# yozoyugen/HAKAI-fem

Hardware: AMD Instinct MI355X
Metric: M element-updates/sec (hex8, 8 Gauss pts) at 1/2/4/8 MI355X; % HBM roofline (higher is better)
Workload: dtype f64

## Files before the change

hakai-fem_amd/csrc/hakai_capi.cpp:

```cpp
#include <hip/hip_runtime.h>

#include <algorithm>
#include <cmath>
#include <cstdarg>
#include <cstdio>
#include <cstdlib>
#include <cstring>
#include <map>
#include <string>
#include <vector>

#include "../../include/hakai_hip.h"
#include "hakai_history.hpp"
#include "hakai_internal.hpp"
#include "hakai_kernels.hpp"
#include "hakai_own_plan.hpp"

using hk::DevMat;

namespace {
thread_local std::string g_err;
}

namespace hkc {

int fail(int code, const char* fmt, ...) {
    char buf[1024];
    va_list ap;
    va_start(ap, fmt);
    vsnprintf(buf, sizeof buf, fmt, ap);
    va_end(ap);
    g_err = buf;
    return code;
}

int hip_fail(hipError_t e, const char* what) {
    return fail(HAKAI_ERR_DEVICE, "%s: %s", what, hipGetErrorString(e));
}

}

using hkc::fail;
using hkc::hip_fail;

#define HIPCHK(x)                                           \
    do {                                                    \
        hipError_t _e = (x);                                \
        if (_e != hipSuccess) return hip_fail(_e, #x);      \
    } while (0)

template <class T>
static hipError_t dalloc(T** p, size_t n) {
    *p = nullptr;
    if (n == 0) n = 1;
    return hipMalloc((void**)p, n * sizeof(T));
}

template <class T>
static void dfree(T*& p) {
    if (p) (void)hipFree((void*)p);
    p = nullptr;
}

namespace hkc {

static void own_free(hakai_ctx* c) {
    dfree(c->d_own_off);
    dfree(c->d_own_seq);
    dfree(c->d_own_bstart);
    dfree(c->d_own_list);
    dfree(c->d_own_q);
    dfree(c->d_own_rp);
    dfree(c->d_own_rows);
    dfree(c->d_own_ridx);
    dfree(c->d_own_dump);
    c->own_built_g = -1;
    c->own_for_g0 = -1;
    c->own_valid = false;
}

static void free_model(hakai_ctx* c) {
    contact_destroy(c);
    dfree(c->d_coord);
    dfree(c->d_u[0]);
    dfree(c->d_u[1]);
    dfree(c->d_mass);
    dfree(c->d_conn);
    dfree(c->d_flag);
    dfree(c->d_mat);
    dfree(c->d_mats);
    dfree(c->d_stress);
    dfree(c->d_strain);
    dfree(c->d_eqps);
    dfree(c->d_yield);
    dfree(c->d_triax);
    dfree(c->d_fe);
    dfree(c->d_inc_ptr);
    dfree(c->d_inc);
    dfree(c->d_inc_row);
    dfree(c->d_inc8);
    dfree(c->d_del_step);
    dfree(c->d_qbuf);
    dfree(c->d_fext);
    own_free(c);
    c->model_ok = false;
    c->state_ok = false;
}

static void free_bc(hakai_ctx* c) {
    dfree(c->d_bc_of_node);
    dfree(c->d_bc_dof);
    dfree(c->d_bc_grp);
    dfree(c->d_bc_val);
    dfree(c->d_amp_n);
    dfree(c->d_amp_off);
    dfree(c->d_amp_t);
    dfree(c->d_amp_v);
    c->nbc = 0;
}

int build_devmat(const hakai_material_t& in, DevMat& o) {
    std::memset(&o, 0, sizeof o);
    const double young = in.young, poisson = in.poisson;
    const double d1 = (1.0 - poisson), d2 = poisson, d3 = (1.0 - 2.0 * poisson) / 2.0;
    const double cc = young / (1.0 + poisson) / (1.0 - 2.0 * poisson);
    o.Dn = cc * d1;
    o.Do = cc * d2;
    o.Ds = cc * d3;
    o.G = young / 2. / (1.0 + poisson);
    o.density = in.density;
    if (in.n_plastic < 0 || in.n_plastic > hk::kMaxPlastic)
        return fail(HAKAI_ERR_ARG, "material: %d plastic rows (max %d)", in.n_plastic, hk::kMaxPlastic);
    if (in.n_ductile < 0 || in.n_ductile > hk::kMaxDuctile)
        return fail(HAKAI_ERR_ARG, "material: %d ductile rows (max %d)", in.n_ductile, hk::kMaxDuctile);
    if (in.n_plastic == 1)
        return fail(HAKAI_ERR_MODEL,
                    "material: a single *Plastic row gives an empty Hd; the reference raises BoundsError "
                    "(v2/HAKAI_j.jl:1267)");
    o.npp = in.n_plastic;
    o.nd = in.n_ductile;
    o.yield0 = in.n_plastic > 0 ? in.plastic[0] : 0.0;
    for (int r = 0; r < in.n_plastic; ++r) o.pl_eps[r] = in.plastic[2 * r + 1];
    for (int r = 0; r + 1 < in.n_plastic; ++r)
        o.Hd[r] = (in.plastic[2 * (r + 1)] - in.plastic[2 * r]) / (in.plastic[2 * (r + 1) + 1] - in.plastic[2 * r + 1]);
    for (int r = 0; r < in.n_ductile; ++r) {
        o.du_eps[r] = in.ductile[3 * r + 0];
        o.du_tri[r] = in.ductile[3 * r + 1];
    }
    double lo = 0.0, hi = 0.0;
    for (int r = 0; r < in.n_ductile; ++r) {
        lo = r == 0 ? o.du_eps[r] : std::min(lo, o.du_eps[r]);
        hi = r == 0 ? o.du_eps[r] : std::max(hi, o.du_eps[r]);
    }
    o.du_floor = in.n_ductile > 0 ? lo - (std::fabs(hi) + std::fabs(lo)) * 0x1p-40 : 0.0;
    if (!(o.du_floor == o.du_floor)) o.du_floor = -HUGE_VAL;
    o.du_skip = o.du_floor > 0.0 ? o.du_floor - o.du_floor * 0x1p-40 : -HUGE_VAL;
    return 0;
}

void pusai_table(double out[192]) {
    static const double delta[8][3] = {{-1.0, -1.0, -1.0}, {1.0, -1.0, -1.0}, {1.0, 1.0, -1.0}, {-1.0, 1.0, -1.0},
                                       {-1.0, -1.0, 1.0},  {1.0, -1.0, 1.0},  {1.0, 1.0, 1.0},  {-1.0, 1.0, 1.0}};
    const double g = 1.0 / std::sqrt(3.0);
    for (int k = 0; k < 8; ++k) {
        const double gzai = (k & 4) ? g : -g, eta = (k & 2) ? g : -g, tueta = (k & 1) ? g : -g;
        for (int i = 0; i < 8; ++i) {
            out[24 * k + i] = 1.0 / 8.0 * delta[i][0] * (1.0 + eta * delta[i][1]) * (1.0 + tueta * delta[i][2]);
            out[24 * k + 8 + i] = 1.0 / 8.0 * delta[i][1] * (1.0 + gzai * delta[i][0]) * (1.0 + tueta * delta[i][2]);
            out[24 * k + 16 + i] = 1.0 / 8.0 * delta[i][2] * (1.0 + gzai * delta[i][0]) * (1.0 + eta * delta[i][1]);
        }
    }
}

hipStream_t ctx_stream(hakai_ctx* c) { return c->stream; }
int ctx_device(hakai_ctx* c) { return c->device; }

}

static void prof_harvest(hakai_ctx* c) {
    if (c->ev_pending.empty()) return;
    (void)hipEventSynchronize(c->ev_pending.back().b);
    for (auto& p : c->ev_pending) {
        float ms = 0.f;
        if (hipEventElapsedTime(&ms, p.a, p.b) == hipSuccess) {
            c->k_ms[p.kernel] += ms;
            c->k_n[p.kernel] += 1;
        }
        c->ev_pool.push_back(p.a);
        c->ev_pool.push_back(p.b);
    }
    c->ev_pending.clear();
}

static hipEvent_t prof_event(hakai_ctx* c) {
    if (c->ev_pool.empty()) {
        if (c->ev_pending.size() >= 2048) prof_harvest(c);
        if (c->ev_pool.empty()) {
            hipEvent_t e;
            (void)hipEventCreate(&e);
            return e;
        }
    }
    hipEvent_t e = c->ev_pool.back();
    c->ev_pool.pop_back();
    return e;
}

namespace hkc {
void prof_begin(hakai_ctx* c, int kernel, EventPair* p) {
    p->kernel = -1;
    if (!c->prof || !((c->prof_mask >> kernel) & 1u)) return;
    p->kernel = kernel;
    p->a = prof_event(c);
    p->b = prof_event(c);
    (void)hipEventRecord(p->a, c->stream);
}
void prof_end(hakai_ctx* c, EventPair* p) {
    if (!c->prof || p->kernel < 0) return;
    (void)hipEventRecord(p->b, c->stream);
    c->ev_pending.push_back(*p);
}
void graph_invalidate(hakai_ctx* c) {
    c->epoch++;
    c->tdev_next = -1;
}
static void graph_free(hakai_ctx* c) {
    for (int g = 0; g < 2; ++g)
        for (int p = 0; p < 2; ++p)
            if (c->g_exec[g][p]) {
                (void)hipGraphExecDestroy(c->g_exec[g][p]);
                c->g_exec[g][p] = nullptr;
                c->g_epoch[g][p] = -1;
            }
}
}


static hk::ElemArgs elem_args(hakai_ctx* c) {
    hk::ElemArgs ea;
    std::memset(&ea, 0, sizeof ea);
    ea.coord = c->d_coord;
    ea.u = c->d_u[c->cur];
    ea.u_pre = c->d_u[1 - c->cur];
    ea.conn = c->d_conn;
    ea.flag = c->d_flag;
    ea.mat = c->d_mat;
    ea.mats = c->d_mats;
    ea.stress = c->d_stress;
    ea.strain = c->d_strain;
    for (int q = 0; q < 6; ++q) {
        ea.sc[q] = c->d_stress + q * c->ld;
        ea.ec[q] = c->d_strain + q * c->ld;
    }
    ea.eqps = c->d_eqps;
    ea.yield = c->d_yield;
    ea.triax = c->d_triax;
    ea.fe = c->d_fe;
    ea.vol = nullptr;
    ea.nE = c->nE;
    ea.nEp = c->nEp;
    ea.ld = c->ld;
    ea.del_step = c->d_del_step;
    ea.step_i = 0;
    ea.any_plastic = c->any_plastic ? 1 : 0;
    ea.pipe_blocks = (c->nEp / 32 >= (long long)c->pipe_min * c->pipe_blocks) ? c->pipe_blocks : 0;
    ea.gp_nt = c->gp_nt;
    ea.nmat = c->nmat;
    ea.exact = c->elem_exact;
    ea.pusai = c->d_pusai;
    ea.poison = c->d_poison;
    return ea;
}

static int fe_download_qe(hakai_ctx* c, double* Qe) {
    HIPCHK(hipMemcpyAsync(Qe, c->d_fe, 24 * (size_t)c->nE * sizeof(double), hipMemcpyDeviceToHost, c->stream));
    HIPCHK(hipStreamSynchronize(c->stream));
    return 0;
}

static int fe_upload_qe(hakai_ctx* c, const double* Qe) {
    HIPCHK(hipMemcpyAsync(c->d_fe, Qe, 24 * (size_t)c->nE * sizeof(double), hipMemcpyHostToDevice, c->stream));
    HIPCHK(hipStreamSynchronize(c->stream));
    return 0;
}

static int fe_upload_incidence(hakai_ctx* c) {
    std::vector<int> inc(c->h_inc0.size());
    for (size_t j = 0; j < inc.size(); ++j) inc[j] = 24 * (c->h_inc0[j] >> 3) + 3 * (c->h_inc0[j] & 7);
    if (!inc.empty())
        HIPCHK(hipMemcpyAsync(c->d_inc, inc.data(), inc.size() * sizeof(int), hipMemcpyHostToDevice, c->stream));
    if (c->d_inc8) {
        std::vector<int> inc8(8 * (size_t)c->nN, (int)(24 * c->nEp));
        for (long long n = 0; n < c->nN; ++n)
            for (int j = c->h_ptr[n]; j < c->h_ptr[n + 1]; ++j) inc8[8 * n + (j - c->h_ptr[n])] = inc[j];
        HIPCHK(hipMemcpyAsync(c->d_inc8, inc8.data(), inc8.size() * sizeof(int), hipMemcpyHostToDevice, c->stream));
    }
    HIPCHK(hipStreamSynchronize(c->stream));
    return 0;
}

extern "C" {

int hakai_abi_version(void) { return HAKAI_ABI_VERSION; }
const char* hakai_last_error(void) { return g_err.c_str(); }

int hakai_device_count(int* n) {
    if (!n) return fail(HAKAI_ERR_ARG, "null");
    int cnt = 0;
    if (hipGetDeviceCount(&cnt) != hipSuccess) cnt = 0;
    *n = cnt;
    return 0;
}

int hakai_create(hakai_ctx** out, int device) {
    if (!out) return fail(HAKAI_ERR_ARG, "null ctx pointer");
    *out = nullptr;
    int cnt = 0;
    if (hipGetDeviceCount(&cnt) != hipSuccess || cnt <= 0)
        return fail(HAKAI_ERR_DEVICE, "no HIP device visible: the HAKAI MI355X path has no CPU fallback");
    if (device < 0 || device >= cnt) return fail(HAKAI_ERR_ARG, "device %d out of range (%d visible)", device, cnt);
    HIPCHK(hipSetDevice(device));
    hipDeviceProp_t prop;
    HIPCHK(hipGetDeviceProperties(&prop, device));
    if (std::strncmp(prop.gcnArchName, "gfx950", 6) != 0)
        return fail(HAKAI_ERR_DEVICE, "device %d is %s; libhakai_hip is built for gfx950 only", device,
                    prop.gcnArchName);
    hakai_ctx* c = new hakai_ctx();
    c->device = device;
    if (const char* v = std::getenv("HAKAI_PIPE_BLOCKS")) c->pipe_blocks = std::atoi(v);
    if (const char* v = std::getenv("HAKAI_GRAPH")) {
        const int g = std::atoi(v);
        c->graph = (g >= 0 && g <= 1024 && !(g & 1)) ? g : 0;
    }
    hipError_t e = hipStreamCreateWithFlags(&c->stream, hipStreamNonBlocking);
    if (e != hipSuccess) {
        delete c;
        return hip_fail(e, "hipStreamCreate");
    }
    if (dalloc(&c->d_negjac, 1) != hipSuccess || dalloc(&c->d_pusai, 192) != hipSuccess ||
        dalloc(&c->d_poison, 2) != hipSuccess || hipMemset(c->d_poison, 0, 2 * sizeof(int)) != hipSuccess) {
        dfree(c->d_negjac);
        dfree(c->d_pusai);
        dfree(c->d_poison);
        delete c;
        return fail(HAKAI_ERR_DEVICE, "hipMalloc for context bookkeeping failed");
    }
    {
        double pus[192];
        hkc::pusai_table(pus);
        bool odd = true;
        for (int k = 0; k < 8; ++k)
            for (int i = 0; i < 8; ++i) {
                const double* p = pus + 24 * k;
                odd = odd && p[i] == -p[i ^ 1] && p[8 + i] == -p[8 + (i ^ 3)] && p[16 + i] == -p[16 + (i ^ 4)];
            }
        e = odd ? hipMemcpy(c->d_pusai, pus, sizeof pus, hipMemcpyHostToDevice) : hipErrorInvalidValue;
        if (e != hipSuccess) {
            dfree(c->d_negjac);
            dfree(c->d_pusai);
            dfree(c->d_poison);
            delete c;
            return hip_fail(e, "hipMemcpy (Pusai table)");
        }
    }
    if (const char* v = std::getenv("HAKAI_ELEM_EXACT")) c->elem_exact = std::atoi(v) ? 1 : 0;
    if (const char* v = std::getenv("HAKAI_OWN_ASSEMBLY")) c->own_assembly = std::atoi(v) ? 1 : 0;
    *out = c;
    return 0;
}

int hakai_destroy(hakai_ctx* c) {
    if (!c) return 0;
    (void)hipSetDevice(c->device);
    (void)hipStreamSynchronize(c->stream);
    prof_harvest(c);
    hkc::graph_free(c);
    dfree(c->d_tstep);
    hkc::history_destroy(c);
    hkc::comm_destroy(c);
    hkc::free_model(c);
    hkc::free_bc(c);
    dfree(c->d_negjac);
    dfree(c->d_pusai);
    dfree(c->d_poison);
    for (auto e : c->ev_pool) (void)hipEventDestroy(e);
    (void)hipStreamDestroy(c->stream);
    delete c;
    return 0;
}

int hakai_upload_model(hakai_ctx* c, int64_t nNode, const double* coordmat, int64_t nElement,
                       const int64_t* elementmat, const int64_t* element_material, int32_t nMat,
                       const hakai_material_t* mats, const double* diag_M) {
    if (c) hkc::graph_invalidate(c);
    if (!c) return fail(HAKAI_ERR_ARG, "null ctx");
    if (nNode <= 0 || nElement < 0 || !coordmat || (nElement > 0 && (!elementmat || !element_material)) || nMat <= 0 ||
        !mats || !diag_M)
        return fail(HAKAI_ERR_ARG, "upload_model: bad arguments");
    if (26 * (nElement + 32) + 8 >= (int64_t)INT32_MAX || nNode >= (int64_t)INT32_MAX)
        return fail(HAKAI_ERR_ARG, "upload_model: mesh too large for int32 indexing on one rank");
    if (192 * (nElement + 32) >= (int64_t)1 << 32)
        return fail(HAKAI_ERR_ARG, "upload_model: %lld elements exceed one context's 32-bit element-kernel offsets "
                    "(max %lld); split the mesh over ranks", (long long)nElement, (long long)(((int64_t)1 << 32) / 192 - 32));
    if (24 * (nNode + 1) >= (int64_t)1 << 32)
        return fail(HAKAI_ERR_ARG, "upload_model: %lld nodes exceed one context's 32-bit element-kernel offsets "
                    "(max %lld); split the mesh over ranks", (long long)nNode, (long long)(((int64_t)1 << 32) / 24 - 1));
    HIPCHK(hipSetDevice(c->device));
    (void)hipStreamSynchronize(c->stream);
    hkc::history_destroy(c);
    hkc::free_model(c);
    hkc::free_bc(c);
    const long long nN = nNode, nE = nElement;
    const long long nEp = ((nE + 31) / 32) * 32;
    std::vector<int> conn((size_t)(8 * nEp), 0), mat((size_t)nEp, 0);
    for (long long e = 0; e < nE; ++e) {
        for (int i = 0; i < 8; ++i) {
            const int64_t n = elementmat[8 * e + i];
            if (n < 1 || n > nN) return fail(HAKAI_ERR_ARG, "elementmat[%d,%lld] = %lld out of 1..%lld", i + 1, e + 1, (long long)n, nN);
            conn[8 * e + i] = (int)(n - 1);
        }
        const int64_t m = element_material[e];
        if (m < 1 || m > nMat) return fail(HAKAI_ERR_ARG, "element_material[%lld] = %lld out of 1..%d", e + 1, (long long)m, nMat);
        mat[e] = (int)(m - 1);
    }
    std::vector<double> mass((size_t)nN);
    for (long long n = 0; n < nN; ++n) {
        const double m0 = diag_M[3 * n], m1 = diag_M[3 * n + 1], m2 = diag_M[3 * n + 2];
        if (!(m0 == m1 && m1 == m2))
            return fail(HAKAI_ERR_ARG, "diag_M: node %lld has different masses per dof", n + 1);
        mass[n] = m0;
    }
    c->h_mats.assign((size_t)nMat, DevMat());
    c->nmat = nMat;
    c->has_ductile = false;
    for (int i = 0; i < nMat; ++i) {
        int r = hkc::build_devmat(mats[i], c->h_mats[i]);
        if (r) return r;
    }
    c->any_plastic = false;
    for (long long e = 0; e < nE; ++e) {
        if (c->h_mats[mat[e]].nd > 0) c->has_ductile = true;
        if (c->h_mats[mat[e]].npp > 0) c->any_plastic = true;
    }
    std::vector<int> ptr((size_t)nN + 1, 0), inc((size_t)(8 * nE));
    for (long long j = 0; j < 8 * nE; ++j) ptr[conn[j] + 1]++;
    for (long long n = 0; n < nN; ++n) ptr[n + 1] += ptr[n];
    {
        std::vector<int> fill(ptr.begin(), ptr.end() - 1);
        for (long long j = 0; j < 8 * nE; ++j) inc[fill[conn[j]]++] = (int)j;
    }
    int maxinc = 0;
    for (long long n = 0; n < nN; ++n) maxinc = std::max(maxinc, ptr[n + 1] - ptr[n]);
    c->nN = nN;
    c->nE = nE;
    c->nEp = nEp;
    c->ld = 8 * nEp;
    const size_t ld = (size_t)c->ld;
    HIPCHK(dalloc(&c->d_coord, 3 * (size_t)nN));
    HIPCHK(dalloc(&c->d_u[0], 3 * (size_t)nN));
    HIPCHK(dalloc(&c->d_u[1], 3 * (size_t)nN));
    HIPCHK(dalloc(&c->d_mass, (size_t)nN));
    HIPCHK(dalloc(&c->d_conn, 8 * (size_t)nEp));
    HIPCHK(dalloc(&c->d_flag, (size_t)nEp));
    HIPCHK(dalloc(&c->d_mat, (size_t)nEp));
    HIPCHK(dalloc(&c->d_del_step, (size_t)nEp + 2));
    HIPCHK(dalloc(&c->d_mats, (size_t)nMat));
    HIPCHK(dalloc(&c->d_stress, 6 * ld));
    HIPCHK(dalloc(&c->d_strain, 6 * ld));
    HIPCHK(dalloc(&c->d_eqps, ld));
    HIPCHK(dalloc(&c->d_yield, ld));
    HIPCHK(dalloc(&c->d_triax, ld));
    c->fe_len = 26 * nEp + 8;
    HIPCHK(dalloc(&c->d_fe, (size_t)c->fe_len));
    HIPCHK(dalloc(&c->d_inc_ptr, (size_t)nN + 1));
    HIPCHK(dalloc(&c->d_inc, 8 * (size_t)nE));
    HIPCHK(dalloc(&c->d_inc_row, 8 * (size_t)nE));
    HIPCHK(dalloc(&c->d_qbuf, 3 * (size_t)nN));
    hipStream_t s = c->stream;
    HIPCHK(hipMemcpyAsync(c->d_coord, coordmat, 3 * nN * sizeof(double), hipMemcpyHostToDevice, s));
    HIPCHK(hipMemcpyAsync(c->d_mass, mass.data(), nN * sizeof(double), hipMemcpyHostToDevice, s));
    if (nE) {
        HIPCHK(hipMemcpyAsync(c->d_conn, conn.data(), 8 * nEp * sizeof(int), hipMemcpyHostToDevice, s));
        HIPCHK(hipMemcpyAsync(c->d_mat, mat.data(), nEp * sizeof(int), hipMemcpyHostToDevice, s));
        HIPCHK(hipMemcpyAsync(c->d_inc_row, inc.data(), 8 * nE * sizeof(int), hipMemcpyHostToDevice, s));
    }
    HIPCHK(hipMemcpyAsync(c->d_mats, c->h_mats.data(), nMat * sizeof(DevMat), hipMemcpyHostToDevice, s));
    HIPCHK(hipMemcpyAsync(c->d_inc_ptr, ptr.data(), (nN + 1) * sizeof(int), hipMemcpyHostToDevice, s));
    if (maxinc <= 8) HIPCHK(dalloc(&c->d_inc8, 8 * (size_t)nN));
    HIPCHK(hipStreamSynchronize(s));
    c->max_inc = maxinc;
    c->h_ptr = ptr;
    c->h_inc0 = inc;
    {
        int r = fe_upload_incidence(c);
        if (r) return r;
    }
    c->h_coord.assign(coordmat, coordmat + 3 * nN);
    c->h_conn.assign(conn.begin(), conn.begin() + 8 * nE);
    c->h_mat.assign(mat.begin(), mat.begin() + nE);
    c->h_young.resize((size_t)nMat);
    for (int i = 0; i < nMat; ++i) c->h_young[i] = mats[i].young;
    c->model_ok = true;
    c->state_ok = false;
    return hakai_reset_state(c, 0, nullptr, nullptr, 1.0);
}

int hakai_set_bc(hakai_ctx* c, const hakai_bc_t* bc) {
    if (c) hkc::graph_invalidate(c);
    if (!c || !bc) return fail(HAKAI_ERR_ARG, "null");
    if (!c->model_ok) return fail(HAKAI_ERR_STATE, "set_bc before upload_model");
    HIPCHK(hipSetDevice(c->device));
    (void)hipStreamSynchronize(c->stream);
    hkc::free_bc(c);
    const int G = bc->n_groups;
    if (G <= 0) return hkc::history_bc_changed(c);
    std::map<long long, std::pair<int, double>> last;
    for (int g = 0; g < G; ++g) {
        if (bc->amp_n[g] == 1)
            return fail(HAKAI_ERR_MODEL, "BC group %d: one-point amplitude, the reference raises BoundsError (:598)", g + 1);
        for (int64_t en = bc->entry_off[g]; en < bc->entry_off[g + 1]; ++en)
            for (int64_t d = bc->dof_off[en]; d < bc->dof_off[en + 1]; ++d) {
                const int64_t dof = bc->dofs[d];
                if (dof < 1 || dof > 3 * c->nN) return fail(HAKAI_ERR_ARG, "BC dof %lld out of range", (long long)dof);
                last[dof - 1] = std::make_pair(g, bc->entry_value[en]);
            }
    }
    std::vector<int> dof, grp;
    std::vector<double> val;
    for (auto& kv : last) {
        dof.push_back((int)kv.first);
        grp.push_back(kv.second.first);
        val.push_back(kv.second.second);
    }
    std::vector<int> amp_n(G), amp_off(G);
    long long n_amp = 0;
    for (int g = 0; g < G; ++g) {
        amp_n[g] = bc->amp_n[g];
        amp_off[g] = (int)bc->amp_off[g];
        n_amp = std::max<long long>(n_amp, bc->amp_off[g] + bc->amp_n[g]);
    }
    c->nbc = (int)dof.size();
    HIPCHK(dalloc(&c->d_bc_dof, dof.size()));
    HIPCHK(dalloc(&c->d_bc_grp, grp.size()));
    HIPCHK(dalloc(&c->d_bc_val, val.size()));
    HIPCHK(dalloc(&c->d_amp_n, (size_t)G));
    HIPCHK(dalloc(&c->d_amp_off, (size_t)G));
    HIPCHK(dalloc(&c->d_amp_t, (size_t)n_amp));
    HIPCHK(dalloc(&c->d_amp_v, (size_t)n_amp));
    hipStream_t s = c->stream;
    if (!dof.empty()) {
        HIPCHK(hipMemcpyAsync(c->d_bc_dof, dof.data(), dof.size() * sizeof(int), hipMemcpyHostToDevice, s));
        HIPCHK(hipMemcpyAsync(c->d_bc_grp, grp.data(), grp.size() * sizeof(int), hipMemcpyHostToDevice, s));
        HIPCHK(hipMemcpyAsync(c->d_bc_val, val.data(), val.size() * sizeof(double), hipMemcpyHostToDevice, s));
    }
    HIPCHK(hipMemcpyAsync(c->d_amp_n, amp_n.data(), G * sizeof(int), hipMemcpyHostToDevice, s));
    HIPCHK(hipMemcpyAsync(c->d_amp_off, amp_off.data(), G * sizeof(int), hipMemcpyHostToDevice, s));
    if (n_amp) {
        HIPCHK(hipMemcpyAsync(c->d_amp_t, bc->amp_time, n_amp * sizeof(double), hipMemcpyHostToDevice, s));
        HIPCHK(hipMemcpyAsync(c->d_amp_v, bc->amp_value, n_amp * sizeof(double), hipMemcpyHostToDevice, s));
    }
    if (!dof.empty()) {
        std::vector<int> of((size_t)c->nN, -1);
        for (size_t i = dof.size(); i-- > 0;) of[(size_t)dof[i] / 3] = (int)i;
        HIPCHK(dalloc(&c->d_bc_of_node, of.size()));
        HIPCHK(hipMemcpyAsync(c->d_bc_of_node, of.data(), of.size() * sizeof(int), hipMemcpyHostToDevice, s));
    }
    HIPCHK(hipStreamSynchronize(s));
    return hkc::history_bc_changed(c);
}

int hakai_reset_state(hakai_ctx* c, int64_t n_ic, const int64_t* ic_dofs, const double* ic_values, double d_time) {
    if (c) hkc::graph_invalidate(c);
    if (c) c->own_valid = false;
    if (!c) return fail(HAKAI_ERR_ARG, "null");
    if (!c->model_ok) return fail(HAKAI_ERR_STATE, "reset_state before upload_model");
    HIPCHK(hipSetDevice(c->device));
    hipStream_t s = c->stream;
    const size_t fn = 3 * (size_t)c->nN;
    c->cur = 0;
    HIPCHK(hipMemsetAsync(c->d_u[0], 0, fn * sizeof(double), s));
    HIPCHK(hipMemsetAsync(c->d_u[1], 0, fn * sizeof(double), s));
    HIPCHK(hipMemsetAsync(c->d_fe, 0, (size_t)c->fe_len * sizeof(double), s));
    HIPCHK(hipMemsetAsync(c->d_del_step, 0, ((size_t)c->nEp + 2) * sizeof(int), s));
    HIPCHK(hk::launch_reset_gp(c->d_stress, c->d_strain, c->d_eqps, c->d_yield, c->d_triax, c->d_flag, c->d_mat,
                               c->d_mats, c->nE, c->nEp, c->ld, s));
    c->h_velo0.assign(fn, 0.0);
    c->q_from_buf = false;
    c->fe_ok = c->triax_ok = true;
    c->steps_done = 0;
    HIPCHK(hipMemsetAsync(c->d_poison, 0, 2 * sizeof(int), s));
    hkc::comm_reset(c);
    if (n_ic > 0) {
        if (!ic_dofs || !ic_values) return fail(HAKAI_ERR_ARG, "reset_state: null IC arrays");
        std::vector<double> dpre(fn, 0.0);
        for (int64_t j = 0; j < n_ic; ++j) {
            const int64_t d = ic_dofs[j];
            if (d < 1 || d > (int64_t)fn) return fail(HAKAI_ERR_ARG, "IC dof %lld out of range", (long long)d);
            dpre[d - 1] = -ic_values[j] * d_time;
            c->h_velo0[d - 1] = ic_values[j];
        }
        HIPCHK(hipMemcpyAsync(c->d_u[1 - c->cur], dpre.data(), fn * sizeof(double), hipMemcpyHostToDevice, s));
        HIPCHK(hipStreamSynchronize(s));
    }
    c->state_ok = true;
    if (int r = hkc::contact_state_reset(c, c->h_velo0.data())) return r;
    if (int r = hkc::history_restart(c)) return r;
    HIPCHK(hipStreamSynchronize(s));
    return 0;
}

static int own_materialize(hakai_ctx* c);

int hakai_upload_state(hakai_ctx* c, const hakai_state_t* st) {
    if (c) hkc::graph_invalidate(c);
    if (!c || !st) return fail(HAKAI_ERR_ARG, "null");
    if (!c->model_ok) return fail(HAKAI_ERR_STATE, "upload_state before upload_model");
    HIPCHK(hipSetDevice(c->device));
    if (c->own_valid && !c->fe_ok && !st->Q && !st->Qe) {
        bool dels = false;
        for (long long e = 0; st->element_flag && e < c->nE && !dels; ++e) dels = st->element_flag[e] == 0;
        if (dels || c->comm)
            return fail(HAKAI_ERR_STATE, "upload_state: the last element step's forces exist only as owner-computed "
                        "node sums (a contact overflow skipped the call's last step); upload Q (from "
                        "hakai_download_state) or Qe with this state");
        if (int r = own_materialize(c)) return r;
    }
    c->own_valid = false;
    hipStream_t s = c->stream;
    const size_t fn = 3 * (size_t)c->nN, nGP = 8 * (size_t)c->nE;
    if (st->disp) HIPCHK(hipMemcpyAsync(c->d_u[c->cur], st->disp, fn * sizeof(double), hipMemcpyHostToDevice, s));
    if (st->disp_pre)
        HIPCHK(hipMemcpyAsync(c->d_u[1 - c->cur], st->disp_pre, fn * sizeof(double), hipMemcpyHostToDevice, s));
    if (st->velo) c->h_velo0.assign(st->velo, st->velo + fn);
    if (st->Q) {
        HIPCHK(hipMemcpyAsync(c->d_qbuf, st->Q, fn * sizeof(double), hipMemcpyHostToDevice, s));
        c->q_from_buf = true;
    }
    if (st->integ_stress || st->integ_strain) {
        double* tmp = nullptr;
        HIPCHK(dalloc(&tmp, 6 * nGP));
        if (st->integ_stress) {
            HIPCHK(hipMemcpyAsync(tmp, st->integ_stress, 6 * nGP * sizeof(double), hipMemcpyHostToDevice, s));
            HIPCHK(hk::launch_aos_to_soa6(tmp, c->d_stress, (long long)nGP, c->ld, s));
        }
        if (st->integ_strain) {
            HIPCHK(hipMemcpyAsync(tmp, st->integ_strain, 6 * nGP * sizeof(double), hipMemcpyHostToDevice, s));
            HIPCHK(hk::launch_aos_to_soa6(tmp, c->d_strain, (long long)nGP, c->ld, s));
        }
        HIPCHK(hipStreamSynchronize(s));
        dfree(tmp);
    }
    if (st->integ_yield_stress)
        HIPCHK(hipMemcpyAsync(c->d_yield, st->integ_yield_stress, nGP * sizeof(double), hipMemcpyHostToDevice, s));
    if (st->integ_eq_plastic_strain)
        HIPCHK(hipMemcpyAsync(c->d_eqps, st->integ_eq_plastic_strain, nGP * sizeof(double), hipMemcpyHostToDevice, s));
    if (st->integ_triax_stress)
        HIPCHK(hipMemcpyAsync(c->d_triax, st->integ_triax_stress, nGP * sizeof(double), hipMemcpyHostToDevice, s));
    if (st->element_flag) {
        std::vector<int> f((size_t)c->nE);
        for (long long e = 0; e < c->nE; ++e) f[e] = st->element_flag[e] != 0 ? 1 : 0;
        HIPCHK(hipMemcpyAsync(c->d_flag, f.data(), c->nE * sizeof(int), hipMemcpyHostToDevice, s));
        std::vector<int> ds((size_t)c->nE);
        for (long long e = 0; e < c->nE; ++e) ds[e] = f[e] ? 0 : -1;
        HIPCHK(hipMemcpyAsync(c->d_del_step, ds.data(), c->nE * sizeof(int), hipMemcpyHostToDevice, s));
        HIPCHK(hipMemsetAsync(c->d_del_step + c->nEp, 0, 2 * sizeof(int), s));
        HIPCHK(hipStreamSynchronize(s));
        bool any = false;
        for (long long e = 0; e < c->nE; ++e) any |= !f[e];
        if (any && !st->Qe) {
            std::vector<double> qe(24 * (size_t)c->nE);
            int r = fe_download_qe(c, qe.data());
            if (r) return r;
            for (long long e = 0; e < c->nE; ++e)
                if (!f[e]) std::fill(qe.begin() + 24 * e, qe.begin() + 24 * (e + 1), 0.0);
            if ((r = fe_upload_qe(c, qe.data()))) return r;
        }
    }
    if (st->Qe) {
        int r = fe_upload_qe(c, st->Qe);
        if (r) return r;
    }
    HIPCHK(hipMemsetAsync(c->d_poison, 0, 2 * sizeof(int), s));
    HIPCHK(hipStreamSynchronize(s));
    c->steps_done = 0;
    c->fe_ok = c->triax_ok = true;
    hkc::comm_reset(c);
    c->state_ok = true;
    if (int r = hkc::history_restart(c)) return r;
    if (c->contact) {
        if (int r = hkc::contact_state_reset(c, c->h_velo0.empty() ? nullptr : c->h_velo0.data())) return r;
        HIPCHK(hipStreamSynchronize(s));
    }
    return 0;
}

int hakai_download_state(hakai_ctx* c, hakai_state_t* st) {
    if (!c || !st) return fail(HAKAI_ERR_ARG, "null");
    if (!c->state_ok) return fail(HAKAI_ERR_STATE, "download_state without state");
    if (st->Qe && !c->fe_ok)
        return fail(HAKAI_ERR_STATE, "download_state: Qe is not available after a call whose last steps a contact "
                    "overflow skipped (owner-computed assembly keeps node sums only); Q is -- or step once more");
    if (st->integ_triax_stress && !c->triax_ok)
        return fail(HAKAI_ERR_STATE, "download_state: integ_triax_stress is not available after a call whose last "
                    "steps a contact overflow skipped (it is stored on a call's last step); step once more");
    HIPCHK(hipSetDevice(c->device));
    hipStream_t s = c->stream;
    const size_t fn = 3 * (size_t)c->nN, nGP = 8 * (size_t)c->nE;
    HIPCHK(hipStreamSynchronize(s));
    if (st->disp) HIPCHK(hipMemcpyAsync(st->disp, c->d_u[c->cur], fn * sizeof(double), hipMemcpyDeviceToHost, s));
    if (st->disp_pre)
        HIPCHK(hipMemcpyAsync(st->disp_pre, c->d_u[1 - c->cur], fn * sizeof(double), hipMemcpyDeviceToHost, s));
    if (st->velo) {
        if (c->steps_done == 0) {
            std::memcpy(st->velo, c->h_velo0.data(), fn * sizeof(double));
        } else {
            std::vector<double> a(fn), b(fn);
            HIPCHK(hipMemcpyAsync(a.data(), c->d_u[c->cur], fn * sizeof(double), hipMemcpyDeviceToHost, s));
            HIPCHK(hipMemcpyAsync(b.data(), c->d_u[1 - c->cur], fn * sizeof(double), hipMemcpyDeviceToHost, s));
            HIPCHK(hipStreamSynchronize(s));
            for (size_t i = 0; i < fn; ++i) {
                const double dd = a[i] - b[i];
                st->velo[i] = dd / c->last_dt;
            }
        }
    }
    if (st->Q) {
        if (c->q_from_buf) {
            HIPCHK(hipMemcpyAsync(st->Q, c->d_qbuf, fn * sizeof(double), hipMemcpyDeviceToHost, s));
        } else {
            double* tmp = nullptr;
            HIPCHK(dalloc(&tmp, fn));
            if (c->own_valid)
                HIPCHK(hk::launch_own_q(c->d_own_q, c->d_own_rp, c->d_own_ridx, c->d_own_rows, tmp, c->nN, s));
            else
                HIPCHK(hk::launch_gather_q(c->d_inc_ptr, c->d_inc, c->d_fe, tmp, c->nN, s));
            HIPCHK(hipMemcpyAsync(st->Q, tmp, fn * sizeof(double), hipMemcpyDeviceToHost, s));
            HIPCHK(hipStreamSynchronize(s));
            dfree(tmp);
        }
    }
    if (st->integ_stress || st->integ_strain) {
        double* tmp = nullptr;
        HIPCHK(dalloc(&tmp, 6 * nGP));
        if (st->integ_stress) {
            HIPCHK(hk::launch_soa_to_aos6(c->d_stress, tmp, (long long)nGP, c->ld, s));
            HIPCHK(hipMemcpyAsync(st->integ_stress, tmp, 6 * nGP * sizeof(double), hipMemcpyDeviceToHost, s));
            HIPCHK(hipStreamSynchronize(s));
        }
        if (st->integ_strain) {
            HIPCHK(hk::launch_soa_to_aos6(c->d_strain, tmp, (long long)nGP, c->ld, s));
            HIPCHK(hipMemcpyAsync(st->integ_strain, tmp, 6 * nGP * sizeof(double), hipMemcpyDeviceToHost, s));
            HIPCHK(hipStreamSynchronize(s));
        }
        dfree(tmp);
    }
    if (st->integ_yield_stress)
        HIPCHK(hipMemcpyAsync(st->integ_yield_stress, c->d_yield, nGP * sizeof(double), hipMemcpyDeviceToHost, s));
    if (st->integ_eq_plastic_strain)
        HIPCHK(hipMemcpyAsync(st->integ_eq_plastic_strain, c->d_eqps, nGP * sizeof(double), hipMemcpyDeviceToHost, s));
    if (st->integ_triax_stress)
        HIPCHK(hipMemcpyAsync(st->integ_triax_stress, c->d_triax, nGP * sizeof(double), hipMemcpyDeviceToHost, s));
    if (st->element_flag) {
        std::vector<int> f((size_t)c->nE);
        HIPCHK(hipMemcpyAsync(f.data(), c->d_flag, c->nE * sizeof(int), hipMemcpyDeviceToHost, s));
        HIPCHK(hipStreamSynchronize(s));
        for (long long e = 0; e < c->nE; ++e) st->element_flag[e] = (f[e] == 1) ? 1 : 0;
    }
    if (st->Qe) {
        int r = fe_download_qe(c, st->Qe);
        if (r) return r;
    }
    HIPCHK(hipStreamSynchronize(s));
    return 0;
}

static bool own_upload(hakai_ctx* c, const hk::OwnSched& sc, const hk::OwnPlan& pl) {
    hkc::own_free(c);
    const long long nN = c->nN, G = (long long)sc.bstart.size() - 1;
    std::vector<int> bst(sc.bstart.begin(), sc.bstart.end());
    hipStream_t s = c->stream;
    auto up = [&](int** d, const std::vector<int>& h) -> hipError_t {
        hipError_t e = dalloc(d, std::max<size_t>(h.size(), 1));
        if (e == hipSuccess && !h.empty()) e = hipMemcpyAsync(*d, h.data(), h.size() * sizeof(int), hipMemcpyHostToDevice, s);
        return e;
    };
    if (up(&c->d_own_off, pl.off) || up(&c->d_own_seq, sc.seq) || up(&c->d_own_bstart, bst) ||
        up(&c->d_own_list, pl.list) || up(&c->d_own_rp, pl.rp) || up(&c->d_own_ridx, pl.ridx) ||
        dalloc(&c->d_own_q, 3 * (size_t)nN) || dalloc(&c->d_own_rows, 3 * (size_t)std::max(pl.rows, 1LL)) ||
        dalloc(&c->d_own_dump, 8 * (size_t)G) ||
        hipMemsetAsync(c->d_own_q, 0, 3 * (size_t)nN * sizeof(double), s) ||
        hipStreamSynchronize(s)) {
        hkc::own_free(c);
        return false;
    }
    c->own_nop = (int)pl.ne;
    c->own_slots = pl.max_slots;
    c->own_rows = pl.rows;
    c->own_entries = pl.ne;
    c->own_built_g = G;
    c->own_s = pl.S;
    c->own_round2 = pl.round2;
    c->own_banded = sc.banded ? 1 : 0;
    return true;
}

static long long own_grid(const hakai_ctx* c) {
    const long long nb = c->nEp / 32;
    const bool pipe = nb >= (long long)c->pipe_min * c->pipe_blocks && c->pipe_blocks > 0;
    return pipe ? std::min<long long>(nb, c->pipe_blocks) : 0;
}

static int own_materialize(hakai_ctx* c) {
    if (!c->own_valid) return 0;
    if (c->comm)
        return fail(HAKAI_ERR_STATE, "owner-computed assembly cannot be switched off or rebuilt on a multi-GPU rank "
                    "mid-run: upload or reset the state first");
    HIPCHK(hk::launch_own_q(c->d_own_q, c->d_own_rp, c->d_own_ridx, c->d_own_rows, c->d_qbuf, c->nN, c->stream));
    c->q_from_buf = true;
    c->own_valid = false;
    return 0;
}

static bool own_use(hakai_ctx* c) {
    if (!c->own_assembly || c->nmat > hk::kMaxLdsMats || c->nE <= 0)
        return false;
    const long long G0 = own_grid(c);
    if (G0 <= 0) return false;
    bool ok = c->own_built_g > 0;
    if (c->own_for_g0 != G0) {
        if (c->own_valid && own_materialize(c)) return false;
        const hk::OwnInput in{c->nE, c->nN, c->nEp, c->h_conn, c->h_ptr, c->h_inc0, c->max_inc,
                              c->own_band_rows, c->own_pass_batches, hkc::comm_dn_nodes(c),
                              {hk::own_slot_cap(c->elem_exact != 0, 1, c->nmat),
                               hk::own_slot_cap(c->elem_exact != 0, 2, c->nmat)}};
        hk::OwnSched sc;
        hk::OwnPlan pl;
        ok = hk::own_choose(in, G0, sc, pl) && own_upload(c, sc, pl);
        if (!ok) {
            hkc::own_free(c);
            c->own_built_g = -2;
        }
        c->own_for_g0 = G0;
    }
    if (ok && c->elem_exact && c->own_round2 > 0 && c->own_assembly == 1 && !(c->comm && c->own_valid))
        return false;
    return ok;
}

enum { kPhaseA1 = 1, kPhaseRest = 2, kPhaseA2 = 4, kPhaseA3 = 8, kPhaseAll = 15 };
static int step_once(hakai_ctx* c, double t, double d_time, bool last, int phase = kPhaseAll) {
    hipStream_t s = c->stream;
    EventPair ep;
    if (c->contact) {
        const int part_bit[3] = {kPhaseA1, kPhaseA2, kPhaseA3};
        for (int part = 1; part <= 3; ++part) {
            if (!(phase & part_bit[part - 1]) || (part > 1 && !hkc::contact_multi(c))) continue;
            hkc::prof_begin(c, HAKAI_K_CONTACT, &ep);
            const int rc = hkc::contact_phase(c, part, t, d_time);
            hkc::prof_end(c, &ep);
            if (rc) return rc;
        }
    }
    if (!(phase & kPhaseRest)) return 0;
    const int par = c->cur;
    hk::NodalArgs na;
    na.u = c->d_u[c->cur];
    na.u_pre_out = c->d_u[1 - c->cur];
    na.mass = c->d_mass;
    na.inc_ptr = c->d_inc_ptr;
    na.inc = c->d_inc;
    na.inc8 = c->d_inc8;
    na.fe = c->d_fe;
    const bool own = own_use(c);
    if (c->own_valid && !own) {
        if (int r = own_materialize(c)) return r;
    }
    na.qbuf = c->q_from_buf ? c->d_qbuf : nullptr;
    na.fext = nullptr;
    na.nN = c->nN;
    na.dt = d_time;
    na.bc_of_node = nullptr;
    const bool own_q = c->own_valid && !na.qbuf;
    na.own_q = own_q ? c->d_own_q : nullptr;
    na.own_rp = own_q ? c->d_own_rp : nullptr;
    na.own_rows = own_q ? c->d_own_rows : nullptr;
    na.own_ridx = own_q ? c->d_own_ridx : nullptr;
    hk::BCArgs ba;
    ba.dof = c->d_bc_dof;
    ba.grp = c->d_bc_grp;
    ba.val = c->d_bc_val;
    ba.n = c->nbc;
    ba.amp_n = c->d_amp_n;
    ba.amp_off = c->d_amp_off;
    ba.amp_t = c->d_amp_t;
    ba.amp_v = c->d_amp_v;
    ba.out = c->d_u[1 - c->cur];
    ba.ct = t * d_time;
    ba.t_rd = c->g_trd;
    ba.dt = d_time;
    ba.poison = c->d_poison;
    na.poison = c->d_poison;
    const bool fuse_bc = c->nbc > 0 && c->d_bc_of_node && c->fuse_bc && !c->comm &&
                         (c->nN <= kFuseBcMaxNodes || c->fuse_bc == 2);
    if (fuse_bc) {
        na.bc_of_node = c->d_bc_of_node;
        na.bc = ba;
    }
    int rc = 0;
    if (c->contact) {
        if (hkc::contact_multi(c)) {
            hkc::prof_begin(c, HAKAI_K_CONTACT_SUM, &ep);
            rc = hkc::contact_step_b(c);
            hkc::prof_end(c, &ep);
            if (rc) return rc;
        }
        na.fext = c->d_fext;
    }
    rc = hkc::comm_pre_nodal(c);
    if (rc) return rc;
    if (c->hist && (rc = hkc::history_seed(c, na, s))) return rc;
    hkc::prof_begin(c, HAKAI_K_NODAL, &ep);
    HIPCHK(hk::launch_nodal(na, s));
    hkc::prof_end(c, &ep);
    hkc::CommFix fix;
    rc = hkc::comm_post_nodal(c, d_time, &fix);
    if (rc) return rc;
    if (c->nbc > 0 && !fuse_bc) {
        hkc::prof_begin(c, HAKAI_K_BC, &ep);
        HIPCHK(hk::launch_bc(ba, s));
        hkc::prof_end(c, &ep);
    }
    if (c->hist && (rc = hkc::history_step(c, na, fix, t, c->g_trd, s))) return rc;
    c->cur = 1 - c->cur;
    c->q_from_buf = false;
    hk::ElemArgs ea = elem_args(c);
    ea.step_i = (int)t;
    if (own) {
        ea.own = c->own_s;
        ea.own_grid = (int)c->own_built_g;
        ea.own_seq = c->d_own_seq;
        ea.own_bstart = c->d_own_bstart;
        ea.own_off = c->d_own_off;
        ea.own_list = reinterpret_cast<const int4*>(c->d_own_list);
        ea.own_nop = c->own_nop;
        ea.own_slots = c->own_slots;
        ea.own_q = c->d_own_q;
        ea.own_rows = c->d_own_rows;
        ea.own_dump = c->d_own_dump;
    }
    if (c->g_trd) {
        ea.t_rd = c->g_trd;
        ea.t_wr = c->d_tstep + par;
    }
    hkc::prof_begin(c, HAKAI_K_ELEMENT, &ep);
    HIPCHK(hk::launch_element(ea, c->has_ductile, last, s));
    hkc::prof_end(c, &ep);
    c->own_valid = own;
    c->own_steps += own ? 1 : 0;
    c->fe_ok = !own || last;
    c->triax_ok = last;
    rc = hkc::comm_post_element(c, (long long)t);
    if (rc) return rc;
    rc = hkc::contact_post_step(c);
    if (rc) return rc;
    c->steps_done++;
    c->last_dt = d_time;
    return 0;
}

static bool graph_eligible(const hakai_ctx* c, double t) {
    return c->graph && !c->comm && !c->prof && !c->q_from_buf && c->nE > 0 && hkc::contact_graph_ok(c, t) &&
           !hkc::history_needs_seed(c) &&
           c->own_valid == own_use(const_cast<hakai_ctx*>(c));
}

static int step_graph(hakai_ctx* c, double t, double d_time, int len) {
    hipStream_t s = c->stream;
    const int p0 = c->cur;
    const int gi = len == 2 ? 1 : 0;
    hipGraphExec_t& ge = c->g_exec[gi][p0];
    if (!c->d_tstep) HIPCHK(dalloc(&c->d_tstep, 2));
    if (c->tdev_next != (long long)t) HIPCHK(hk::launch_set_step(c->d_tstep + (1 - p0), t - 1.0, s));
    if (ge && (c->g_epoch[gi][p0] != c->epoch || c->g_dt[gi][p0] != d_time || c->g_len[gi][p0] != len)) {
        HIPCHK(hipStreamSynchronize(s));
        (void)hipGraphExecDestroy(ge);
        ge = nullptr;
    }
    if (!ge) {
        hipGraph_t g = nullptr;
        HIPCHK(hipStreamBeginCapture(s, hipStreamCaptureModeThreadLocal));
        int rc = 0;
        for (int k = 0; k < len && !rc; ++k) {
            c->g_trd = c->d_tstep + (1 - c->cur);
            rc = step_once(c, t + k, d_time, false);
        }
        c->g_trd = nullptr;
        hipError_t e = hipStreamEndCapture(s, &g);
        if (rc) {
            if (g) (void)hipGraphDestroy(g);
            return rc;
        }
        if (e != hipSuccess) return hip_fail(e, "hipStreamEndCapture (step graph)");
        e = hipGraphInstantiate(&ge, g, nullptr, nullptr, 0);
        (void)hipGraphDestroy(g);
        if (e != hipSuccess) {
            ge = nullptr;
            return hip_fail(e, "hipGraphInstantiate (step graph)");
        }
        c->g_epoch[gi][p0] = c->epoch;
        c->g_dt[gi][p0] = d_time;
        c->g_len[gi][p0] = len;
    } else {
        hkc::contact_graph_advance(c, t + len - 1);
        c->q_from_buf = false;
        c->own_steps += c->own_valid ? len : 0;
        c->fe_ok = !c->own_valid;
        c->triax_ok = false;
        c->steps_done += len;
        c->last_dt = d_time;
    }
    HIPCHK(hipGraphLaunch(ge, s));
    c->tdev_next = (long long)t + len;
    c->graph_steps += len;
    return 0;
}

struct CallSnap {
    int cur = 0;
    long long done = 0;
    bool fe_ok = true, triax_ok = true, own_valid = false, q_from_buf = false;
    bool comm_pending = false;
    int comm_par = 0;
};
static CallSnap call_snap(const hakai_ctx* c) {
    CallSnap s;
    hkc::comm_pending_get(c, &s.comm_pending, &s.comm_par);
    s.cur = c->cur;
    s.done = c->steps_done;
    s.fe_ok = c->fe_ok;
    s.triax_ok = c->triax_ok;
    s.own_valid = c->own_valid;
    s.q_from_buf = c->q_from_buf;
    return s;
}

static int finish_call(hakai_ctx* c, double t_first, int64_t n_steps, const CallSnap& s0) {
    const int rc = hkc::contact_check(c);
    if (rc && c->contact) {
        int pz[2] = {0, 0};
        HIPCHK(hipMemcpy(pz, c->d_poison, sizeof pz, hipMemcpyDeviceToHost));
        if (pz[0]) {
            c->poison_step = pz[1];
            const long long good = (long long)pz[1] - (long long)t_first;
            const bool rolled = good >= 0 && good <= n_steps;
            if (rolled) {
                c->cur = (good & 1) ? 1 - s0.cur : s0.cur;
                c->steps_done = s0.done + good;
                if (good == 0) {
                    c->fe_ok = s0.fe_ok;
                    c->triax_ok = s0.triax_ok;
                    c->own_valid = s0.own_valid;
                    c->q_from_buf = s0.q_from_buf;
                } else {
                    c->fe_ok = !c->own_valid;
                    c->triax_ok = false;
                }
                hkc::comm_rollback(c, good > 0, (long long)pz[1] - 1, s0.comm_pending, s0.comm_par);
            }
            hkc::graph_invalidate(c);
            hkc::contact_after_overflow(c, c->steps_done);
            if (!rolled) (void)hkc::contact_exchange_retry(c);
            HIPCHK(hipMemset(c->d_poison, 0, 2 * sizeof(int)));
            const std::string msg = hakai_last_error();
            return fail(rc, "%s; step %d was not applied: the state is that after step %d", msg.c_str(), pz[1],
                        pz[1] - 1);
        }
    }
    return rc;
}

static int step_call(hakai_ctx* c, double t_first, int64_t n_steps, double d_time);
static constexpr int kExchangeRetries = 8;

int hakai_step(hakai_ctx* c, double t_first, int64_t n_steps, double d_time) {
    if (!c) return fail(HAKAI_ERR_ARG, "null");
    if (!c->model_ok || !c->state_ok) return fail(HAKAI_ERR_STATE, "step before upload_model/reset_state");
    if (n_steps < 0 || !(d_time > 0)) return fail(HAKAI_ERR_ARG, "step: n_steps=%lld d_time=%g", (long long)n_steps, d_time);
    if (n_steps > 1 && hkc::comm_is_local(c))
        return fail(HAKAI_ERR_ARG, "step: an in-process group is stepped one step per call, rank by rank");
    if (hkc::comm_is_local(c) && hkc::contact_multi(c) && hkc::comm_size(c) > 1)
        return fail(HAKAI_ERR_STATE, "step: rank %d of an in-process group with multi-GPU contact is stepped by "
                    "hakai_step_group only", hkc::comm_rank(c));
    HIPCHK(hipSetDevice(c->device));
    for (int attempt = 0;; ++attempt) {
        const int rc = step_call(c, t_first, n_steps, d_time);
        if (!rc || attempt >= kExchangeRetries || !hkc::contact_exchange_retry(c)) return rc;
        ++c->exchange_retries;
        n_steps -= (int64_t)(c->poison_step - (long long)t_first);
        t_first = (double)c->poison_step;
    }
}

static int step_call(hakai_ctx* c, double t_first, int64_t n_steps, double d_time) {
    (void)own_use(c);
    const CallSnap s0 = call_snap(c);
    int64_t it = 0;
    while (it < n_steps) {
        const double t = t_first + (double)it;
        int rc;
        const int len = (c->graph > 2 && it + c->graph < n_steps) ? c->graph : 2;
        if (c->graph && it + len < n_steps && graph_eligible(c, t)) {
            rc = step_graph(c, t, d_time, len);
            it += len;
        } else {
            rc = step_once(c, t, d_time, it == n_steps - 1);
            c->tdev_next = -1;
            ++it;
        }
        if (rc) return rc;
    }
    return finish_call(c, t_first, n_steps, s0);
}

static int step_group_call(hakai_ctx** ctxs, int32_t n, double t_first, int64_t n_steps, double d_time) {
    std::vector<CallSnap> s0(n);
    for (int r = 0; r < n; ++r) {
        (void)own_use(ctxs[r]);
        s0[r] = call_snap(ctxs[r]);
    }
    const int phases[4] = {kPhaseA1, kPhaseA2, kPhaseA3, kPhaseRest};
    for (int64_t it = 0; it < n_steps; ++it) {
        const double t = t_first + (double)it;
        const bool last = it == n_steps - 1;
        for (int ph : phases)
            for (int r = 0; r < n; ++r) {
                if (ctxs[0]->group_serial == 2) HIPCHK(hk::launch_hold(96, ctxs[r]->stream));
                if (int rc = step_once(ctxs[r], t, d_time, last, ph)) return rc;
                if (ph == kPhaseRest) ctxs[r]->tdev_next = -1;
                if (ctxs[0]->group_serial) HIPCHK(hipStreamSynchronize(ctxs[r]->stream));
            }
    }
    int first = 0;
    for (int r = 0; r < n; ++r) {
        const int rc = finish_call(ctxs[r], t_first, n_steps, s0[r]);
        if (rc && !first) first = rc;
    }
    return first;
}

int hakai_step_group(hakai_ctx** ctxs, int32_t n, double t_first, int64_t n_steps, double d_time) {
    if (!ctxs || n <= 0) return fail(HAKAI_ERR_ARG, "step_group: no contexts");
    if (n_steps < 0 || !(d_time > 0)) return fail(HAKAI_ERR_ARG, "step_group: n_steps=%lld d_time=%g",
                                                  (long long)n_steps, d_time);
    for (int r = 0; r < n; ++r) {
        hakai_ctx* c = ctxs[r];
        if (!c) return fail(HAKAI_ERR_ARG, "step_group: null context %d", r);
        if (!c->model_ok || !c->state_ok) return fail(HAKAI_ERR_STATE, "step_group: rank %d has no model/state", r);
        if (n > 1 && (!c->comm || hkc::comm_rank(c) != r || hkc::comm_size(c) != n ||
                      hkc::comm_peer_ctx(c, r) != c))
            return fail(HAKAI_ERR_ARG, "step_group: context %d is not rank %d of an in-process group of %d", r, r, n);
        hkc::graph_invalidate(c);
    }
    HIPCHK(hipSetDevice(ctxs[0]->device));
    for (int attempt = 0;; ++attempt) {
        const int rc = step_group_call(ctxs, n, t_first, n_steps, d_time);
        if (!rc || attempt >= kExchangeRetries) return rc;
        bool retry = true;
        for (int r = 0; r < n; ++r) retry = hkc::contact_exchange_retry(ctxs[r]) && retry;
        if (!retry) return rc;
        const long long p = ctxs[0]->poison_step;
        for (int r = 1; r < n; ++r)
            if (ctxs[r]->poison_step != p)
                return fail(rc, "step_group: ranks disagree on the poisoned step (rank 0: %lld, rank %d: %lld)", p, r,
                            ctxs[r]->poison_step);
        for (int r = 0; r < n; ++r) ++ctxs[r]->exchange_retries;
        n_steps -= (int64_t)(p - (long long)t_first);
        t_first = (double)p;
    }
}

int hakai_graph_steps(hakai_ctx* c, int64_t* n) {
    if (!c || !n) return fail(HAKAI_ERR_ARG, "null");
    *n = c->graph_steps;
    return 0;
}

int hakai_stat(hakai_ctx* c, const char* key, int64_t* value) {
    if (!c || !key || !value) return fail(HAKAI_ERR_ARG, "null");
    if (!std::strcmp(key, "graph_steps")) *value = c->graph_steps;
    else if (!std::strcmp(key, "own_steps")) *value = c->own_steps;
    else if (!std::strcmp(key, "exchange_retries")) *value = c->exchange_retries;
    else if (!std::strcmp(key, "own_rows")) *value = c->own_built_g > 0 ? c->own_rows : -1;
    else if (!std::strcmp(key, "own_entries")) *value = c->own_built_g > 0 ? c->own_entries : -1;
    else if (!std::strcmp(key, "own_superbatch")) *value = c->own_built_g > 0 ? c->own_s : 0;
    else if (!std::strcmp(key, "own_round2")) *value = c->own_built_g > 0 ? c->own_round2 : 0;
    else if (!std::strcmp(key, "own_slots")) *value = c->own_built_g > 0 ? c->own_slots : 0;
    else if (!std::strcmp(key, "own_banded")) *value = c->own_built_g > 0 ? c->own_banded : 0;
    else if (!std::strcmp(key, "own_grid")) *value = c->own_built_g > 0 ? c->own_built_g : 0;
    else return fail(HAKAI_ERR_ARG, "unknown stat '%s'", key);
    return 0;
}

int hakai_sync(hakai_ctx* c) {
    if (!c) return fail(HAKAI_ERR_ARG, "null");
    HIPCHK(hipSetDevice(c->device));
    HIPCHK(hipStreamSynchronize(c->stream));
    return 0;
}

int hakai_deleted(hakai_ctx* c, int64_t* n_deleted, int64_t* log, int64_t cap) {
    if (!c) return fail(HAKAI_ERR_ARG, "null");
    if (!c->model_ok) return fail(HAKAI_ERR_STATE, "deleted before upload_model");
    HIPCHK(hipSetDevice(c->device));
    std::vector<int> ds((size_t)c->nE);
    if (c->nE) HIPCHK(hipMemcpyAsync(ds.data(), c->d_del_step, c->nE * sizeof(int), hipMemcpyDeviceToHost, c->stream));
    HIPCHK(hipStreamSynchronize(c->stream));
    std::vector<std::pair<long long, long long>> v;
    for (long long e = 0; e < c->nE; ++e)
        if (ds[e] > 0) v.push_back(std::make_pair((long long)ds[e], e + 1 + c->elem_offset));
    std::sort(v.begin(), v.end());
    if (n_deleted) *n_deleted = (int64_t)v.size();
    if (log)
        for (long long i = 0; i < (long long)v.size() && i < cap; ++i) {
            log[2 * i] = v[i].first;
            log[2 * i + 1] = v[i].second;
        }
    return 0;
}

int hakai_set_tuning(hakai_ctx* c, const char* key, int64_t value) {
    if (c) hkc::graph_invalidate(c);
    if (!c || !key) return fail(HAKAI_ERR_ARG, "set_tuning: null");
    if (!std::strcmp(key, "elem_pipe_blocks")) {
        if (value < 0 || value > 65536) return fail(HAKAI_ERR_ARG, "elem_pipe_blocks out of range");
        c->pipe_blocks = (int)value;
        return 0;
    }
    if (!std::strcmp(key, "elem_gp_nt")) {
        if (value != 0 && value != 1) return fail(HAKAI_ERR_ARG, "elem_gp_nt must be 0 or 1");
        c->gp_nt = (int)value;
        return 0;
    }
    if (!std::strcmp(key, "fuse_bc")) {
        if (value < 0 || value > 2) return fail(HAKAI_ERR_ARG, "fuse_bc must be 0, 1 or 2 (any mesh size)");
        c->fuse_bc = (int)value;
        return 0;
    }
    if (!std::strcmp(key, "elem_pipe_min")) {
        if (value < 0 || value > 1024) return fail(HAKAI_ERR_ARG, "elem_pipe_min out of range");
        c->pipe_min = (int)value;
        return 0;
    }
    if (!std::strcmp(key, "elem_exact")) {
        if (value != 0 && value != 1) return fail(HAKAI_ERR_ARG, "elem_exact must be 0 or 1");
        if (c->elem_exact != (int)value && c->own_for_g0 != -1) {
            if (!(c->comm && c->own_valid)) {
                c->own_for_g0 = -1;
            } else if (c->own_built_g > 0 && c->own_slots > hk::own_slot_cap(value != 0, c->own_s, c->nmat)) {
                return fail(HAKAI_ERR_STATE, "elem_exact: the owner-assembly lists of this multi-GPU rank need %d LDS "
                            "slots, more than the %s kernel has; switch between calls after hakai_upload_state / "
                            "hakai_reset_state", c->own_slots, value ? "reference-order" : "fused");
            }
        }
        c->elem_exact = (int)value;
        return 0;
    }
    if (!std::strcmp(key, "group_serial")) {
        if (value < 0 || value > 2) return fail(HAKAI_ERR_ARG, "group_serial must be 0, 1 or 2");
        c->group_serial = (int)value;
        return 0;
    }
    if (!std::strcmp(key, "nodal_padded")) {
        if (!value) {
            dfree(c->d_inc8);
            return 0;
        }
        return c->d_inc8 ? 0 : fail(HAKAI_ERR_STATE, "padded incidence table unavailable (>8 incidences)");
    }
    if (!std::strcmp(key, "own_assembly")) {
        if (value < 0 || value > 2) return fail(HAKAI_ERR_ARG, "own_assembly must be 0, 1 or 2");
        c->own_assembly = (int)value;
        return 0;
    }
    if (!std::strcmp(key, "own_pass_batches")) {
        if (value < 0 || value > 2) return fail(HAKAI_ERR_ARG, "own_pass_batches must be 0, 1 or 2");
        if (c->own_pass_batches != (int)value) c->own_for_g0 = -1;
        c->own_pass_batches = (int)value;
        return 0;
    }
    if (!std::strcmp(key, "own_band_rows")) {
        if (value < 0 || value > 4096) return fail(HAKAI_ERR_ARG, "own_band_rows must be in [0, 4096]");
        if (c->own_band_rows != (int)value) c->own_for_g0 = -1;
        c->own_band_rows = (int)value;
        return 0;
    }
    if (!std::strcmp(key, "graph")) {
        if (value < 0 || value > 1024 || (value & 1)) return fail(HAKAI_ERR_ARG, "graph must be 0 or an even step count <= 1024");
        c->graph = (int)value;
        return 0;
    }
    if (!std::strcmp(key, "history_one_block")) {
        if (value < -1 || value > 1) return fail(HAKAI_ERR_ARG, "history_one_block must be -1 (by size), 0 or 1");
        c->hist_one_block = (int)value;
        return 0;
    }
    if (!std::strncmp(key, "contact_", 8)) {
        HIPCHK(hipSetDevice(c->device));
        return hkc::contact_tuning(c, key, value);
    }
    return fail(HAKAI_ERR_ARG, "unknown tuning key '%s'", key);
}

int hakai_set_element_offset(hakai_ctx* c, int64_t element_offset) {
    if (c) hkc::graph_invalidate(c);
    if (!c || element_offset < 0) return fail(HAKAI_ERR_ARG, "set_element_offset: bad args");
    c->elem_offset = element_offset;
    return 0;
}

int hakai_negative_jacobians(hakai_ctx* c, int64_t* n) {
    if (!c || !n) return fail(HAKAI_ERR_ARG, "null");
    if (!c->state_ok) return fail(HAKAI_ERR_STATE, "negative_jacobians without state");
    HIPCHK(hipSetDevice(c->device));
    HIPCHK(hipMemsetAsync(c->d_negjac, 0, sizeof(unsigned long long), c->stream));
    HIPCHK(hk::launch_negjac(elem_args(c), c->d_negjac, c->stream));
    unsigned long long v = 0;
    HIPCHK(hipMemcpyAsync(&v, c->d_negjac, sizeof v, hipMemcpyDeviceToHost, c->stream));
    HIPCHK(hipStreamSynchronize(c->stream));
    *n = (int64_t)v;
    return 0;
}

int hakai_node_stress_strain(hakai_ctx* c, double* node_stress, double* node_strain, double* node_eqps,
                             double* node_mises, double* node_triax) {
    if (!c) return fail(HAKAI_ERR_ARG, "null");
    if (!c->state_ok) return fail(HAKAI_ERR_STATE, "node_stress_strain without state");
    HIPCHK(hipSetDevice(c->device));
    hipStream_t s = c->stream;
    const size_t nN = (size_t)c->nN;
    double *ns = nullptr, *nn = nullptr, *ne = nullptr, *nm = nullptr, *nt = nullptr;
    HIPCHK(dalloc(&ns, 6 * nN));
    HIPCHK(dalloc(&nn, 6 * nN));
    HIPCHK(dalloc(&ne, nN));
    HIPCHK(dalloc(&nm, nN));
    HIPCHK(dalloc(&nt, nN));
    HIPCHK(hk::launch_node_average(c->d_inc_ptr, c->d_inc_row, c->d_stress, c->d_strain, c->d_eqps, c->d_triax, c->ld,
                                   c->nN, ns, nn, ne, nm, nt, s));
    if (node_stress) HIPCHK(hipMemcpyAsync(node_stress, ns, 6 * nN * sizeof(double), hipMemcpyDeviceToHost, s));
    if (node_strain) HIPCHK(hipMemcpyAsync(node_strain, nn, 6 * nN * sizeof(double), hipMemcpyDeviceToHost, s));
    if (node_eqps) HIPCHK(hipMemcpyAsync(node_eqps, ne, nN * sizeof(double), hipMemcpyDeviceToHost, s));
    if (node_mises) HIPCHK(hipMemcpyAsync(node_mises, nm, nN * sizeof(double), hipMemcpyDeviceToHost, s));
    if (node_triax) HIPCHK(hipMemcpyAsync(node_triax, nt, nN * sizeof(double), hipMemcpyDeviceToHost, s));
    HIPCHK(hipStreamSynchronize(s));
    dfree(ns);
    dfree(nn);
    dfree(ne);
    dfree(nm);
    dfree(nt);
    return 0;
}

int hakai_profile_enable(hakai_ctx* c, int on) { return hakai_profile_mask(c, on ? (1u << HAKAI_K_COUNT) - 1 : 0u); }

int hakai_profile_mask(hakai_ctx* c, uint32_t mask) {
    if (c) hkc::graph_invalidate(c);
    if (!c) return fail(HAKAI_ERR_ARG, "null");
    if (!mask) prof_harvest(c);
    c->prof = mask != 0;
    c->prof_mask = mask;
    for (int k = 0; k < HAKAI_K_COUNT; ++k) {
        c->k_ms[k] = 0;
        c->k_n[k] = 0;
    }
    return 0;
}

int hakai_profile_read(hakai_ctx* c, int kernel, double* total_ms, int64_t* launches) {
    if (!c || kernel < 0 || kernel >= HAKAI_K_COUNT) return fail(HAKAI_ERR_ARG, "bad profile query");
    (void)hipSetDevice(c->device);
    prof_harvest(c);
    if (total_ms) *total_ms = c->k_ms[kernel];
    if (launches) *launches = c->k_n[kernel];
    return 0;
}

int hakai_stress_hexa(int device, int64_t nNode, int64_t nElement, double* Qe, double* integ_stress,
                      double* integ_strain, double* integ_yield_stress, double* integ_eq_plastic_strain,
                      const double* position, const double* d_disp, const int64_t* elementmat,
                      const int64_t* element_flag, int32_t integ_num, int32_t nMat, const hakai_material_t* mats,
                      const int64_t* element_material, double* elementVolume) {
    if (integ_num != 8) return fail(HAKAI_ERR_ARG, "integ_num must be 8 (v2/HAKAI_j.jl:177)");
    if (!Qe || !integ_stress || !integ_strain || !integ_yield_stress || !integ_eq_plastic_strain || !position ||
        !d_disp || !element_flag)
        return fail(HAKAI_ERR_ARG, "stress_hexa: null array");
    hakai_ctx* c = nullptr;
    int r = hakai_create(&c, device);
    if (r) return r;
    struct Guard {
        hakai_ctx* c;
        ~Guard() { hakai_destroy(c); }
    } guard{c};
    std::vector<double> ones(3 * (size_t)nNode, 1.0);
    r = hakai_upload_model(c, nNode, position, nElement, elementmat, element_material, nMat, mats, ones.data());
    if (r) return r;
    std::vector<double> zero(3 * (size_t)nNode, 0.0), mdu(3 * (size_t)nNode);
    for (size_t i = 0; i < mdu.size(); ++i) mdu[i] = -d_disp[i];
    hakai_state_t st;
    std::memset(&st, 0, sizeof st);
    st.disp = zero.data();
    st.disp_pre = mdu.data();
    st.integ_stress = integ_stress;
    st.integ_strain = integ_strain;
    st.integ_yield_stress = integ_yield_stress;
    st.integ_eq_plastic_strain = integ_eq_plastic_strain;
    st.element_flag = const_cast<int64_t*>(element_flag);
    r = hakai_upload_state(c, &st);
    if (r) return r;
    hipStream_t s = c->stream;
    double* d_vol = nullptr;
    HIPCHK(dalloc(&d_vol, (size_t)c->nEp));
    HIPCHK(hipMemsetAsync(c->d_fe, 0, 24 * (size_t)nElement * sizeof(double), s));
    hk::ElemArgs ea = elem_args(c);
    ea.vol = d_vol;
    ea.pipe_blocks = 0;
    HIPCHK(hk::launch_element(ea, false, false, s));
    std::vector<double> fe(24 * (size_t)nElement), vol((size_t)nElement);
    HIPCHK(hipMemcpyAsync(fe.data(), c->d_fe, fe.size() * sizeof(double), hipMemcpyDeviceToHost, s));
    HIPCHK(hipMemcpyAsync(vol.data(), d_vol, vol.size() * sizeof(double), hipMemcpyDeviceToHost, s));
    HIPCHK(hipStreamSynchronize(s));
    dfree(d_vol);
    c->steps_done = 1;
    c->last_dt = 1.0;
    hakai_state_t out;
    std::memset(&out, 0, sizeof out);
// ... 38 lines not shown
```

hakai-fem_amd/csrc/hakai_comm.cpp:

```cpp
#include <hip/hip_runtime.h>
#include <rccl/rccl.h>

#include <algorithm>
#include <cstdint>
#include <cstring>
#include <map>
#include <mutex>
#include <vector>

#include "hakai_internal.hpp"

namespace hkc {

struct LocalGroup;

struct Comm {
    int mode = 0;
    ncclComm_t nc = nullptr;
    LocalGroup* group = nullptr;
    long long group_key = 0;
    int rank = 0, nranks = 1;
    hipStream_t cs = nullptr;
    hipEvent_t ev_packed[2] = {nullptr, nullptr}, ev_done = nullptr;
    int nslot = 0;
// ... 224 lines not shown
        hipEventCreateWithFlags(&m->ev_done, hipEventDisableTiming) != hipSuccess) {
        c->comm = m;
        hkc::comm_destroy(c);
        return fail(HAKAI_ERR_DEVICE, "comm_init: stream/event creation failed");
    }
    c->comm = m;
    return 0;
}

__global__ void k_gather_local(hkc::LocalGather g, char* dst) {
    const int q = (int)blockIdx.y;
    const char* src = g.src[q];
    char* out = dst + g.off[q];
    const long long nb = g.bytes[q];
    if (!src || nb <= 0) return;
    const long long nw = nb >> 3;
    const long long stride = (long long)gridDim.x * blockDim.x;
    const long long i0 = blockIdx.x * (long long)blockDim.x + threadIdx.x;
    for (long long i = i0; i < nw; i += stride)
        reinterpret_cast<unsigned long long*>(out)[i] = reinterpret_cast<const unsigned long long*>(src)[i];
    for (long long i = (nw << 3) + i0; i < nb; i += stride) out[i] = src[i];
}

}

namespace hkc {

int gather_local(hakai_ctx* c, const LocalGather& g, int n, void* dst) {
    long long mx = 0;
    for (int q = 0; q < n; ++q) {
        if (((uintptr_t)g.src[q] | (uintptr_t)g.off[q]) & 7)
            return fail(HAKAI_ERR_ARG, "gather_local: rank %d block not 8-byte aligned", q);
        mx = std::max(mx, g.bytes[q]);
    }
    if (mx <= 0) return 0;
    const unsigned gx = (unsigned)std::min<long long>(std::max<long long>(((mx >> 3) + 255) / 256, 1), 512);
    hipLaunchKernelGGL(k_gather_local, dim3(gx, (unsigned)n), dim3(256), 0, c->stream, g, (char*)dst);
    HIPCHK(hipGetLastError());
    return 0;
}

void comm_destroy(hakai_ctx* c) {
    Comm* m = c->comm;
    if (!m) return;
    if (m->cs) (void)hipStreamSynchronize(m->cs);
    (void)hipStreamSynchronize(c->stream);
    free_iface(m);
    if (m->nc) (void)ncclCommDestroy(m->nc);
    if (m->group) {
        std::lock_guard<std::mutex> lk(g_groups_mu);
        m->group->ctx[m->rank] = nullptr;
        if (--m->group->refs == 0) {
            g_groups.erase(m->group_key);
            delete m->group;
        }
    }
    for (int p = 0; p < 2; ++p)
        if (m->ev_packed[p]) (void)hipEventDestroy(m->ev_packed[p]);
    if (m->ev_ag_ready) (void)hipEventDestroy(m->ev_ag_ready);
    if (m->ev_ag_done) (void)hipEventDestroy(m->ev_ag_done);
    if (m->ev_done) (void)hipEventDestroy(m->ev_done);
    if (m->cs) (void)hipStreamDestroy(m->cs);
    delete m;
    c->comm = nullptr;
}

bool comm_is_local(const hakai_ctx* c) {
    return c->comm && c->comm->mode == 1 && (c->comm->n_up + c->comm->n_dn > 0 || c->contact);
}

int comm_rank(const hakai_ctx* c) { return c->comm ? c->comm->rank : 0; }
int comm_size(const hakai_ctx* c) { return c->comm ? c->comm->nranks : 1; }

int comm_allgather_raw(hakai_ctx* c, const void* send, void* recv, size_t bytes) {
    Comm* m = c->comm;
    if (!m || m->mode != 0) return fail(HAKAI_ERR_STATE, "all-gather: not an RCCL communicator");
    if (bytes == 0) return 0;
    HIPCHK(hipEventRecord(m->ev_ag_ready, c->stream));
    HIPCHK(hipStreamWaitEvent(m->cs, m->ev_ag_ready, 0));
    NCCLCHK(ncclAllGather(send, recv, bytes, ncclUint8, m->nc, m->cs));
    HIPCHK(hipEventRecord(m->ev_ag_done, m->cs));
    HIPCHK(hipStreamWaitEvent(c->stream, m->ev_ag_done, 0));
    return 0;
}

int comm_allgatherv_raw(hakai_ctx* c, const void* send, void* recv, const size_t* bytes, const size_t* off) {
    Comm* m = c->comm;
    if (!m || m->mode != 0) return fail(HAKAI_ERR_STATE, "all-gather: not an RCCL communicator");
    HIPCHK(hipEventRecord(m->ev_ag_ready, c->stream));
    HIPCHK(hipStreamWaitEvent(m->cs, m->ev_ag_ready, 0));
    NCCLCHK(ncclGroupStart());
    for (int q = 0; q < m->nranks; ++q) {
        if (q == m->rank) continue;
        if (bytes[m->rank]) NCCLCHK(ncclSend(send, bytes[m->rank], ncclUint8, q, m->nc, m->cs));
        if (bytes[q]) NCCLCHK(ncclRecv(static_cast<char*>(recv) + off[q], bytes[q], ncclUint8, q, m->nc, m->cs));
    }
    NCCLCHK(ncclGroupEnd());
    HIPCHK(hipEventRecord(m->ev_ag_done, m->cs));
    HIPCHK(hipStreamWaitEvent(c->stream, m->ev_ag_done, 0));
    return 0;
}

int comm_allreduce_min_u64(hakai_ctx* c, const void* send, void* recv, size_t count) {
    Comm* m = c->comm;
    if (!m || m->mode != 0) return fail(HAKAI_ERR_STATE, "all-reduce: not an RCCL communicator");
    if (count == 0) return 0;
    HIPCHK(hipEventRecord(m->ev_ag_ready, c->stream));
    HIPCHK(hipStreamWaitEvent(m->cs, m->ev_ag_ready, 0));
    NCCLCHK(ncclAllReduce(send, recv, count, ncclUint64, ncclMin, m->nc, m->cs));
    HIPCHK(hipEventRecord(m->ev_ag_done, m->cs));
    HIPCHK(hipStreamWaitEvent(c->stream, m->ev_ag_done, 0));
    return 0;
}

bool comm_is_rccl(const hakai_ctx* c) { return c->comm && c->comm->mode == 0; }

hakai_ctx* comm_peer_ctx(hakai_ctx* c, int q) {
    Comm* m = c->comm;
    if (!m || m->mode != 1 || !m->group || q < 0 || q >= m->nranks) return nullptr;
    return m->group->ctx[q];
}

int comm_reset(hakai_ctx* c) {
    if (c->comm) c->comm->pending = false;
    return 0;
}

void comm_pending_get(const hakai_ctx* c, bool* pending, int* par) {
    *pending = c->comm && c->comm->pending;
    *par = c->comm ? c->comm->pending_par : 0;
}

void comm_rollback(hakai_ctx* c, bool had_good, long long last_good, bool pending, int par) {
    Comm* m = c->comm;
    if (!m) return;
    if (had_good) {
        m->pending = m->n_up + m->n_dn > 0;
        m->pending_par = (int)(last_good & 1);
    } else {
        m->pending = pending;
        m->pending_par = par;
    }
}

const std::vector<int>* comm_dn_nodes(const hakai_ctx* c) { return c->comm ? &c->comm->h_dn : nullptr; }
const std::vector<int>* comm_up_nodes(const hakai_ctx* c) { return c->comm ? &c->comm->h_up : nullptr; }
bool comm_iface_set(const hakai_ctx* c) { return c->comm && c->comm->iface_set; }

int comm_pre_nodal(hakai_ctx* c) {
    Comm* m = c->comm;
    if (!m || m->n_up + m->n_dn == 0 || !m->pending) return 0;
    const int n = m->n_up + m->n_dn;
    hipLaunchKernelGGL(k_save_upre, dim3((n + 255) / 256), dim3(256), 0, c->stream, m->d_up, m->n_up, m->d_dn, m->n_dn,
                       c->d_u[1 - c->cur], m->d_saved);
    HIPCHK(hipGetLastError());
    return 0;
}

int comm_post_nodal(hakai_ctx* c, double d_time, CommFix* fix) {
    Comm* m = c->comm;
    if (!m || m->n_up + m->n_dn == 0 || !m->pending) return 0;
    m->pending = false;
    const int par = m->pending_par;
    if (fix && !c->q_from_buf) {
        fix->ran = true;
        fix->n_up = m->n_up;
        fix->nslot = m->nslot;
        fix->up_sendP = m->d_up_sendP[par];
        fix->up_recvC = m->d_up_recvC;
    }
    EventPair ep;
    prof_begin(c, HAKAI_K_EXCHANGE, &ep);
    if (m->mode == 0) {
        HIPCHK(hipStreamWaitEvent(c->stream, m->ev_done, 0));
    } else {
        if (m->n_up) {
            Comm* p = peer(m, m->rank + 1);
            if (!p) return fail(HAKAI_ERR_COMM, "local group: rank %d missing", m->rank + 1);
            HIPCHK(hipStreamWaitEvent(c->stream, p->ev_packed[par], 0));
            HIPCHK(hipMemcpyAsync(m->d_up_recvC, p->d_dn_sendC[par], sizeof(double) * 3 * m->nslot * m->n_up,
                                  hipMemcpyDeviceToDevice, c->stream));
        }
        if (m->n_dn) {
            Comm* p = peer(m, m->rank - 1);
            if (!p) return fail(HAKAI_ERR_COMM, "local group: rank %d missing", m->rank - 1);
            HIPCHK(hipStreamWaitEvent(c->stream, p->ev_packed[par], 0));
            HIPCHK(hipMemcpyAsync(m->d_dn_recvP, p->d_up_sendP[par], sizeof(double) * 3 * m->n_dn,
                                  hipMemcpyDeviceToDevice, c->stream));
        }
    }
    if (!c->q_from_buf && c->own_valid) {
        const int n = m->n_up + m->n_dn;
        hipLaunchKernelGGL(k_fix_own, dim3((n + 255) / 256), dim3(256), 0, c->stream, m->d_up, m->n_up, m->d_dn,
                           m->n_dn, c->d_own_rp, c->d_own_ridx, c->d_own_rows, m->nslot, m->d_up_sendP[par],
                           m->d_up_recvC, m->d_dn_recvP, m->d_saved, c->d_u[c->cur], c->d_u[1 - c->cur], c->d_mass,
                           c->contact ? c->d_fext : nullptr, d_time, c->d_poison);
        HIPCHK(hipGetLastError());
    } else if (!c->q_from_buf) {
        const int n = m->n_up + m->n_dn;
        hipLaunchKernelGGL(k_fix, dim3((n + 255) / 256), dim3(256), 0, c->stream, m->d_up, m->n_up, m->d_dn, m->n_dn,
                           c->d_inc_ptr, c->d_inc, c->d_fe, m->nslot, m->d_up_sendP[par], m->d_up_recvC, m->d_dn_recvP,
                           m->d_saved, c->d_u[c->cur], c->d_u[1 - c->cur], c->d_mass, c->contact ? c->d_fext : nullptr,
                           d_time, c->d_poison);
        HIPCHK(hipGetLastError());
    }
    prof_end(c, &ep);
    return 0;
}

int comm_post_element(hakai_ctx* c, long long step) {
    Comm* m = c->comm;
    if (!m || m->n_up + m->n_dn == 0) return 0;
    const int par = (int)(step & 1);
    const int n = m->n_up + m->n_dn;
    if (c->own_valid)
        hipLaunchKernelGGL(k_pack_own, dim3((n + 255) / 256), dim3(256), 0, c->stream, m->d_up, m->n_up, m->d_dn,
                           m->n_dn, c->d_own_rp, c->d_own_ridx, c->d_own_rows, c->d_own_q, m->nslot,
                           m->d_up_sendP[par], m->d_dn_sendC[par]);
    else
        hipLaunchKernelGGL(k_pack, dim3((n + 255) / 256), dim3(256), 0, c->stream, m->d_up, m->n_up, m->d_dn, m->n_dn,
                           c->d_inc_ptr, c->d_inc, c->d_fe, m->nslot, m->d_up_sendP[par], m->d_dn_sendC[par]);
    HIPCHK(hipGetLastError());
    HIPCHK(hipEventRecord(m->ev_packed[par], c->stream));
    if (m->mode == 0) {
        HIPCHK(hipStreamWaitEvent(m->cs, m->ev_packed[par], 0));
        NCCLCHK(ncclGroupStart());
        if (m->n_up) {
            NCCLCHK(ncclSend(m->d_up_sendP[par], (size_t)3 * m->n_up, ncclDouble, m->rank + 1, m->nc, m->cs));
            NCCLCHK(ncclRecv(m->d_up_recvC, (size_t)3 * m->nslot * m->n_up, ncclDouble, m->rank + 1, m->nc, m->cs));
        }
        if (m->n_dn) {
            NCCLCHK(ncclSend(m->d_dn_sendC[par], (size_t)3 * m->nslot * m->n_dn, ncclDouble, m->rank - 1, m->nc, m->cs));
            NCCLCHK(ncclRecv(m->d_dn_recvP, (size_t)3 * m->n_dn, ncclDouble, m->rank - 1, m->nc, m->cs));
        }
        NCCLCHK(ncclGroupEnd());
        HIPCHK(hipEventRecord(m->ev_done, m->cs));
    }
    m->pending = true;
    m->pending_par = par;
    return 0;
}

}

extern "C" {

int hakai_comm_unique_id(uint8_t id[128]) {
    if (!id) return fail(HAKAI_ERR_ARG, "null id");
    static_assert(sizeof(ncclUniqueId) == 128, "ncclUniqueId size");
    ncclUniqueId u;
    NCCLCHK(ncclGetUniqueId(&u));
    std::memcpy(id, &u, 128);
    return 0;
}

int hakai_comm_init(hakai_ctx* c, int rank, int nranks, const uint8_t id[128]) {
    if (c) hkc::graph_invalidate(c);
    if (!c || !id || nranks < 1 || rank < 0 || rank >= nranks) return fail(HAKAI_ERR_ARG, "comm_init: bad args");
    if (c->hist)
        return fail(HAKAI_ERR_STATE, "comm_init: history output is enabled (its node ownership comes from the "
                    "interface); disable it first");
    HIPCHK(hipSetDevice(c->device));
    hkc::comm_destroy(c);
    hkc::Comm* m = new hkc::Comm();
    m->rank = rank;
    m->nranks = nranks;
    ncclUniqueId u;
    std::memcpy(&u, id, 128);
    ncclResult_t r = ncclCommInitRank(&m->nc, nranks, u, rank);
    if (r != ncclSuccess) {
        delete m;
        return fail(HAKAI_ERR_COMM, "ncclCommInitRank: %s", ncclGetErrorString(r));
    }
    return comm_common_init(c, m);
}

int hakai_comm_init_local(hakai_ctx* c, int rank, int nranks, int64_t group_key) {
    if (c) hkc::graph_invalidate(c);
    if (!c || nranks < 1 || rank < 0 || rank >= nranks) return fail(HAKAI_ERR_ARG, "comm_init_local: bad args");
    if (c->hist)
        return fail(HAKAI_ERR_STATE, "comm_init_local: history output is enabled (its node ownership comes from "
                    "the interface); disable it first");
    HIPCHK(hipSetDevice(c->device));
    hkc::comm_destroy(c);
    hkc::Comm* m = new hkc::Comm();
    m->mode = 1;
    m->rank = rank;
    m->nranks = nranks;
    m->group_key = group_key;
    {
        std::lock_guard<std::mutex> lk(hkc::g_groups_mu);
        hkc::LocalGroup*& g = hkc::g_groups[group_key];
        if (!g) {
            g = new hkc::LocalGroup();
            g->nranks = nranks;
            g->ctx.assign(nranks, nullptr);
        }
        if (g->nranks != nranks || g->ctx[rank]) {
            delete m;
            return fail(HAKAI_ERR_ARG, "comm_init_local: group %lld size/rank clash", (long long)group_key);
        }
        for (int q = 0; q < nranks; ++q)
            if (g->ctx[q] && g->ctx[q]->device != c->device) {
                delete m;
                return fail(HAKAI_ERR_ARG, "comm_init_local: rank %d is on device %d but rank %d of group %lld is on "
                            "device %d; an in-process group shares one device (use hakai_comm_init, RCCL, across "
                            "devices)", rank, c->device, q, (long long)group_key, g->ctx[q]->device);
            }
        g->ctx[rank] = c;
        g->refs++;
        m->group = g;
    }
    return comm_common_init(c, m);
}

int hakai_set_interface(hakai_ctx* c, int64_t n_shared, const int64_t* local_node, const int32_t* rank_lo,
                        const int32_t* rank_hi) {
    if (c) hkc::graph_invalidate(c);
    if (!c) return fail(HAKAI_ERR_ARG, "null");
    hkc::Comm* m = c->comm;
    if (!m) return fail(HAKAI_ERR_STATE, "set_interface before comm_init");
    if (!c->model_ok) return fail(HAKAI_ERR_STATE, "set_interface before upload_model");
    if (c->hist)
        return fail(HAKAI_ERR_STATE, "set_interface: history output is enabled (its node ownership comes from the "
                    "interface); disable it first");
    if (n_shared < 0 || (n_shared > 0 && (!local_node || !rank_lo || !rank_hi)))
        return fail(HAKAI_ERR_ARG, "set_interface: bad arrays");
    HIPCHK(hipSetDevice(c->device));
    HIPCHK(hipStreamSynchronize(c->stream));
    HIPCHK(hipStreamSynchronize(m->cs));
    free_iface(m);
    std::vector<int> up, dn;
    for (int64_t j = 0; j < n_shared; ++j) {
        if (rank_hi[j] != rank_lo[j] + 1)
            return fail(HAKAI_ERR_ARG, "set_interface: node shared by ranks %d..%d; only adjacent-rank sharing is supported",
                        rank_lo[j], rank_hi[j]);
        if (local_node[j] < 0 || local_node[j] >= c->nN) return fail(HAKAI_ERR_ARG, "set_interface: node out of range");
        if (rank_lo[j] == m->rank) up.push_back((int)local_node[j]);
        else if (rank_hi[j] == m->rank) dn.push_back((int)local_node[j]);
        else return fail(HAKAI_ERR_ARG, "set_interface: node %lld not shared with this rank", (long long)local_node[j]);
    }
    if ((!up.empty() && m->rank + 1 >= m->nranks) || (!dn.empty() && m->rank == 0))
        return fail(HAKAI_ERR_ARG, "set_interface: neighbour rank does not exist");
    std::vector<int> ptr((size_t)c->nN + 1);
    HIPCHK(hipMemcpy(ptr.data(), c->d_inc_ptr, ptr.size() * sizeof(int), hipMemcpyDeviceToHost));
    int nslot = 0;
    for (int n : dn) nslot = std::max(nslot, ptr[n + 1] - ptr[n]);
    if (m->mode == 0) {
        int* d_ns = nullptr;
        HIPCHK(dalloc(&d_ns, 1));
        HIPCHK(hipMemcpy(d_ns, &nslot, sizeof(int), hipMemcpyHostToDevice));
        NCCLCHK(ncclAllReduce(d_ns, d_ns, 1, ncclInt32, ncclMax, m->nc, m->cs));
        HIPCHK(hipStreamSynchronize(m->cs));
        HIPCHK(hipMemcpy(&nslot, d_ns, sizeof(int), hipMemcpyDeviceToHost));
        dfree(d_ns);
// ... 30 lines not shown
```

hakai-fem_amd/csrc/hakai_contact.hip:

```cpp
#include <hip/hip_runtime.h>

#include <algorithm>
#include <climits>
#include <cmath>
#include <cstring>
#include <vector>

#include "hakai_contact_dev.hpp"

using hkc::fail;
using hkc::hip_fail;

#define HIPCHK(x)                                      \
    do {                                               \
        hipError_t _e = (x);                           \
        if (_e != hipSuccess) return hip_fail(_e, #x); \
    } while (0)

namespace {

using namespace hkc::ck;
using hkc::Contact;
using hkc::PairParam;
using hkc::Seg;
// ... 628 lines not shown
        }
        unsigned base = 0;
        if (lane == 63) base = atomicAdd(&ctl[kTerms], (unsigned)x);
        base = __shfl(base, 63);
        if (q < nt) {
            toff[q] = (int)base + x - c;
            tcnt[q] = c;
        }
    }
}

__global__ void k_ct_alloc(unsigned int* ctl, int tsel, const int* touched, const int* cnt, int* toff, int* tcnt) {
    alloc_body(blockIdx.x, gridDim.x, ctl, tsel, touched, cnt, toff, tcnt);
}

__device__ __forceinline__ void scatter_body(int bid, int nb, unsigned int* ctl, const unsigned int* evs,
                                             long long shard_cap, const int* ev_nodes, const double* ev_f,
                                             const int* toff, const int* tpos, int* cnt, double* terms) {
#pragma clang fp contract(off)
    __shared__ unsigned s_pre[kEvShards + 4];
    const long long n = 4 * shard_prefix(bid, ctl, evs, shard_cap, s_pre);
    for (long long e = bid * (long long)blockDim.x + threadIdx.x; e < n; e += (long long)nb * blockDim.x) {
        const long long ev = shard_slot(s_pre, shard_cap, e >> 2);
        const int role = (int)(e & 3);
        const int node = ev_nodes[4 * ev + role];
        const int slot = toff[tpos[node]] + atomicSub(&cnt[node], 1) - 1;
        const double* f = ev_f + 3 * ev;
        double* o = terms + 3 * (long long)slot;
        term_write(o, role, f);
    }
}

__global__ void k_ct_scatter(unsigned int* ctl, const unsigned int* evs, long long shard_cap, const int* ev_nodes,
                             const double* ev_f, const int* toff, const int* tpos, int* cnt, double* terms) {
    scatter_body(blockIdx.x, gridDim.x, ctl, evs, shard_cap, ev_nodes, ev_f, toff, tpos, cnt, terms);
}

__device__ __forceinline__ void sum_body(int bid, int nb, const unsigned int* ctl, int tsel, const int* touched,
                                         const int* toff, const int* tcnt, const double* terms, double* fext,
                                         const int* g2l = nullptr) {
#pragma clang fp contract(off)
    const int nt = (int)ld_ctl(&ctl[kTouched + tsel]);
    for (int q = bid * blockDim.x + threadIdx.x; q < nt; q += nb * blockDim.x) {
        const long long n = g2l ? g2l[touched[q]] : touched[q];
        const int a = toff[q], b = a + tcnt[q];
        for (int c = 0; c < 3; ++c) {
            double s = 0.0, e = 0.0;
            for (int i = a; i < b; ++i) {
                const double x = terms[3 * (long long)i + c];
                const double t = s + x;
                const double bp = t - s;
                const double err = (s - (t - bp)) + (x - bp);
                s = t;
                e += err;
            }
            fext[3 * n + c] = s + e;
        }
    }
}

__global__ void k_ct_sum(unsigned int* ctl, int tsel, const int* touched, const int* toff, const int* tcnt,
                         const double* terms, double* fext, const int* g2l) {
    sum_body(blockIdx.x, gridDim.x, ctl, tsel, touched, toff, tcnt, terms, fext, g2l);
    if (g2l && blockIdx.x == 0 && threadIdx.x == 0) ctl[kTouched + 1 - tsel] = 0;
}

constexpr int kSmallThreads = 1024;

__global__ __launch_bounds__(kSmallThreads) void k_ct_prologue1(
    unsigned long long* bbox, int npairs, unsigned int* ctl, unsigned int* evs, unsigned int* ccnt, const int* del_any,
    int t, const double* t_rd, const int* touched_prev, int tsel, double* fext, const int* del_step, int nE,
    int* dlist, AppendIn A, int* reg, int* ni_live, int* nj_live, int* tri_live, int with_lists) {
    reset_body(0, 1, bbox, npairs, ctl, evs, ccnt, 0, del_any, t, t_rd, touched_prev, tsel, fext);
    if (!with_lists) return;
    __syncthreads();
    find_del_body(0, 1, ctl, del_step, nE, t, t_rd, dlist);
    __syncthreads();
    append_body(0, 1, ctl, dlist, A, del_step, t, t_rd, reg, ni_live, nj_live, tri_live, (int)threadIdx.x,
                (int)blockDim.x);
}

__global__ __launch_bounds__(kSmallThreads) void k_ct_gather1(unsigned int* ctl, const unsigned int* evs,
                                                              long long shard_cap, const int* ev_nodes,
                                                              const double* ev_f, int* cnt, int* touched, int* tpos,
                                                              int tsel, int* poison, int t,
                                                              const double* t_rd, int* toff, int* tcnt,
                                                              double* terms, double* fext) {
    count_body(0, 1, ctl, evs, shard_cap, ev_nodes, cnt, touched, tpos, tsel, poison, t, t_rd);
    __syncthreads();
    alloc_body(0, 1, ctl, tsel, touched, cnt, toff, tcnt);
    __syncthreads();
    scatter_body(0, 1, ctl, evs, shard_cap, ev_nodes, ev_f, toff, tpos, cnt, terms);
    __syncthreads();
    sum_body(0, 1, ctl, tsel, touched, toff, tcnt, terms, fext);
}

__global__ __launch_bounds__(kB) void k_ct_binfilter(StepIn s, const Seg* segs, const int* reg, const int* ni_live,
                                                     const int* ni_pair, const int* ni_node, const PairParam* par,
                                                     const unsigned long long* bbox, const unsigned int* ctl,
                                                     unsigned long long* head, BEnt* blist, BVel* bvel,
                                                     int sb, int nbin, const int* tri_cnt,
                                                     const int* tri_live, const int* tri_pair, const int* tri_nodes,
                                                     const int* tri_ele, unsigned int* ccnt, TriRec* cand,
                                                     long long cshard_cap, uint2* item) {
    if ((int)blockIdx.x < nbin)
        bin_body(blockIdx.x, s, segs, reg, ni_live, ni_pair, ni_node, par, bbox, ctl, head, blist, bvel, sb);
    else
        tri_filter_body(blockIdx.x - nbin, gridDim.x - nbin, s, tri_cnt, tri_live, tri_pair, tri_nodes, tri_ele, par,
                        bbox, ccnt, cand, cshard_cap, item);
}

}

namespace hkc {

void contact_destroy(hakai_ctx* c) {
    Contact* C = c->contact;
    if (!C) return;
    (void)hipStreamSynchronize(c->stream);
    if (C->xr) xr_destroy(C);
    delete C;
    c->contact = nullptr;
    c->d_fext = nullptr;
}

int contact_state_reset(hakai_ctx* c, const double* velo0_host) {
    Contact* C = c->contact;
    if (!C) return 0;
    C->use_velo0 = true;
    C->force_rebuild = true;
    if (velo0_host)
        HIPCHK(hipMemcpyAsync(C->d_velo0, velo0_host, 3 * (size_t)c->nN * sizeof(double), hipMemcpyHostToDevice,
                              c->stream));
    return C->xr ? xr_state_reset(c) : 0;
}

static int search(hakai_ctx* c, const StepIn& in, bool fused);

unsigned filter_grid(const Contact* C) {
    return (unsigned)std::max(1, std::min((C->n_tri + kB - 1) / kB, kFilterBlocks));
}

void tri_prefilter(hakai_ctx* c, const StepIn& in, const unsigned long long* bbox) {
    Contact* C = c->contact;
    hipLaunchKernelGGL(k_ct_tri_filter, dim3(filter_grid(C)), dim3(kB), 0, c->stream, in, C->d_reg + 2 * C->tri_reg + 1,
                       C->d_tri_live, C->d_tri_pair, C->d_tri_nodes, C->d_tri_ele, C->d_par, bbox, C->d_ccnt,
                       C->d_cand, C->cshard_cap, C->small ? nullptr : C->d_item);
}

StepIn step_in(hakai_ctx* c, double t, double d_time) {
    Contact* C = c->contact;
    StepIn in;
    in.coord = c->d_coord;
    in.u = c->d_u[c->cur];
    in.u_pre = c->d_u[1 - c->cur];
    in.flag = c->d_flag;
    in.conn = c->d_conn;
    in.mass = c->d_mass;
    in.l2g = nullptr;
    in.del_step = c->d_del_step;
    in.velo0 = C->use_velo0 ? C->d_velo0 : nullptr;
    in.d_time = d_time;
    in.t = (int)t;
    return in;
}

static AppendIn append_in(const Contact* C) {
    AppendIn A;
    A.el_tri_ptr = C->d_el_tri_ptr; A.el_tri = C->d_el_tri;
    A.el_ni_ptr = C->d_el_ni_ptr; A.el_ni = C->d_el_ni; A.el_nj_ptr = C->d_el_nj_ptr; A.el_nj = C->d_el_nj;
    A.ni_orig = C->d_ni_orig; A.ni_aptr = C->d_ni_aptr; A.ni_add = C->d_ni_add; A.ni_pair = C->d_ni_pair;
    A.nj_orig = C->d_nj_orig; A.nj_aptr = C->d_nj_aptr; A.nj_add = C->d_nj_add; A.nj_pair = C->d_nj_pair;
    A.pair_reg = C->d_pair_reg;
    A.tri_reg = C->tri_reg;
    return A;
}

static LiveIn live_in(const hakai_ctx* c, const int* del_step, int t) {
    const Contact* C = c->contact;
    LiveIn L;
    L.ni_orig = C->d_ni_orig; L.ni_aptr = C->d_ni_aptr; L.ni_add = C->d_ni_add;
    L.nj_orig = C->d_nj_orig; L.nj_aptr = C->d_nj_aptr; L.nj_add = C->d_nj_add;
    L.tri_ele = C->d_tri_ele; L.tri_adder = C->d_tri_adder;
    L.flag = c->d_flag; L.del_step = del_step; L.t = t;
    return L;
}

bool step_begin(Contact* C, int t) {
    if ((long long)t != C->last_t + 1 || C->always_rebuild) C->force_rebuild = true;
    const bool rebuild = C->force_rebuild;
    C->tsel = 1 - C->tsel;
    C->force_rebuild = false;
    C->last_t = t;
    return rebuild;
}

void launch_reset(hakai_ctx* c, unsigned long long* bbox, bool rebuild, const int* del_any, int t, const int* g2l,
                  int* zero_hdr) {
    Contact* C = c->contact;
    hipLaunchKernelGGL(k_ct_reset, dim3(C->g_reset), dim3(kB), 0, c->stream, bbox, C->npairs, C->d_ctl, C->d_evs,
                       C->d_ccnt, rebuild ? 1 : 0, del_any, t, c->g_trd, C->d_touched[1 - C->tsel], C->tsel, c->d_fext,
                       g2l, zero_hdr);
}

void live_rebuild(hakai_ctx* c, const int* del_step, int t) {
    Contact* C = c->contact;
    if (C->ntile == 0) return;
    hipStream_t s = c->stream;
    const LiveIn L = live_in(c, del_step, t);
    const Tile* tl = C->d_tiles;
    const unsigned gt = (unsigned)std::min(C->ntile, 2048);
    hipLaunchKernelGGL(k_ct_live_count, dim3(gt), dim3(kB), 0, s, C->d_ctl, L, tl, C->ntile, C->d_tile_cnt);
    hipLaunchKernelGGL(k_ct_live_scan, dim3(1), dim3(kB), 0, s, C->d_ctl, C->ntile, C->d_tile_cnt, C->d_tile_off,
                       C->nreg, C->d_reg_first, C->d_reg);
    hipLaunchKernelGGL(k_ct_live_write, dim3(gt), dim3(kB), 0, s, C->d_ctl, L, tl, C->ntile, C->d_tile_off,
                       C->d_reg_first, C->d_reg, C->d_ni_live, C->d_nj_live, C->d_tri_live);
}

void live_append(hakai_ctx* c, const int* del_step, int t) {
    Contact* C = c->contact;
    if (C->ntile == 0) return;
    hipLaunchKernelGGL(k_ct_append, dim3(256), dim3(64), 0, c->stream, C->d_ctl, C->d_dlist, append_in(C), del_step, t,
                       c->g_trd, C->d_reg, C->d_ni_live, C->d_nj_live, C->d_tri_live);
}

void launch_boxes(hakai_ctx* c, const StepIn& in, unsigned long long* bbox) {
    Contact* C = c->contact;
    if (C->nseg > 0)
        hipLaunchKernelGGL(k_ct_bbox, dim3(C->nseg * C->g_box), dim3(kB), 0, c->stream, in, C->d_seg, C->d_reg,
                           C->d_ni_live, C->d_nj_live, C->d_ni_node, C->d_nj_node, bbox, C->g_box);
}

void launch_alloc(hakai_ctx* c) {
    Contact* C = c->contact;
    hipLaunchKernelGGL(k_ct_alloc, dim3(C->g_node), dim3(kB), 0, c->stream, C->d_ctl, C->tsel, C->d_touched[C->tsel],
                       C->d_cnt, C->d_toff, C->d_tcnt);
}

void launch_sum(hakai_ctx* c, const int* g2l) {
    Contact* C = c->contact;
    hipLaunchKernelGGL(k_ct_sum, dim3(C->g_node), dim3(kB), 0, c->stream, C->d_ctl, C->tsel, C->d_touched[C->tsel],
                       C->d_toff, C->d_tcnt, C->d_terms, c->d_fext, g2l);
}

static int step_start(hakai_ctx* c, double t, double d_time) {
    Contact* C = c->contact;
    hipStream_t s = c->stream;
    const StepIn in = step_in(c, t, d_time);
    const int* del_step = c->d_del_step;
    const int* del_any = c->d_del_step + c->nEp + 1;
    const bool rebuild = step_begin(C, in.t);
    const bool fused = C->small && C->fuse_small;
    if (fused && !rebuild) {
        hipLaunchKernelGGL(k_ct_prologue1, dim3(1), dim3(kSmallThreads), 0, s, C->d_bbox, C->npairs, C->d_ctl, C->d_evs,
                           C->d_ccnt, del_any, in.t, c->g_trd, C->d_touched[1 - C->tsel], C->tsel, c->d_fext, del_step,
                           (int)C->nE, C->d_dlist, append_in(C), C->d_reg, C->d_ni_live, C->d_nj_live, C->d_tri_live,
                           C->ntile > 0 ? 1 : 0);
    } else {
        launch_reset(c, C->d_bbox, rebuild, del_any, in.t, nullptr, nullptr);
        if (rebuild) live_rebuild(c, del_step, in.t);
        if (C->ntile > 0)
            hipLaunchKernelGGL(k_ct_find_del, dim3(C->g_del), dim3(kB), 0, s, C->d_ctl, del_step, (int)C->nE, in.t,
                               c->g_trd, C->d_dlist);
        live_append(c, del_step, in.t);
    }
    launch_boxes(c, in, C->d_bbox);
    HIPCHK(hipGetLastError());
    return search(c, in, fused);
}

static int search(hakai_ctx* c, const StepIn& in, bool fused) {
    Contact* C = c->contact;
    hipStream_t s = c->stream;
    const int tsel = C->tsel;
    const unsigned gfilt = filter_grid(C);
    const bool fused_mid = (fused || C->fuse_binfilter) && C->nseg > 0 && C->n_tri > 0;
    const Seg* sg = C->d_seg;
    if (C->nseg > 0) {
        if (fused_mid) {
            const int nbin = C->nseg * C->g_seg;
            hipLaunchKernelGGL(k_ct_binfilter, dim3((unsigned)nbin + gfilt), dim3(kB), 0, s, in, sg, C->d_reg,
                               C->d_ni_live, C->d_ni_pair, C->d_ni_node, C->d_par, C->d_bbox, C->d_ctl, C->d_head,
                               C->d_blist, C->d_bvel, C->g_seg, nbin, C->d_reg + 2 * C->tri_reg + 1, C->d_tri_live,
                               C->d_tri_pair, C->d_tri_nodes, C->d_tri_ele, C->d_ccnt, C->d_cand,
                               C->cshard_cap, C->small ? nullptr : C->d_item);
        } else {
            hipLaunchKernelGGL(k_ct_bin, dim3(C->nseg * C->g_seg), dim3(kB), 0, s, in, sg, C->d_reg, C->d_ni_live,
                               C->d_ni_pair, C->d_ni_node, C->d_par, C->d_bbox, C->d_ctl, C->d_head, C->d_blist,
                               C->d_bvel, C->g_seg);
        }
    }
    if (C->n_tri > 0) {
        if (!fused_mid) tri_prefilter(c, in, C->d_bbox);
        tri_search(c, in);
    }
    const unsigned ge = (unsigned)C->g_ev;
    if (fused) {
        hipLaunchKernelGGL(k_ct_gather1, dim3(1), dim3(kSmallThreads), 0, s, C->d_ctl, C->d_evs, C->cap / kEvShards,
                           C->d_ev_nodes, C->d_ev_f, C->d_cnt, C->d_touched[tsel], C->d_tpos, tsel, c->d_poison,
                           in.t, c->g_trd, C->d_toff, C->d_tcnt, C->d_terms, c->d_fext);
        HIPCHK(hipGetLastError());
        C->use_velo0 = false;
        return 0;
    }
    hipLaunchKernelGGL(k_ct_count, dim3(ge), dim3(kB), 0, s, C->d_ctl, C->d_evs, C->cap / kEvShards, C->d_ev_nodes,
                       C->d_cnt, C->d_touched[tsel], C->d_tpos, tsel, c->d_poison, in.t, c->g_trd);
    launch_alloc(c);
    hipLaunchKernelGGL(k_ct_scatter, dim3(ge), dim3(kB), 0, s, C->d_ctl, C->d_evs, C->cap / kEvShards, C->d_ev_nodes,
// ... 389 lines not shown
```

hakai-fem_amd/csrc/hakai_internal.hpp:

```cpp
#pragma once
#include <hip/hip_runtime.h>

#include <string>
#include <vector>

#include "../../include/hakai_hip.h"
#include "hakai_device.hpp"

namespace hkc {
struct Comm;
struct Contact;
struct History;
int fail(int code, const char* fmt, ...);
int hip_fail(hipError_t e, const char* what);
}

struct EventPair {
    hipEvent_t a, b;
    int kernel;
};


constexpr long long kFuseBcMaxNodes = 1 << 18;

struct hakai_ctx {
    int device = 0;
    hipStream_t stream = nullptr;
    long long nN = 0, nE = 0, nEp = 0, ld = 0;
    double* d_coord = nullptr;
    double* d_u[2] = {nullptr, nullptr};
    int cur = 0;
    double* d_mass = nullptr;
    int* d_conn = nullptr;
    int* d_flag = nullptr;
    int* d_mat = nullptr;
    hk::DevMat* d_mats = nullptr;
    std::vector<hk::DevMat> h_mats;
    bool has_ductile = false;
    double* d_stress = nullptr;
    double* d_strain = nullptr;
    double* d_eqps = nullptr;
    double* d_yield = nullptr;
    double* d_triax = nullptr;
    double* d_fe = nullptr;
    int* d_inc_ptr = nullptr;
    int* d_inc = nullptr;
    int* d_inc_row = nullptr;
    int* d_inc8 = nullptr;
    long long fe_len = 0;
    int max_inc = 0;
    std::vector<int> h_ptr, h_inc0;
    int pipe_blocks = 512;
    int pipe_min = 2;
    int gp_nt = 1;
    int elem_exact = 0;
    int group_serial = 0;
    double* d_pusai = nullptr;
    int nmat = 0;
    long long elem_offset = 0;
    int nbc = 0;
    int* d_bc_dof = nullptr;
    int* d_bc_grp = nullptr;
    double* d_bc_val = nullptr;
    int* d_amp_n = nullptr;
    int* d_amp_off = nullptr;
    double* d_amp_t = nullptr;
    double* d_amp_v = nullptr;
    int* d_bc_of_node = nullptr;
    int fuse_bc = 1;
    double* d_qbuf = nullptr;
    bool q_from_buf = false;
    bool fe_ok = true, triax_ok = true;
    std::vector<double> h_velo0;
    long long steps_done = 0;
    double last_dt = 0.0;
    int* d_del_step = nullptr;
    unsigned long long* d_negjac = nullptr;
    int* d_poison = nullptr;
    long long poison_step = -1;
    long long exchange_retries = 0;
    bool any_plastic = false;
    bool model_ok = false;
    bool state_ok = false;
    std::vector<double> h_coord;
    std::vector<int> h_conn;
    std::vector<int> h_mat;
    std::vector<double> h_young;
    double* d_fext = nullptr;
    hkc::Contact* contact = nullptr;
    bool prof = false;
    uint32_t prof_mask = 0;
    std::vector<hipEvent_t> ev_pool;
    std::vector<EventPair> ev_pending;
    double k_ms[HAKAI_K_COUNT] = {0, 0, 0, 0};
    long long k_n[HAKAI_K_COUNT] = {0, 0, 0, 0};
    double* d_tstep = nullptr;
    const double* g_trd = nullptr;
    hipGraphExec_t g_exec[2][2] = {{nullptr, nullptr}, {nullptr, nullptr}};
    double g_dt[2][2] = {{0.0, 0.0}, {0.0, 0.0}};
    long long g_epoch[2][2] = {{-1, -1}, {-1, -1}};
    int g_len[2][2] = {{0, 0}, {0, 0}};
    long long epoch = 0;
    long long tdev_next = -1;
    int graph = 16;
    long long graph_steps = 0;
    int own_assembly = 1;
    long long own_built_g = -1;
    long long own_for_g0 = -1;
    int own_band_rows = 0;
    int own_pass_batches = 0;
    bool own_valid = false;
    int* d_own_off = nullptr;
    int* d_own_seq = nullptr;
    int* d_own_bstart = nullptr;
    int own_banded = 0;
    long long own_round2 = 0;
    int* d_own_list = nullptr;
    int own_nop = 0;
    int own_slots = 0;
    double* d_own_q = nullptr;
    int* d_own_rp = nullptr;
    double* d_own_rows = nullptr;
    int* d_own_ridx = nullptr;
    double* d_own_dump = nullptr;
    long long own_rows = 0, own_entries = 0;
    long long own_steps = 0;
    int own_s = 2;
    hkc::Comm* comm = nullptr;
    hkc::History* hist = nullptr;
    int hist_one_block = -1;
};


namespace hkc {
void prof_begin(hakai_ctx* c, int kernel, EventPair* p);
void prof_end(hakai_ctx* c, EventPair* p);
void comm_destroy(hakai_ctx* c);
int comm_reset(hakai_ctx* c);
void comm_pending_get(const hakai_ctx* c, bool* pending, int* par);
void comm_rollback(hakai_ctx* c, bool had_good, long long last_good, bool pending, int par);
int comm_pre_nodal(hakai_ctx* c);
struct CommFix {
    bool ran = false;
    int n_up = 0, nslot = 0;
    const double* up_sendP = nullptr;
    const double* up_recvC = nullptr;
};
int comm_post_nodal(hakai_ctx* c, double d_time, CommFix* fix = nullptr);
int comm_post_element(hakai_ctx* c, long long step);
bool comm_is_local(const hakai_ctx* c);
const std::vector<int>* comm_dn_nodes(const hakai_ctx* c);
const std::vector<int>* comm_up_nodes(const hakai_ctx* c);
bool comm_iface_set(const hakai_ctx* c);
int comm_rank(const hakai_ctx* c);
int comm_size(const hakai_ctx* c);
constexpr int kMaxLocalGather = 64;
struct LocalGather {
    const char* src[kMaxLocalGather];
    long long bytes[kMaxLocalGather];
    long long off[kMaxLocalGather];
};
int gather_local(hakai_ctx* c, const LocalGather& g, int n, void* dst);
int comm_allgather_raw(hakai_ctx* c, const void* send, void* recv, size_t bytes);
int comm_allgatherv_raw(hakai_ctx* c, const void* send, void* recv, const size_t* bytes, const size_t* off);
int comm_allreduce_min_u64(hakai_ctx* c, const void* send, void* recv, size_t count);
bool comm_is_rccl(const hakai_ctx* c);
hakai_ctx* comm_peer_ctx(hakai_ctx* c, int q);
void contact_destroy(hakai_ctx* c);
int contact_state_reset(hakai_ctx* c, const double* velo0_host);
int contact_step(hakai_ctx* c, double t, double d_time);
int contact_phase(hakai_ctx* c, int part, double t, double d_time);
int contact_step_b(hakai_ctx* c);
bool contact_multi(const hakai_ctx* c);
int contact_post_step(hakai_ctx* c);
int contact_check(hakai_ctx* c);
void contact_after_overflow(hakai_ctx* c, long long steps_since_reset);
bool contact_exchange_retry(hakai_ctx* c);
void graph_invalidate(hakai_ctx* c);
bool contact_graph_ok(const hakai_ctx* c, double t);
void contact_graph_advance(hakai_ctx* c, double t_last);
int contact_tuning(hakai_ctx* c, const char* key, long long value);
}
```

hakai-fem_amd/csrc/hakai_kernels.hip:

```cpp
#include <hip/hip_runtime.h>

#include <algorithm>
#include <type_traits>

#include "hakai_exact_math.hpp"
#include "hakai_kernels.hpp"

namespace hk {

constexpr int kBlock = 256;
constexpr int kEPB = kBlock / 8;
constexpr int kLdsStride = 50;
constexpr int kFeStride = 25;
__device__ __forceinline__ int fe_at(int l, int c) { return (l >> 3) * kFeStride + 3 * (l & 7) + c; }
constexpr int kPusStride = 26;

__device__ __forceinline__ int ref_of_sign(int s) {
    constexpr unsigned kTab = 0u | 4u << 3 | 3u << 6 | 7u << 9 | 1u << 12 | 5u << 15 | 2u << 18 | 6u << 21;
    return (int)((kTab >> (3 * s)) & 7u);
}

__device__ constexpr double kSx[8] = {-1., 1., 1., -1., -1., 1., 1., -1.};
__device__ constexpr double kSy[8] = {-1., -1., 1., 1., -1., -1., 1., 1.};
__device__ constexpr double kSz[8] = {-1., -1., -1., -1., 1., 1., 1., 1.};
// ... 537 lines not shown
            const double dep = (q - ys) / (3.0 * M->G + H);
            const double s = ys + H * dep;
            const double rq = 1.0 / q;
#pragma unroll
            for (int r = 0; r < 3; ++r) fin[r] = div_cr(dev[r] * s, q, rq) + mean;
#pragma unroll
            for (int r = 3; r < 6; ++r) fin[r] = div_cr(dev[r] * s, q, rq) + 0.0;
            eqp = eqp + dep;
            ys = ys + H * dep;
        }
    }
    auto triax = [&]() {
        const double mean = div3(fin[0] + fin[1] + fin[2]);
        const double a01 = fin[0] - fin[1], a12 = fin[1] - fin[2], a20 = fin[2] - fin[0];
        const double oeq = sqrt(0.5 * (a01 * a01 + a12 * a12 + a20 * a20) +
                                3.0 * (fin[3] * fin[3] + fin[4] * fin[4] + fin[5] * fin[5]));
        return (oeq < 1e-10) ? 0.0 : mean / oeq;
    };
    double eps[6];
#pragma unroll
    for (int c = 0; c < 6; ++c) eps[c] = active ? in.eps[c] + de[c] : in.eps[c];
#pragma unroll
    for (int c = 0; c < 6; ++c) fin[c] = active ? fin[c] : in.sig[c];
    if (!active) {
        eqp = in.eqp;
        ys = in.ys;
    }

    HK_PH(pc, 5);
    double tri = STORE_TRIAX ? triax() : 0.0;
    bool kill = false;
    if (DO_DELETE && nd > 0 && __builtin_amdgcn_ballot_w64(eqp >= M->du_skip) != 0) {
        const double v_e = gp_all8(xb, k, eqp) * 0.125;
        if (v_e >= M->du_floor) {
            if (!STORE_TRIAX) tri = triax();
            const double t_e = gp_all8(xb, k, tri) * 0.125;
            if (!(t_e < 0.0)) kill = active && v_e >= ductile_fr(M->du_eps, M->du_tri, nd, t_e);
        }
    }

    if (WITH_VOL) a.vol[e] = V;
    {
        const double nofk[3] = {0.0, 0.0, 0.0};
        elem_writeback<DO_DELETE, STORE_TRIAX, ANY_PLASTIC, NT, true, OWN, true, kWbState>(a, e, k, in, active, kill,
                                                                                          nofk, fin, eps, eqp, ys, tri);
    }
    double fk[3];
    {
        double w[8];
#pragma unroll
        for (int i = 0; i < 8; ++i) {
            const double t0 = tq(i, 0);
            double acc = (pd[i][0] + t0) * fin[0];
            acc = __builtin_fma(t0, fin[1], acc);
            acc = __builtin_fma(t0, fin[2], acc);
            acc = __builtin_fma(pd[i][1], fin[3], acc);
            acc = __builtin_fma(pd[i][2], fin[5], acc);
            w[i] = v * acc;
        }
        fk[0] = gp_sum8(xb, k, w);
#pragma unroll
        for (int i = 0; i < 8; ++i) {
            const double t1 = tq(i, 1);
            double acc = t1 * fin[0];
            acc = __builtin_fma(pd[i][1] + t1, fin[1], acc);
            acc = __builtin_fma(t1, fin[2], acc);
            acc = __builtin_fma(pd[i][0], fin[3], acc);
            acc = __builtin_fma(pd[i][2], fin[4], acc);
            w[i] = v * acc;
        }
        fk[1] = gp_sum8(xb, k, w);
#pragma unroll
        for (int i = 0; i < 8; ++i) {
            const double t2 = tq(i, 2);
            double acc = t2 * fin[0];
            acc = __builtin_fma(t2, fin[1], acc);
            acc = __builtin_fma(pd[i][2] + t2, fin[2], acc);
            acc = __builtin_fma(pd[i][1], fin[4], acc);
            acc = __builtin_fma(pd[i][0], fin[5], acc);
            w[i] = v * acc;
        }
        fk[2] = gp_sum8(xb, k, w);
    }
    HK_PH(pc, 6);
    elem_writeback<DO_DELETE, STORE_TRIAX, ANY_PLASTIC, NT, true, OWN, true, kWbForce>(a, e, k, in, active, kill, fk,
                                                                                      fin, eps, eqp, ys, tri, sfe);
    HK_PH(pc, 7);
}

__device__ __forceinline__ void stage_pusai(const ElemArgs& a, double* s_pus) {
    for (int w = threadIdx.x; w < 192; w += blockDim.x) s_pus[w / 24 * kPusStride + w % 24] = a.pusai[w];
}

__device__ __forceinline__ bool poisoned(const int* p) { return p && *p; }

__device__ __forceinline__ void graph_step(ElemArgs& a) {
    if (a.t_rd) {
        const double tp = *a.t_rd;
        a.step_i = (int)tp + 1;
        if (a.t_wr && blockIdx.x == 0 && threadIdx.x == 0) *a.t_wr = tp + 1.0;
    }
}

template <bool DO_DELETE, bool STORE_TRIAX, bool WITH_VOL, bool EXACT>
__global__ __launch_bounds__(kBlock, 2) void k_element(ElemArgs a) {
    __shared__ __attribute__((aligned(16))) double s_nd[kEPB * kLdsStride];
    __shared__ __attribute__((aligned(16))) double s_xb[EXACT ? kEPB * kXbStride : 1];
    __shared__ __attribute__((aligned(16))) double s_pus[EXACT ? 8 * kPusStride : 1];
    const long long vb = xcd_remap(blockIdx.x, gridDim.x);
    if (poisoned(a.poison)) return;
    graph_step(a);
    const int k = threadIdx.x & 7;
    const int grp = threadIdx.x >> 3;
    if (EXACT) {
        stage_pusai(a, s_pus);
        __syncthreads();
    }
    const long long e = vb * kEPB + grp;
    ElemIn in;
    load_stage_a<EXACT>(a, e, k, in);
    if (EXACT) {
        load_node_raw(a, in);
        load_gp<true>(a, e, k, in);
    } else {
        load_stage_b<true>(a, e, k, in);
    }
#ifdef HK_DIAG_PHASE
    PhaseClock pc;
#endif
    if (EXACT)
        elem_step_exact<DO_DELETE, STORE_TRIAX, true, WITH_VOL>(a, a.mats, e, k, s_nd + grp * kLdsStride,
                                                                s_xb + grp * kXbStride, s_pus, in, nullptr HK_PH_PASS);
    else
        elem_step<DO_DELETE, STORE_TRIAX, true, WITH_VOL>(a, a.mats, e, k, s_nd + grp * kLdsStride, in);
}


__device__ __forceinline__ void lds_barrier() {
    __builtin_amdgcn_fence(__ATOMIC_RELEASE, "workgroup", "local");
    __builtin_amdgcn_s_barrier();
    __builtin_amdgcn_fence(__ATOMIC_ACQUIRE, "workgroup", "local");
}

__device__ __forceinline__ int4 own_load(const ElemArgs& a, long long b) {
    const int o0 = a.own_off[b], o1 = a.own_off[b + 1];
    const int idx = o0 + (int)threadIdx.x;
    int4 en = a.own_list[idx < o1 ? idx : a.own_nop];
    en.y |= (o1 - o0 > kBlock) ? kOwnRound2 : 0;
    return en;
}

__device__ __forceinline__ int own_lane(int4 en, int j) { return own_lane(en.y, en.z, en.w, j); }

__device__ __forceinline__ void own_entry(const ElemArgs& a, int4 en, const double* s_fe, double* s_part) {
#pragma clang fp contract(off)
    const int slot = own_slot(en.y), flags = own_flags(en.y), n = own_n(en.y);
    double* dump = a.own_dump + 8 * (long long)blockIdx.x;
    double v[3];
    if (flags & (kOwnExp | kOwnNop)) {
#pragma unroll
        for (int j = 0; j < kOwnExpRows; ++j) {
            const int l = own_lane(en, j);
            double* dst = ((flags & kOwnExp) && j < n) ? a.own_rows + 3 * ((long long)en.x + (long long)j * slot) : dump;
#pragma unroll
            for (int c = 0; c < 3; ++c) dst[c] = s_fe[fe_at(l, c)];
        }
        return;
    }
#pragma unroll
    for (int c = 0; c < 3; ++c) v[c] = (flags & kOwnInit) ? 0.0 : s_part[3 * slot + c];
    for (int j = 0; j < n; ++j) {
        const int l = own_lane(en, j);
#pragma unroll
        for (int c = 0; c < 3; ++c) v[c] += s_fe[fe_at(l, c)];
    }
    if (!(flags & kOwnFin)) {
#pragma unroll
        for (int c = 0; c < 3; ++c) s_part[3 * slot + c] = v[c];
    }
    double* dst = (flags & kOwnFin) ? a.own_q + 3 * (long long)en.x : dump;
#pragma unroll
    for (int c = 0; c < 3; ++c) dst[c] = v[c];
}

#ifdef HK_DIAG_WAVE
constexpr int kDiagWaves = 8192, kDiagWords = 8;
__device__ unsigned long long g_diag[kDiagWaves * kDiagWords];
struct PassClock {
    long long bar = 0, pass = 0, n = 0;
};
#define HK_DIAG_ARG , PassClock& dg
#define HK_DIAG_PASS , dg
#else
#define HK_DIAG_ARG
#define HK_DIAG_PASS
#endif

__device__ __forceinline__ void own_pass(const ElemArgs& a, int4 en, long long sb, const double* s_fe,
                                         double* s_part HK_DIAG_ARG) {
#ifdef HK_DIAG_WAVE
    const long long t0 = clock64();
#endif
    lds_barrier();
#ifdef HK_DIAG_WAVE
    const long long t1 = clock64();
#endif
    const int o0 = a.own_off[sb], o1 = a.own_off[sb + 1];
    if (o0 + (int)(threadIdx.x & ~63u) < o1) own_entry(a, en, s_fe, s_part);
    if (en.y & kOwnRound2) {
        const int idx = o0 + kBlock + (int)threadIdx.x;
        if (o0 + kBlock + (int)(threadIdx.x & ~63u) < o1)
            own_entry(a, a.own_list[idx < o1 ? idx : a.own_nop], s_fe, s_part);
    }
#ifdef HK_DIAG_WAVE
    const long long t2 = clock64();
    dg.bar += t1 - t0;
    dg.pass += t2 - t1;
    dg.n += 1;
#endif
}

template <bool DO_DELETE, bool STORE_TRIAX, bool ANY_PLASTIC, bool LDS_MATS, int NT, bool EXACT, int OS = 0>
__global__ __launch_bounds__(kBlock, 2) void k_element_pipe(ElemArgs a) {
    constexpr bool OWN = OS > 0;
    constexpr int kOwnFe = OS * kEPB * kFeStride;
    __shared__ __attribute__((aligned(16))) double s_nd[kEPB * kLdsStride];
    __shared__ __attribute__((aligned(16))) double s_fe[OWN ? 2 * kOwnFe : 1];
    extern __shared__ __attribute__((aligned(16))) double s_dyn[];
    double* s_part = s_dyn;
    DevMat* s_mats = reinterpret_cast<DevMat*>(s_dyn + (OWN ? 3 * a.own_slots : 0));
    __shared__ __attribute__((aligned(16))) double s_xb[EXACT ? kEPB * kXbStride : 1];
    __shared__ __attribute__((aligned(16))) double s_pus[EXACT ? 8 * kPusStride : 1];
    if (poisoned(a.poison)) return;
    graph_step(a);
    const int k = threadIdx.x & 7;
    const int grp = threadIdx.x >> 3;
    if (LDS_MATS) {
        const int words = a.nmat * (int)(sizeof(DevMat) / sizeof(double));
        const double* src = reinterpret_cast<const double*>(a.mats);
        double* dst = reinterpret_cast<double*>(s_mats);
        for (int w = threadIdx.x; w < words; w += kBlock) dst[w] = src[w];
    }
    if (EXACT) stage_pusai(a, s_pus);
    if (LDS_MATS || EXACT) __syncthreads();
    const DevMat* mats = LDS_MATS ? s_mats : a.mats;
    double* nd8 = s_nd + grp * kLdsStride;
    double* xb = s_xb + (EXACT ? grp * kXbStride : 0);
    const long long nb = a.nEp / kEPB;
    long long first, stride, count;
    if (OWN) {
        first = a.own_bstart[blockIdx.x];
        stride = 1;
        count = a.own_bstart[blockIdx.x + 1] - first;
    } else if (gridDim.x % 8 != 0) {
        first = (long long)blockIdx.x * nb / gridDim.x;
        stride = 1;
        count = ((long long)blockIdx.x + 1) * nb / gridDim.x - first;
    } else {
        const long long x = blockIdx.x & 7, j = blockIdx.x >> 3, per = gridDim.x >> 3;
        const long long r0 = x * nb / 8, r1 = (x + 1) * nb / 8;
        first = r0 + j;
        stride = per;
        count = first < r1 ? (r1 - first + per - 1) / per : 0;
    }
    if (count <= 0) return;
    auto pos_of = [&](long long i) { return first + (i < count ? i : count - 1) * stride; };
    auto vb_of = [&](long long i) { return OWN ? (long long)a.own_seq[pos_of(i)] : pos_of(i); };
    auto elem_of = [&](long long i) { return vb_of(i) * kEPB + grp; };

#ifdef HK_DIAG_WAVE
    PassClock dg;
    const long long dg_t0 = clock64();
#endif
#ifdef HK_DIAG_PHASE
    PhaseClock pc;
#endif
    ElemIn cur, nxt;
    int4 ent_cur = {0, 0, 0, 0}, ent_nxt = {0, 0, 0, 0};
    load_stage_a<EXACT>(a, elem_of(0), k, cur);
    load_stage_a<EXACT>(a, elem_of(1), k, nxt);
    if (!EXACT) load_stage_b<ANY_PLASTIC, NT>(a, elem_of(0), k, cur);
    constexpr int S = OS > 0 ? OS : 1;
    auto sb_of = [&](long long i) { return pos_of((i < count ? i : count - 1) / S * S); };
    if (OWN) ent_cur = own_load(a, sb_of(0));
    for (long long i = 0; i < count; ++i) {
        ElemIn nn;
        load_stage_a<EXACT>(a, elem_of(i + 2), k, nn);
        if (!EXACT) load_stage_b<ANY_PLASTIC, NT>(a, elem_of(i + 1), k, nxt);
        if (OWN) ent_nxt = own_load(a, sb_of(i + 1));
        double* sfe = s_fe + ((i / S) & 1) * kOwnFe + (i % S) * (kEPB * kFeStride);
        if (EXACT) {
#ifdef HK_DIAG_PHASE
            pc.last = clock64();
#endif
            load_node_raw(a, cur);
            load_gp<ANY_PLASTIC, NT>(a, elem_of(i), k, cur);
            HK_PH(pc, 0);
            elem_step_exact<DO_DELETE, STORE_TRIAX, ANY_PLASTIC, false, NT, OWN>(a, mats, elem_of(i), k, nd8, xb, s_pus,
                                                                                 cur, sfe HK_PH_PASS);
        }
        else
            elem_step<DO_DELETE, STORE_TRIAX, ANY_PLASTIC, false, NT, OWN>(a, mats, elem_of(i), k, nd8, cur, sfe);
        if (OWN) {
            if ((i + 1) % S == 0 || i + 1 == count)
                own_pass(a, ent_cur, sb_of(i), s_fe + ((i / S) & 1) * kOwnFe, s_part HK_DIAG_PASS);
            ent_cur = ent_nxt;
        }
        cur = nxt;
        nxt = nn;
    }
#ifdef HK_DIAG_WAVE
    const long long dg_t1 = clock64();
    const unsigned gw = blockIdx.x * (kBlock / 64) + threadIdx.x / 64;
    if ((threadIdx.x & 63) == 0 && gw < (unsigned)kDiagWaves) {
        unsigned long long* d = g_diag + (size_t)kDiagWords * gw;
        atomicAdd(d + 0, (unsigned long long)(dg_t1 - dg_t0));
        atomicAdd(d + 1, (unsigned long long)dg.bar);
        atomicAdd(d + 2, (unsigned long long)dg.pass);
        atomicAdd(d + 3, (unsigned long long)dg.n);
        atomicAdd(d + 4, (unsigned long long)count);
        atomicAdd(d + 5, 1ull);
        atomicExch(d + 6, (unsigned long long)__builtin_amdgcn_s_getreg((31 << 11) | 4));
#ifdef HK_DIAG_PHASE
        unsigned long long* q = g_diag + (size_t)kDiagWords * (kDiagWaves / 2 + gw);
        for (int j = 0; j < 8; ++j) atomicAdd(q + j, (unsigned long long)pc.t[j]);
#endif
    }
#endif
}

#ifdef HK_DIAG_WAVE
extern "C" int hk_diag_reset() {
    void* p = nullptr;
    if (hipGetSymbolAddress(&p, HIP_SYMBOL(g_diag)) != hipSuccess) return -1;
    return hipMemset(p, 0, sizeof(g_diag)) == hipSuccess ? 0 : -1;
}
extern "C" int hk_diag_read(unsigned long long* out, int n) {
    if (hipDeviceSynchronize() != hipSuccess) return -1;
    return hipMemcpyFromSymbol(out, HIP_SYMBOL(g_diag), sizeof(unsigned long long) * (size_t)std::min(n, kDiagWaves * kDiagWords)) == hipSuccess ? 0 : -1;
}
#endif

template <bool EXACT>
static void launch_element_w(const ElemArgs& a, bool do_delete, bool store_triax, bool with_vol, unsigned grid,
                             hipStream_t s) {
    if (with_vol) {
        hipLaunchKernelGGL((k_element<false, false, true, EXACT>), dim3(grid), dim3(kBlock), 0, s, a);
    } else if (do_delete) {
        if (store_triax)
            hipLaunchKernelGGL((k_element<true, true, false, EXACT>), dim3(grid), dim3(kBlock), 0, s, a);
        else
            hipLaunchKernelGGL((k_element<true, false, false, EXACT>), dim3(grid), dim3(kBlock), 0, s, a);
    } else {
        if (store_triax)
            hipLaunchKernelGGL((k_element<false, true, false, EXACT>), dim3(grid), dim3(kBlock), 0, s, a);
        else
            hipLaunchKernelGGL((k_element<false, false, false, EXACT>), dim3(grid), dim3(kBlock), 0, s, a);
    }
}

template <bool ANY_PLASTIC, bool LDS_MATS, int NT, bool EXACT, int OS>
static void launch_pipe(const ElemArgs& a, bool do_delete, bool store_triax, unsigned grid, hipStream_t s) {
    const size_t dyn = (OS > 0 ? 24 * (size_t)a.own_slots : 0) + (LDS_MATS ? sizeof(DevMat) * (size_t)a.nmat : 0);
    if (do_delete) {
        if (store_triax)
            hipLaunchKernelGGL((k_element_pipe<true, true, ANY_PLASTIC, LDS_MATS, NT, EXACT, OS>), dim3(grid),
                               dim3(kBlock), dyn, s, a);
        else
            hipLaunchKernelGGL((k_element_pipe<true, false, ANY_PLASTIC, LDS_MATS, NT, EXACT, OS>), dim3(grid),
                               dim3(kBlock), dyn, s, a);
    } else {
        if (store_triax)
            hipLaunchKernelGGL((k_element_pipe<false, true, ANY_PLASTIC, LDS_MATS, NT, EXACT, OS>), dim3(grid),
                               dim3(kBlock), dyn, s, a);
        else
            hipLaunchKernelGGL((k_element_pipe<false, false, ANY_PLASTIC, LDS_MATS, NT, EXACT, OS>), dim3(grid),
                               dim3(kBlock), dyn, s, a);
    }
}

template <bool ANY_PLASTIC, bool LDS_MATS, bool EXACT, int OS>
static void launch_pipe_nt(const ElemArgs& a, bool do_delete, bool store_triax, unsigned grid, hipStream_t s) {
    if (a.gp_nt)
        launch_pipe<ANY_PLASTIC, LDS_MATS, 3, EXACT, OS>(a, do_delete, store_triax, grid, s);
    else
        launch_pipe<ANY_PLASTIC, LDS_MATS, 0, EXACT, OS>(a, do_delete, store_triax, grid, s);
}

template <bool ANY_PLASTIC, bool LDS_MATS, bool EXACT>
static void launch_pipe_os(const ElemArgs& a, bool do_delete, bool store_triax, unsigned grid, hipStream_t s) {
    if (a.own == 1)
        launch_pipe_nt<ANY_PLASTIC, true, EXACT, 1>(a, do_delete, store_triax, grid, s);
    else if (a.own == 2)
        launch_pipe_nt<ANY_PLASTIC, true, EXACT, 2>(a, do_delete, store_triax, grid, s);
    else
        launch_pipe_nt<ANY_PLASTIC, LDS_MATS, EXACT, 0>(a, do_delete, store_triax, grid, s);
}

template <bool EXACT>
static void launch_pipe_p(const ElemArgs& a, bool do_delete, bool store_triax, unsigned grid, hipStream_t s) {
    const bool lds = a.nmat <= kMaxLdsMats;
    if (a.any_plastic) {
        if (lds) launch_pipe_os<true, true, EXACT>(a, do_delete, store_triax, grid, s);
        else launch_pipe_os<true, false, EXACT>(a, do_delete, store_triax, grid, s);
    } else {
        if (lds) launch_pipe_os<false, true, EXACT>(a, do_delete, store_triax, grid, s);
        else launch_pipe_os<false, false, EXACT>(a, do_delete, store_triax, grid, s);
    }
}

hipError_t launch_element(const ElemArgs& a, bool do_delete, bool store_triax, hipStream_t s) {
    if (a.nE <= 0) return hipSuccess;
    if (a.exact && !a.pusai) return hipErrorInvalidValue;
    const long long nb = a.nEp / kEPB;
    if (nb <= 0) return hipSuccess;
    if (a.own) {
        if (a.own > 2 || a.vol || a.pipe_blocks <= 0 || a.nmat > kMaxLdsMats || !a.own_off || !a.own_list ||
            !a.own_seq || !a.own_bstart || !a.own_q || !a.own_dump || a.own_slots < 1 ||
            a.own_slots > own_slot_cap(a.exact != 0, a.own, a.nmat))
            return hipErrorInvalidValue;
        if (a.own_grid <= 0 || a.own_grid > nb) return hipErrorInvalidValue;
        if (a.exact)
            launch_pipe_p<true>(a, do_delete, store_triax, (unsigned)a.own_grid, s);
        else
            launch_pipe_p<false>(a, do_delete, store_triax, (unsigned)a.own_grid, s);
        return hipGetLastError();
    }
    if (a.pipe_blocks > 0 && !a.vol) {
        const unsigned grid = (unsigned)std::min<long long>(nb, a.pipe_blocks);
        if (a.exact)
            launch_pipe_p<true>(a, do_delete, store_triax, grid, s);
        else
            launch_pipe_p<false>(a, do_delete, store_triax, grid, s);
        return hipGetLastError();
    }
    if (a.exact)
        launch_element_w<true>(a, do_delete, store_triax, a.vol != nullptr, (unsigned)nb, s);
    else
        launch_element_w<false>(a, do_delete, store_triax, a.vol != nullptr, (unsigned)nb, s);
    return hipGetLastError();
}

__global__ void k_negjac(ElemArgs a, unsigned long long* count) {
    const long long t = (long long)blockIdx.x * blockDim.x + threadIdx.x;
    if (t >= 8 * a.nE) return;
    const long long e = t >> 3;
    const int k = t & 7;
    if (a.flag[e] != 1) return;
    const double g = 1.0 / __builtin_sqrt(3.0);
    const double gz = (k & 4) ? g : -g, et = (k & 2) ? g : -g, tu = (k & 1) ? g : -g;
    double J[3][3] = {{0., 0., 0.}, {0., 0., 0.}, {0., 0., 0.}};
    for (int i = 0; i < 8; ++i) {
        const long long n = a.conn[8 * e + i];
        const double p0 = 0.125 * kSx[i] * (1.0 + et * kSy[i]) * (1.0 + tu * kSz[i]);
        const double p1 = 0.125 * kSy[i] * (1.0 + gz * kSx[i]) * (1.0 + tu * kSz[i]);
        const double p2 = 0.125 * kSz[i] * (1.0 + gz * kSx[i]) * (1.0 + et * kSy[i]);
        for (int c = 0; c < 3; ++c) {
            const double X = a.coord[3 * n + c] + a.u[3 * n + c];
            J[0][c] += p0 * X;
            J[1][c] += p1 * X;
            J[2][c] += p2 * X;
        }
    }
    const double det = J[0][0] * (J[1][1] * J[2][2] - J[1][2] * J[2][1]) +
                       J[0][1] * (J[1][2] * J[2][0] - J[1][0] * J[2][2]) +
                       J[0][2] * (J[1][0] * J[2][1] - J[1][1] * J[2][0]);
    if (det < 0.0) atomicAdd(count, 1ull);
}

hipError_t launch_negjac(const ElemArgs& a, unsigned long long* count, hipStream_t s) {
    if (a.nE <= 0) return hipSuccess;
    hipLaunchKernelGGL(k_negjac, dim3((unsigned)((8 * a.nE + 255) / 256)), dim3(256), 0, s, a, count);
    return hipGetLastError();
}

__device__ __forceinline__ double bc_value(const BCArgs& a, int i) {
#pragma clang fp contract(off)
    const int g = a.grp[i];
    const double ct = a.t_rd ? (*a.t_rd + 1.0) * a.dt : a.ct;
    double amp = 1.0;
    const int na = a.amp_n[g];
    if (na > 0) {
        const double* at = a.amp_t + a.amp_off[g];
        const double* av = a.amp_v + a.amp_off[g];
        int ti = 0;
        for (int j = 0; j < na - 1; ++j)
            if (ct >= at[j] && ct <= at[j + 1]) {
                ti = j;
                break;
            }
        amp = av[ti] + (av[ti + 1] - av[ti]) * (ct - at[ti]) / (at[ti + 1] - at[ti]);
    }
    return a.val[i] * amp;
}

struct NodeIn {
    double m, uc[3], up[3], f[3];
};

template <bool FEXT>
__device__ __forceinline__ void nodal_load(const NodalArgs& a, long long n, NodeIn& in) {
    in.m = a.mass[n];
#pragma unroll
    for (int c = 0; c < 3; ++c) {
        in.uc[c] = a.u[3 * n + c];
        in.up[c] = a.u_pre_out[3 * n + c];
        in.f[c] = FEXT ? a.fext[3 * n + c] : 0.0;
    }
}

template <bool BCF>
__device__ __forceinline__ void nodal_update(const NodalArgs& a, long long n, const NodeIn& in, double Q0, double Q1,
                                             double Q2) {
#pragma clang fp contract(off)
    const double m = in.m;
    const double dt = a.dt;
    const double dC = 0.0 * m;
    const double mdt2 = m / (dt * dt);
    const double inv = 1.0 / (mdt2 + dC / 2.0 / dt);
    const double Q[3] = {Q0, Q1, Q2};
    const int b0 = BCF ? a.bc_of_node[n] : -1;
#pragma unroll
    for (int c = 0; c < 3; ++c) {
        const double up = in.up[c];
        double v = inv * (in.f[c] - Q[c] + mdt2 * (2.0 * in.uc[c] - up) + dC / 2.0 / dt * up);
        if (BCF) {
            const long long dc = 3 * n + c;
            for (int j = b0; j >= 0 && j < a.bc.n && a.bc.dof[j] <= dc; ++j)
                if (a.bc.dof[j] == dc) v = bc_value(a.bc, j);
        }
        a.u_pre_out[3 * n + c] = v;
    }
}

template <int MODE, bool FEXT, bool BCF>
__global__ __launch_bounds__(kBlock) void k_nodal(NodalArgs a) {
#pragma clang fp contract(off)
    if (poisoned(a.poison)) return;
    const unsigned lb = xcd_remap_rev(blockIdx.x, gridDim.x);
    const long long n = (long long)lb * kBlock + threadIdx.x;
    if (n >= a.nN) return;
    NodeIn in;
    nodal_load<FEXT>(a, n, in);
    double Q0 = 0.0, Q1 = 0.0, Q2 = 0.0;
    if (MODE == 2) {
        Q0 = a.qbuf[3 * n + 0];
        Q1 = a.qbuf[3 * n + 1];
        Q2 = a.qbuf[3 * n + 2];
    } else if (MODE == 3) {
        Q0 = a.own_q[3 * n + 0];
        Q1 = a.own_q[3 * n + 1];
        Q2 = a.own_q[3 * n + 2];
        const int j0 = a.own_rp[n], j1 = a.own_rp[n + 1];
        for (int j = j0; j < j1; ++j) {
            const long long r = a.own_ridx[j];
            Q0 += a.own_rows[3 * r + 0];
            Q1 += a.own_rows[3 * r + 1];
            Q2 += a.own_rows[3 * r + 2];
        }
    } else if (MODE == 0) {
        const int4 lo = reinterpret_cast<const int4*>(a.inc8)[2 * n];
        const int4 hi = reinterpret_cast<const int4*>(a.inc8)[2 * n + 1];
        const int idx[8] = {lo.x, lo.y, lo.z, lo.w, hi.x, hi.y, hi.z, hi.w};
        double f[8][3];
#pragma unroll
        for (int j = 0; j < 8; ++j) {
            const double* p = a.fe + idx[j];
            f[j][0] = p[0];
            f[j][1] = p[1];
            f[j][2] = p[2];
        }
#pragma unroll
        for (int j = 0; j < 8; ++j) {
            Q0 += f[j][0];
            Q1 += f[j][1];
            Q2 += f[j][2];
        }
    } else {
        const int j0 = a.inc_ptr[n], j1 = a.inc_ptr[n + 1];
        for (int j = j0; j < j1; ++j) {
            const double* f = a.fe + a.inc[j];
            Q0 += f[0];
            Q1 += f[1];
            Q2 += f[2];
        }
    }
    nodal_update<BCF>(a, n, in, Q0, Q1, Q2);
}

template <bool FEXT, bool BCF>
static void launch_nodal_m(const NodalArgs& a, unsigned grid, hipStream_t s) {
    if (a.qbuf)
        hipLaunchKernelGGL((k_nodal<2, FEXT, BCF>), dim3(grid), dim3(kBlock), 0, s, a);
    else if (a.own_q)
        hipLaunchKernelGGL((k_nodal<3, FEXT, BCF>), dim3(grid), dim3(kBlock), 0, s, a);
    else if (a.inc8)
        hipLaunchKernelGGL((k_nodal<0, FEXT, BCF>), dim3(grid), dim3(kBlock), 0, s, a);
    else
        hipLaunchKernelGGL((k_nodal<1, FEXT, BCF>), dim3(grid), dim3(kBlock), 0, s, a);
}

hipError_t launch_nodal(const NodalArgs& a, hipStream_t s) {
    if (a.nN <= 0) return hipSuccess;
    const unsigned grid = (unsigned)((a.nN + kBlock - 1) / kBlock);
    if (a.bc_of_node) {
        if (a.fext)
            launch_nodal_m<true, true>(a, grid, s);
        else
            launch_nodal_m<false, true>(a, grid, s);
    } else {
        if (a.fext)
            launch_nodal_m<true, false>(a, grid, s);
        else
            launch_nodal_m<false, false>(a, grid, s);
    }
    return hipGetLastError();
}

__global__ __launch_bounds__(kBlock) void k_bc(BCArgs a) {
    if (poisoned(a.poison)) return;
    const int i = blockIdx.x * kBlock + threadIdx.x;
    if (i >= a.n) return;
    a.out[a.dof[i]] = bc_value(a, i);
}

hipError_t launch_bc(const BCArgs& a, hipStream_t s) {
    if (a.n <= 0) return hipSuccess;
    hipLaunchKernelGGL(k_bc, dim3((a.n + kBlock - 1) / kBlock), dim3(kBlock), 0, s, a);
    return hipGetLastError();
}

__global__ void k_set_step(double* slot, double t_prev) {
    if (threadIdx.x == 0) *slot = t_prev;
}

__global__ void k_hold(int rounds) {
    for (int i = 0; i < rounds; ++i) __builtin_amdgcn_s_sleep(127);
}

hipError_t launch_hold(int rounds, hipStream_t s) {
    hipLaunchKernelGGL(k_hold, dim3(1), dim3(64), 0, s, rounds);
    return hipGetLastError();
}

hipError_t launch_set_step(double* slot, double t_prev, hipStream_t s) {
    hipLaunchKernelGGL(k_set_step, dim3(1), dim3(64), 0, s, slot, t_prev);
    return hipGetLastError();
}

__global__ void k_gather_q(const int* __restrict__ ptr, const int* __restrict__ inc, const double* __restrict__ fe,
                           double* Q, long long nN) {
#pragma clang fp contract(off)
    const long long n = (long long)blockIdx.x * blockDim.x + threadIdx.x;
    if (n >= nN) return;
    double q0 = 0.0, q1 = 0.0, q2 = 0.0;
    for (int j = ptr[n]; j < ptr[n + 1]; ++j) {
        const double* f = fe + inc[j];
        q0 += f[0];
        q1 += f[1];
        q2 += f[2];
    }
    Q[3 * n + 0] = q0;
    Q[3 * n + 1] = q1;
    Q[3 * n + 2] = q2;
}

hipError_t launch_gather_q(const int* inc_ptr, const int* inc, const double* fe, double* Q, long long nN,
                           hipStream_t s) {
    if (nN <= 0) return hipSuccess;
    hipLaunchKernelGGL(k_gather_q, dim3((unsigned)((nN + 255) / 256)), dim3(256), 0, s, inc_ptr, inc, fe, Q, nN);
    return hipGetLastError();
}

__global__ void k_own_q(const double* __restrict__ own_q, const int* __restrict__ rp, const int* __restrict__ ridx,
                        const double* __restrict__ rows, double* Q, long long nN) {
#pragma clang fp contract(off)
    const long long n = (long long)blockIdx.x * blockDim.x + threadIdx.x;
    if (n >= nN) return;
    double q0 = own_q[3 * n + 0], q1 = own_q[3 * n + 1], q2 = own_q[3 * n + 2];
    for (int j = rp[n]; j < rp[n + 1]; ++j) {
        const long long r = ridx[j];
        q0 += rows[3 * r + 0];
        q1 += rows[3 * r + 1];
        q2 += rows[3 * r + 2];
    }
    Q[3 * n + 0] = q0;
    Q[3 * n + 1] = q1;
    Q[3 * n + 2] = q2;
}

hipError_t launch_own_q(const double* own_q, const int* rp, const int* ridx, const double* rows, double* Q,
                        long long nN, hipStream_t s) {
    if (nN <= 0) return hipSuccess;
    hipLaunchKernelGGL(k_own_q, dim3((unsigned)((nN + 255) / 256)), dim3(256), 0, s, own_q, rp, ridx, rows, Q, nN);
    return hipGetLastError();
}

__global__ void k_aos_to_soa6(const double* __restrict__ aos, double* __restrict__ soa, long long n, long long ld) {
    const long long i = (long long)blockIdx.x * blockDim.x + threadIdx.x;
    if (i >= 6 * n) return;
    const long long g = i / 6, c = i % 6;
    soa[c * ld + g] = aos[i];
}
__global__ void k_soa_to_aos6(const double* __restrict__ soa, double* __restrict__ aos, long long n, long long ld) {
    const long long i = (long long)blockIdx.x * blockDim.x + threadIdx.x;
    if (i >= 6 * n) return;
    const long long g = i / 6, c = i % 6;
    aos[i] = soa[c * ld + g];
}

hipError_t launch_aos_to_soa6(const double* aos, double* soa, long long nGP, long long ld, hipStream_t s) {
    if (nGP <= 0) return hipSuccess;
    hipLaunchKernelGGL(k_aos_to_soa6, dim3((unsigned)((6 * nGP + 255) / 256)), dim3(256), 0, s, aos, soa, nGP, ld);
    return hipGetLastError();
}
hipError_t launch_soa_to_aos6(const double* soa, double* aos, long long nGP, long long ld, hipStream_t s) {
    if (nGP <= 0) return hipSuccess;
    hipLaunchKernelGGL(k_soa_to_aos6, dim3((unsigned)((6 * nGP + 255) / 256)), dim3(256), 0, s, soa, aos, nGP, ld);
    return hipGetLastError();
}

__global__ void k_reset_gp(double* stress, double* strain, double* eqps, double* yield, double* triax, int* flag,
                           const int* mat, const DevMat* mats, long long nE, long long nEp, long long ld) {
    const long long g = (long long)blockIdx.x * blockDim.x + threadIdx.x;
    if (g >= 8 * nEp) return;
    const long long e = g >> 3;
#pragma unroll
    for (int c = 0; c < 6; ++c) {
        stress[c * ld + g] = 0.0;
        strain[c * ld + g] = 0.0;
    }
    eqps[g] = 0.0;
    triax[g] = 0.0;
    const DevMat* M = mats + mat[e];
    yield[g] = (e < nE && M->npp > 0) ? M->yield0 : 0.0;
    if ((g & 7) == 0) flag[e] = e < nE ? 1 : 0;
}

hipError_t launch_reset_gp(double* stress, double* strain, double* eqps, double* yield, double* triax, int* flag,
                           const int* mat, const DevMat* mats, long long nE, long long nEp, long long ld, hipStream_t s) {
    if (nEp <= 0) return hipSuccess;
    hipLaunchKernelGGL(k_reset_gp, dim3((unsigned)((8 * nEp + 255) / 256)), dim3(256), 0, s, stress, strain, eqps,
                       yield, triax, flag, mat, mats, nE, nEp, ld);
    return hipGetLastError();
}

__global__ void k_triax_aos(const double* __restrict__ st, double* __restrict__ tx, long long n) {
    const long long i = (long long)blockIdx.x * blockDim.x + threadIdx.x;
    if (i >= n) return;
    const double* s = st + 6 * i;
    const double mean = (s[0] + s[1] + s[2]) / 3.0;
    const double a01 = s[0] - s[1], a12 = s[1] - s[2], a20 = s[2] - s[0];
    const double oeq = sqrt(0.5 * (a01 * a01 + a12 * a12 + a20 * a20) + 3.0 * (s[3] * s[3] + s[4] * s[4] + s[5] * s[5]));
    tx[i] = (oeq < 1e-10) ? 0.0 : mean / oeq;
}

// ... 66 lines not shown
```

hakai-fem_amd/csrc/hakai_kernels.hpp:

```cpp
#pragma once
#include <hip/hip_runtime.h>
#include <stdint.h>

#include "hakai_device.hpp"
#include "hakai_own_entry.hpp"

namespace hk {

struct ElemArgs {
    const double* coord;
    const double* u;
    const double* u_pre;
    const int* conn;
    int* flag;
    const int* mat;
    const DevMat* mats;
    double* stress;
    double* strain;
    double* sc[6];
    double* ec[6];
    double* eqps;
    double* yield;
    double* triax;
    double* fe;
    double* vol;
    long long nE;
    long long nEp;
    long long ld;
    int* del_step;
    int step_i;
    const double* t_rd;
    double* t_wr;
    int any_plastic;
    int pipe_blocks;
    int nmat;
    int gp_nt;
    int exact;
    const double* pusai;
    const int* poison;
    int own;
    int own_grid;
    const int* own_seq;
    const int* own_bstart;
    const int* own_off;
    const int4* own_list;
    int own_nop;
    int own_slots;
    double* own_q;
    double* own_rows;
    double* own_dump;
};

struct BCArgs {
    const int* dof;
    const int* grp;
    const double* val;
    int n;
    const int* amp_n;
    const int* amp_off;
    const double* amp_t;
    const double* amp_v;
    double* out;
    double ct;
    const double* t_rd;
    double dt;
    const int* poison;
};

struct NodalArgs {
    const double* u;
    double* u_pre_out;
    const double* mass;
    const int* inc_ptr;
    const int* inc;
    const int* inc8;
    const double* fe;
    const double* qbuf;
    const double* fext;
    long long nN;
    double dt;
    const int* bc_of_node;
    BCArgs bc;
    const int* poison;
    const double* own_q;
    const int* own_rp;
    const int* own_ridx;
    const double* own_rows;
};


inline int own_slot_cap(bool exact, int batches_per_pass, int nmat) {
    const int stat = 12800 + 6400 * batches_per_pass * 2 + (exact ? 20608 : 0) + 64;
    const int left = 81920 - 256 - stat - nmat * (int)sizeof(DevMat);
    return left < 24 ? 0 : (left / 24 > kOwnSlotsMax ? kOwnSlotsMax : left / 24);
}

hipError_t launch_element(const ElemArgs& a, bool do_delete, bool store_triax, hipStream_t s);
hipError_t launch_negjac(const ElemArgs& a, unsigned long long* count, hipStream_t s);
hipError_t launch_nodal(const NodalArgs& a, hipStream_t s);
hipError_t launch_bc(const BCArgs& a, hipStream_t s);
hipError_t launch_set_step(double* slot, double t_prev, hipStream_t s);
hipError_t launch_hold(int rounds, hipStream_t s);

hipError_t launch_gather_q(const int* inc_ptr, const int* inc, const double* fe, double* Q, long long nN,
                           hipStream_t s);
hipError_t launch_own_q(const double* own_q, const int* rp, const int* ridx, const double* rows, double* Q,
                        long long nN, hipStream_t s);
hipError_t launch_aos_to_soa6(const double* aos, double* soa, long long nGP, long long ld, hipStream_t s);
hipError_t launch_soa_to_aos6(const double* soa, double* aos, long long nGP, long long ld, hipStream_t s);
hipError_t launch_reset_gp(double* stress, double* strain, double* eqps, double* yield, double* triax, int* flag,
                           const int* mat, const DevMat* mats, long long nE, long long nEp, long long ld, hipStream_t s);
hipError_t launch_triax_aos(const double* stress_aos, double* triax, long long nGP, hipStream_t s);
hipError_t launch_node_average(const int* inc_ptr, const int* inc, const double* stress, const double* strain,
                               const double* eqps, const double* triax, long long ld, long long nN,
                               double* node_stress, double* node_strain, double* node_eqps, double* node_mises,
                               double* node_triax, hipStream_t s);

}
```

hakai-fem_amd/csrc/hakai_own_entry.hpp:

```cpp
#pragma once

#if defined(__HIPCC__) || defined(__CUDACC__)
#define HK_HD __host__ __device__ __forceinline__
#else
#define HK_HD static inline
#endif

namespace hk {

enum { kOwnInit = 1, kOwnFin = 2, kOwnExp = 4, kOwnNop = 8 };
constexpr int kOwnExpRows = 4;
constexpr int kOwnSlotsMax = 2048;
constexpr int kOwnRound2 = 1 << 27;

HK_HD constexpr int own_pack_y(int slot, int flags, int n, int lane7) {
    return (int)(((unsigned)slot & 1023u) | (unsigned)flags << 10 | (unsigned)n << 14 | (unsigned)lane7 << 18 |
                 ((unsigned)slot & 1024u) << 18);
}
static_assert((own_pack_y(kOwnSlotsMax - 1, 15, 15, 511) & kOwnRound2) == 0, "kOwnRound2 overlaps a packed field");

HK_HD void own_pack(int target, int slot, int flags, int n, const int lanes[8], int w[4]) {
    unsigned long long lo = 0;
    for (int q = 0; q < 7; ++q) lo |= (unsigned long long)lanes[q] << (9 * q);
    w[0] = target;
    w[1] = own_pack_y(slot, flags, n, lanes[7]);
    w[2] = (int)(unsigned)(lo & 0xffffffffu);
    w[3] = (int)(unsigned)(lo >> 32);
}

HK_HD int own_slot(int y) { return (y & 1023) | ((y >> 18) & 1024); }
HK_HD int own_flags(int y) { return (y >> 10) & 15; }
HK_HD int own_n(int y) { return (y >> 14) & 15; }
HK_HD int own_lane(int y, int z, int w, int j) {
    const unsigned long long lo = (unsigned long long)(unsigned)z | ((unsigned long long)(unsigned)w << 32);
    return j < 7 ? (int)((lo >> (9 * j)) & 511) : (int)(((unsigned)y >> 18) & 511);
}

}
```

hakai-fem_amd/csrc/hakai_own_plan.cpp:

```cpp
#include "hakai_own_plan.hpp"

#include <algorithm>
#include <cmath>
#include <utility>

#include "hakai_own_entry.hpp"

namespace hk {

static OwnSched own_contiguous(long long nb, long long G, int epb) {
    OwnSched sc;
    sc.epb = epb;
    sc.seq.resize(nb);
    for (long long b = 0; b < nb; ++b) sc.seq[b] = (int)b;
    sc.bstart.resize(G + 1);
    for (long long lb = 0; lb <= G; ++lb) sc.bstart[lb] = lb * nb / G;
    return sc;
}

static bool lattice_strides(const OwnInput& in, std::vector<int>& nx, std::vector<int>& L) {
    const long long nE = in.nE;
    nx.assign(nE, -1);
    L.assign(nE, -1);
    long long found = 0;
    for (long long e = 0; e < nE; ++e) {
        for (int k = 0; k < 8; ++k) {
            const int n = in.conn[8 * e + k];
            const int j0 = in.ptr[n];
            if (in.ptr[n + 1] - j0 != 8 || in.inc0[j0] / 8 != e) continue;
            long long q[8];
            for (int i = 0; i < 8; ++i) q[i] = in.inc0[j0 + i] / 8 - e;
            const long long a = q[2], l = q[4];
            if (q[1] == 1 && a > 1 && q[3] == a + 1 && l > a + 1 && q[5] == l + 1 && q[6] == l + a &&
                q[7] == l + a + 1 && l % a == 0 && l < (1LL << 30)) {
                nx[e] = (int)a;
                L[e] = (int)l;
                ++found;
                break;
            }
        }
    }
    if (found * 2 < nE) return false;
    long long first = -1;
    for (long long e = 0; e < nE; ++e)
        if (nx[e] > 0) {
            first = e;
            break;
        }
    for (long long e = 0; e < nE; ++e) {
        if (nx[e] > 0) continue;
        const long long src = e < first ? first : e - 1;
        nx[e] = nx[src];
        L[e] = L[src];
    }
    return true;
}

static bool own_banded(const OwnInput& in, long long G, const std::vector<int>& nx, const std::vector<int>& L,
                       int shrink, int epb, int slot_cap, OwnSched& sc) {
    const long long nb = in.nEp / epb, nE = in.nE;
    sc.epb = epb;
    std::vector<long long> rstart{0};
    for (long long x = 1; x < nE; ++x)
        if (nx[x] != nx[x - 1] || L[x] != L[x - 1]) rstart.push_back(x);
    rstart.push_back(nE);
    std::vector<long long> Rreg(rstart.size() - 1);
    for (size_t r = 0; r + 1 < rstart.size(); ++r) {
        const long long e0 = rstart[r], ne = rstart[r + 1] - e0;
        const long long rows = L[e0] / nx[e0], layers = std::max<long long>(1, ne / L[e0]);
        const double Gr = std::max(1.0, (double)G * (double)ne / (double)nE);
        const long long Rcap = (slot_cap - slot_cap / 16) / (nx[e0] + 1) - 1;
        const long long Ropt = (long long)std::llround(std::sqrt(1.5 * (double)layers * (double)rows / Gr));
        const long long Rwant = in.band_rows > 0 ? (long long)in.band_rows : std::max<long long>(Ropt, 1);
        Rreg[r] = std::max<long long>(1, std::min(Rcap, Rwant) - shrink);
    }
    std::vector<long long> key(nb);
    bool any_split = false;
    size_t region = 0;
    for (long long b = 0; b < nb; ++b) {
        const long long e = std::min(epb * b, nE - 1);
        while (e >= rstart[region + 1]) ++region;
        const long long rows = L[e] / nx[e];
        long long R = Rreg[region];
        if (R >= rows) R = rows;
        else any_split = true;
        const long long row = ((e - rstart[region]) % L[e]) / nx[e];
        key[b] = ((long long)region << 32) | (row / R);
    }
    if (!any_split) return false;
    std::vector<int> order(nb);
    for (long long b = 0; b < nb; ++b) order[b] = (int)b;
    std::stable_sort(order.begin(), order.end(), [&](int x, int y) { return key[x] < key[y]; });
    std::vector<std::pair<long long, long long>> bands;
    for (long long p = 0; p < nb;) {
        long long q = p;
        while (q < nb && key[order[q]] == key[order[p]]) ++q;
        bands.emplace_back(p, q);
        p = q;
    }
    const long long nbands = (long long)bands.size();
    if (nbands > G) return false;
    std::vector<long long> runs(nbands);
    std::vector<std::pair<double, long long>> rem;
    long long used = 0;
    for (long long i = 0; i < nbands; ++i) {
        const long long m = bands[i].second - bands[i].first;
        const double want = (double)G * (double)m / (double)nb;
        runs[i] = std::max<long long>(1, std::min<long long>(m, (long long)want));
        used += runs[i];
        rem.emplace_back(want - (double)runs[i], i);
    }
    std::sort(rem.begin(), rem.end(), [](const std::pair<double, long long>& x, const std::pair<double, long long>& y) {
        return x.first > y.first || (x.first == y.first && x.second < y.second);
    });
    for (size_t r = 0; used < G && r < rem.size(); ++r) {
        const long long i = rem[r].second;
        if (runs[i] < bands[i].second - bands[i].first) {
            ++runs[i];
            ++used;
        }
    }
    for (long long i = 0; used > G && i < nbands; ++i)
        while (runs[i] > 1 && used > G) {
            --runs[i];
            --used;
        }
    sc.seq = order;
    sc.bstart.assign(1, 0);
    for (long long i = 0; i < nbands; ++i) {
        const long long p = bands[i].first, m = bands[i].second - p;
        for (long long r = 1; r <= runs[i]; ++r) sc.bstart.push_back(p + r * m / runs[i]);
    }
    sc.banded = true;
    return true;
}

static bool own_plan(const OwnInput& in, const OwnSched& sc, int S, int slot_cap, OwnPlan& pl) {
    const int epb = sc.epb, bs = 8 * epb;
    const long long nb = in.nEp / epb, nN = in.nN;
    const long long G = (long long)sc.bstart.size() - 1;
    if (G <= 0 || in.max_inc > 8 || in.ptr.size() != (size_t)nN + 1) return false;
    pl.S = S;
    struct Ent { int target, slot, flags, n; int lanes[8]; int inc[4]; };
    std::vector<int> pos_of(nb), block_of(nb);
    std::vector<long long> sb_pos(nb);
    for (long long lb = 0; lb < G; ++lb)
        for (long long p = sc.bstart[lb]; p < sc.bstart[lb + 1]; ++p) {
            const int b = sc.seq[p];
            if (p > sc.bstart[lb] && b <= sc.seq[p - 1]) return false;
            pos_of[b] = (int)p;
            block_of[b] = (int)lb;
            sb_pos[b] = sc.bstart[lb] + (p - sc.bstart[lb]) / S * S;
        }
    std::vector<std::vector<Ent>> per(nb);
    std::vector<int> rp(nN + 1, 0);
    long long rows = 0;
    struct Seg { long long s0, s1; std::vector<std::pair<long long, int>> refs; };
    std::vector<std::vector<Seg>> segs(G);
    auto batch_of = [&](int j) { return (long long)(in.inc0[j] / 8) / epb; };
    auto lane_of = [&](int j) {
        const long long e = in.inc0[j] / 8;
        const long long b = e / epb;
        return (int)(((pos_of[b] - sb_pos[b]) * epb + e % epb) * 8 + in.inc0[j] % 8);
    };
    std::vector<std::pair<long long, int>> exports;
    std::vector<char> all_rows(nN, 0);
    if (const std::vector<int>* dn = in.all_rows)
        for (int n : *dn) all_rows[n] = 1;
    for (long long n = 0; n < nN; ++n) {
        const int j0 = in.ptr[n], j1 = in.ptr[n + 1];
        if (j0 == j1) continue;
        if (all_rows[n]) {
            for (int j = j0; j < j1; ++j) exports.emplace_back(sb_pos[batch_of(j)], j);
            continue;
        }
        const int hb = block_of[batch_of(j0)];
        int j = j0;
        Seg sg;
        sg.s0 = -1;
        while (j < j1 && block_of[batch_of(j)] == hb) {
            const long long sb = sb_pos[batch_of(j)];
            Ent en{(int)n, 0, 0, 0, {0, 0, 0, 0, 0, 0, 0, 0}, {0, 0, 0, 0}};
            while (j < j1 && sb_pos[batch_of(j)] == sb) {
                if (en.n == 8) return false;
                en.lanes[en.n++] = lane_of(j);
                ++j;
            }
            if (sg.s0 < 0) {
                sg.s0 = sb;
                en.flags |= kOwnInit;
            }
            sg.s1 = sb;
            per[sb].push_back(en);
            sg.refs.emplace_back(sb, (int)per[sb].size() - 1);
        }
        per[sg.s1][sg.refs.back().second].flags |= kOwnFin;
        if (sg.s1 > sg.s0) segs[hb].push_back(std::move(sg));
        for (; j < j1; ++j) exports.emplace_back(sb_pos[batch_of(j)], j);
    }
    std::stable_sort(exports.begin(), exports.end(),
                     [](const std::pair<long long, int>& x, const std::pair<long long, int>& y) { return x.first < y.first; });
    std::vector<int> row_of_inc(in.inc0.size(), -1);
    for (size_t q = 0; q < exports.size();) {
        const long long sb = exports[q].first;
        Ent en{0, 0, kOwnExp, 0, {0, 0, 0, 0, 0, 0, 0, 0}, {0, 0, 0, 0}};
        while (q < exports.size() && exports[q].first == sb && en.n < kOwnExpRows) {
            const int j = exports[q].second;
            en.inc[en.n] = j;
            en.lanes[en.n++] = lane_of(j);
            ++q;
        }
        per[sb].push_back(en);
    }
    for (long long b = 0; b < nb; ++b) {
        std::vector<Ent>& v = per[b];
        for (size_t p = 0; p < v.size();) {
            if (!(v[p].flags & kOwnExp)) {
                ++p;
                continue;
            }
            size_t p1 = p;
            while (p1 < v.size() && (v[p1].flags & kOwnExp) && p1 / 64 == p / 64) ++p1;
            const int g = (int)(p1 - p);
            std::vector<std::pair<int, int>> cs;
            for (size_t i = p; i < p1; ++i)
                for (int k = 0; k < v[i].n; ++k) cs.emplace_back(v[i].inc[k], v[i].lanes[k]);
            const int m = (int)cs.size();
            for (int i = 0; i < g; ++i) {
                Ent& en = v[p + (size_t)i];
                en.target = (int)(rows + i);
                en.slot = g;
                en.n = 0;
                for (int q = i; q < m; q += g) {
                    en.inc[en.n] = cs[(size_t)q].first;
                    en.lanes[en.n++] = cs[(size_t)q].second;
                    row_of_inc[cs[(size_t)q].first] = (int)(rows + q);
                }
            }
            rows += m;
            p = p1;
        }
    }
    std::vector<int>& ridx = pl.ridx;
    ridx.clear();
    ridx.reserve(exports.size());
    for (long long n = 0; n < nN; ++n) {
        rp[n] = (int)ridx.size();
        for (int j = in.ptr[n]; j < in.ptr[n + 1]; ++j)
            if (row_of_inc[j] >= 0) ridx.push_back(row_of_inc[j]);
    }
    rp[nN] = (int)ridx.size();
    if (rows > (1LL << 31) - 1) return false;
    int max_slots = 1;
    for (long long lb = 0; lb < G; ++lb) {
        auto& v = segs[lb];
        std::sort(v.begin(), v.end(), [](const Seg& x, const Seg& y) { return x.s0 < y.s0; });
        std::vector<std::pair<long long, int>> busy;
        std::vector<int> free_slots;
        int next = 0;
        auto cmp = [](const std::pair<long long, int>& x, const std::pair<long long, int>& y) { return x.first > y.first; };
        for (auto& sg : v) {
            while (!busy.empty() && busy.front().first < sg.s0) {
                free_slots.push_back(busy.front().second);
                std::pop_heap(busy.begin(), busy.end(), cmp);
                busy.pop_back();
            }
            int slot;
            if (!free_slots.empty()) {
                slot = free_slots.back();
                free_slots.pop_back();
            } else {
                slot = next++;
            }
            if (slot >= slot_cap) return false;
            max_slots = std::max(max_slots, slot + 1);
            for (auto& r : sg.refs) per[r.first][r.second].slot = slot;
            busy.emplace_back(sg.s1, slot);
            std::push_heap(busy.begin(), busy.end(), cmp);
        }
    }
    std::vector<int>& off = pl.off;
    off.assign(nb + 1, 0);
    for (long long b = 0; b < nb; ++b) {
        if (per[b].size() > 2 * (size_t)bs) return false;
        pl.round2 += per[b].size() > (size_t)bs ? 1 : 0;
        off[b + 1] = off[b] + (int)per[b].size();
    }
    const long long ne = off[nb];
    std::vector<int>& list = pl.list;
    list.assign(4 * (size_t)(ne + 1), 0);
    for (long long b = 0; b < nb; ++b)
        for (size_t i = 0; i < per[b].size(); ++i) {
            const Ent& en = per[b][i];
            own_pack(en.target, en.slot, en.flags, en.n, en.lanes, &list[4 * ((size_t)off[b] + i)]);
        }
    const int no_lanes[8] = {0, 0, 0, 0, 0, 0, 0, 0};
    own_pack(0, 0, kOwnNop, 0, no_lanes, &list[4 * (size_t)ne]);
    pl.rp = std::move(rp);
    pl.rows = rows;
    pl.ne = ne;
    pl.max_slots = max_slots;
    return true;
}

bool own_choose(const OwnInput& in, long long G0, OwnSched& best_sc, OwnPlan& best, int only) {
    const int epb = 32;
    const long long nb = in.nEp / epb;
    auto cap_of = [&](int S) { return in.slot_cap[S - 1]; };
    const int cap = cap_of(2);
    bool have = false;
    auto consider = [&](const OwnSched& sc) {
        for (int S : {2, 1}) {
            if (in.pass_batches > 0 && S != in.pass_batches) continue;
            OwnPlan pl;
            if (!own_plan(in, sc, S, cap_of(S), pl)) continue;
            if (!have || pl.cost() < best.cost()) {
                best = std::move(pl);
                best_sc = sc;
                have = true;
            }
            return true;
        }
        return false;
    };
    if (only != 2) consider(own_contiguous(nb, G0, epb));
    if (only != 1) {
        std::vector<int> nx, L;
        if (lattice_strides(in, nx, L)) {
            OwnSched sc;
            for (int shrink : {0, 1, 2, 4})
                if (own_banded(in, G0, nx, L, shrink, epb, cap, sc) && consider(sc)) break;
        }
    }
    if (!have && only != 2 && 8 * G0 <= nb) consider(own_contiguous(nb, 8 * G0, epb));
    return have;
}

}
```

hakai-fem_amd/csrc/hakai_own_plan.hpp:

```cpp
#pragma once
#include <vector>

namespace hk {

struct OwnSched {
    int epb = 32;
    std::vector<int> seq;
    std::vector<long long> bstart;
    bool banded = false;
};

struct OwnPlan {
    int S = 2;
    std::vector<int> off, list, rp, ridx;
    long long rows = 0, ne = 0;
    int max_slots = 1;
    long long round2 = 0;
    double cost() const { return 16.0 * (double)ne + 52.0 * (double)rows; }
};

struct OwnInput {
    long long nE, nN, nEp;
    const std::vector<int>& conn;
    const std::vector<int>& ptr;
    const std::vector<int>& inc0;
    int max_inc;
    int band_rows;
    int pass_batches;
    const std::vector<int>* all_rows;
    int slot_cap[2];
};

bool own_choose(const OwnInput& in, long long G0, OwnSched& best_sc, OwnPlan& best, int only = 0);

}
```

Baseline: 2587.

## Fold nodal displacement update into element kernel via triple-buffered displacements

Adds an optional fold mode in which the element kernel, when it finalizes a node's owned force sum, immediately computes that node's next displacement using precomputed per-node coefficients. It writes the result into a third displacement buffer. Only the remnant nodes not finalized inside the element kernel are updated by a smaller list-driven nodal kernel. This is meant to remove most of the separate nodal pass and its re-reading of forces and displacements. The cost is a third displacement buffer, a rotation scheme with more state, extra graph variants, and restrictions to configurations without contact, comm, history, or exact mode. It is gated by the own_fold flag, which defaults from an environment variable.

```diff
diff --git a/hakai-fem_amd/csrc/hakai_capi.cpp b/hakai-fem_amd/csrc/hakai_capi.cpp
--- a/hakai-fem_amd/csrc/hakai_capi.cpp
+++ b/hakai-fem_amd/csrc/hakai_capi.cpp
@@ -74,9 +74,12 @@
     dfree(c->d_own_rows);
     dfree(c->d_own_ridx);
     dfree(c->d_own_dump);
+    dfree(c->d_own_rem);
+    c->own_rem_n = 0;
     c->own_built_g = -1;
     c->own_for_g0 = -1;
     c->own_valid = false;
+    c->fold_valid = false;
 }
 
 static void free_model(hakai_ctx* c) {
@@ -84,6 +87,9 @@
     dfree(c->d_coord);
     dfree(c->d_u[0]);
     dfree(c->d_u[1]);
+    dfree(c->d_u[2]);
+    dfree(c->d_fold_coef);
+    c->fold_coef_dt = 0.0;
     dfree(c->d_mass);
     dfree(c->d_conn);
     dfree(c->d_flag);
@@ -226,7 +232,7 @@
 }
 static void graph_free(hakai_ctx* c) {
     for (int g = 0; g < 2; ++g)
-        for (int p = 0; p < 2; ++p)
+        for (int p = 0; p < 6; ++p)
             if (c->g_exec[g][p]) {
                 (void)hipGraphExecDestroy(c->g_exec[g][p]);
                 c->g_exec[g][p] = nullptr;
@@ -240,8 +246,8 @@
     hk::ElemArgs ea;
     std::memset(&ea, 0, sizeof ea);
     ea.coord = c->d_coord;
-    ea.u = c->d_u[c->cur];
-    ea.u_pre = c->d_u[1 - c->cur];
+    ea.u = hkc::disp(c);
+    ea.u_pre = hkc::disp_pre(c);
     ea.conn = c->d_conn;
     ea.flag = c->d_flag;
     ea.mat = c->d_mat;
@@ -365,6 +371,7 @@
     }
     if (const char* v = std::getenv("HAKAI_ELEM_EXACT")) c->elem_exact = std::atoi(v) ? 1 : 0;
     if (const char* v = std::getenv("HAKAI_OWN_ASSEMBLY")) c->own_assembly = std::atoi(v) ? 1 : 0;
+    if (const char* v = std::getenv("HAKAI_OWN_FOLD")) c->own_fold = std::atoi(v) ? 1 : 0;
     *out = c;
     return 0;
 }
@@ -459,6 +466,7 @@
     HIPCHK(dalloc(&c->d_coord, 3 * (size_t)nN));
     HIPCHK(dalloc(&c->d_u[0], 3 * (size_t)nN));
     HIPCHK(dalloc(&c->d_u[1], 3 * (size_t)nN));
+    HIPCHK(dalloc(&c->d_u[2], 3 * (size_t)nN));
     HIPCHK(dalloc(&c->d_mass, (size_t)nN));
     HIPCHK(dalloc(&c->d_conn, 8 * (size_t)nEp));
     HIPCHK(dalloc(&c->d_flag, (size_t)nEp));
@@ -571,15 +579,15 @@
 
 int hakai_reset_state(hakai_ctx* c, int64_t n_ic, const int64_t* ic_dofs, const double* ic_values, double d_time) {
     if (c) hkc::graph_invalidate(c);
-    if (c) c->own_valid = false;
+    if (c) c->own_valid = c->fold_valid = false;
     if (!c) return fail(HAKAI_ERR_ARG, "null");
     if (!c->model_ok) return fail(HAKAI_ERR_STATE, "reset_state before upload_model");
     HIPCHK(hipSetDevice(c->device));
     hipStream_t s = c->stream;
     const size_t fn = 3 * (size_t)c->nN;
     c->cur = 0;
-    HIPCHK(hipMemsetAsync(c->d_u[0], 0, fn * sizeof(double), s));
-    HIPCHK(hipMemsetAsync(c->d_u[1], 0, fn * sizeof(double), s));
+    c->pre = 1;
+    for (int b = 0; b < 3; ++b) HIPCHK(hipMemsetAsync(c->d_u[b], 0, fn * sizeof(double), s));
     HIPCHK(hipMemsetAsync(c->d_fe, 0, (size_t)c->fe_len * sizeof(double), s));
     HIPCHK(hipMemsetAsync(c->d_del_step, 0, ((size_t)c->nEp + 2) * sizeof(int), s));
     HIPCHK(hk::launch_reset_gp(c->d_stress, c->d_strain, c->d_eqps, c->d_yield, c->d_triax, c->d_flag, c->d_mat,
@@ -599,7 +607,7 @@
             dpre[d - 1] = -ic_values[j] * d_time;
             c->h_velo0[d - 1] = ic_values[j];
         }
-        HIPCHK(hipMemcpyAsync(c->d_u[1 - c->cur], dpre.data(), fn * sizeof(double), hipMemcpyHostToDevice, s));
+        HIPCHK(hipMemcpyAsync(hkc::disp_pre(c), dpre.data(), fn * sizeof(double), hipMemcpyHostToDevice, s));
         HIPCHK(hipStreamSynchronize(s));
     }
     c->state_ok = true;
@@ -625,12 +633,12 @@
                         "hakai_download_state) or Qe with this state");
         if (int r = own_materialize(c)) return r;
     }
-    c->own_valid = false;
+    c->own_valid = c->fold_valid = false;
     hipStream_t s = c->stream;
     const size_t fn = 3 * (size_t)c->nN, nGP = 8 * (size_t)c->nE;
-    if (st->disp) HIPCHK(hipMemcpyAsync(c->d_u[c->cur], st->disp, fn * sizeof(double), hipMemcpyHostToDevice, s));
+    if (st->disp) HIPCHK(hipMemcpyAsync(hkc::disp(c), st->disp, fn * sizeof(double), hipMemcpyHostToDevice, s));
     if (st->disp_pre)
-        HIPCHK(hipMemcpyAsync(c->d_u[1 - c->cur], st->disp_pre, fn * sizeof(double), hipMemcpyHostToDevice, s));
+        HIPCHK(hipMemcpyAsync(hkc::disp_pre(c), st->disp_pre, fn * sizeof(double), hipMemcpyHostToDevice, s));
     if (st->velo) c->h_velo0.assign(st->velo, st->velo + fn);
     if (st->Q) {
         HIPCHK(hipMemcpyAsync(c->d_qbuf, st->Q, fn * sizeof(double), hipMemcpyHostToDevice, s));
@@ -707,16 +715,16 @@
     hipStream_t s = c->stream;
     const size_t fn = 3 * (size_t)c->nN, nGP = 8 * (size_t)c->nE;
     HIPCHK(hipStreamSynchronize(s));
-    if (st->disp) HIPCHK(hipMemcpyAsync(st->disp, c->d_u[c->cur], fn * sizeof(double), hipMemcpyDeviceToHost, s));
+    if (st->disp) HIPCHK(hipMemcpyAsync(st->disp, hkc::disp(c), fn * sizeof(double), hipMemcpyDeviceToHost, s));
     if (st->disp_pre)
-        HIPCHK(hipMemcpyAsync(st->disp_pre, c->d_u[1 - c->cur], fn * sizeof(double), hipMemcpyDeviceToHost, s));
+        HIPCHK(hipMemcpyAsync(st->disp_pre, hkc::disp_pre(c), fn * sizeof(double), hipMemcpyDeviceToHost, s));
     if (st->velo) {
         if (c->steps_done == 0) {
             std::memcpy(st->velo, c->h_velo0.data(), fn * sizeof(double));
         } else {
             std::vector<double> a(fn), b(fn);
-            HIPCHK(hipMemcpyAsync(a.data(), c->d_u[c->cur], fn * sizeof(double), hipMemcpyDeviceToHost, s));
-            HIPCHK(hipMemcpyAsync(b.data(), c->d_u[1 - c->cur], fn * sizeof(double), hipMemcpyDeviceToHost, s));
+            HIPCHK(hipMemcpyAsync(a.data(), hkc::disp(c), fn * sizeof(double), hipMemcpyDeviceToHost, s));
+            HIPCHK(hipMemcpyAsync(b.data(), hkc::disp_pre(c), fn * sizeof(double), hipMemcpyDeviceToHost, s));
             HIPCHK(hipStreamSynchronize(s));
             for (size_t i = 0; i < fn; ++i) {
                 const double dd = a[i] - b[i];
@@ -786,6 +794,7 @@
     };
     if (up(&c->d_own_off, pl.off) || up(&c->d_own_seq, sc.seq) || up(&c->d_own_bstart, bst) ||
         up(&c->d_own_list, pl.list) || up(&c->d_own_rp, pl.rp) || up(&c->d_own_ridx, pl.ridx) ||
+        up(&c->d_own_rem, pl.remnant) ||
         dalloc(&c->d_own_q, 3 * (size_t)nN) || dalloc(&c->d_own_rows, 3 * (size_t)std::max(pl.rows, 1LL)) ||
         dalloc(&c->d_own_dump, 8 * (size_t)G) ||
         hipMemsetAsync(c->d_own_q, 0, 3 * (size_t)nN * sizeof(double), s) ||
@@ -793,6 +802,7 @@
         hkc::own_free(c);
         return false;
     }
+    c->own_rem_n = (long long)pl.remnant.size();
     c->own_nop = (int)pl.ne;
     c->own_slots = pl.max_slots;
     c->own_rows = pl.rows;
@@ -848,6 +858,18 @@
 }
 
 enum { kPhaseA1 = 1, kPhaseRest = 2, kPhaseA2 = 4, kPhaseA3 = 8, kPhaseAll = 15 };
+
+static bool fold_ok(const hakai_ctx* c) {
+    return c->own_fold && !c->elem_exact && !c->contact && !c->comm && !c->hist;
+}
+
+static void advance_bufs(hakai_ctx* c, bool folded, long long steps) {
+    for (long long k = folded ? steps % 3 : steps % 2; k > 0; --k) {
+        const int fr = 3 - c->cur - c->pre, old = c->cur;
+        c->cur = folded ? fr : c->pre;
+        c->pre = old;
+    }
+}
 static int step_once(hakai_ctx* c, double t, double d_time, bool last, int phase = kPhaseAll) {
     hipStream_t s = c->stream;
     EventPair ep;
@@ -864,8 +886,8 @@
     if (!(phase & kPhaseRest)) return 0;
     const int par = c->cur;
     hk::NodalArgs na;
-    na.u = c->d_u[c->cur];
-    na.u_pre_out = c->d_u[1 - c->cur];
+    na.u = hkc::disp(c);
+    na.u_pre_out = hkc::disp_pre(c);
     na.mass = c->d_mass;
     na.inc_ptr = c->d_inc_ptr;
     na.inc = c->d_inc;
@@ -875,6 +897,13 @@
     if (c->own_valid && !own) {
         if (int r = own_materialize(c)) return r;
     }
+    const bool folded = c->fold_valid;
+    if (folded && (!own || !c->own_valid || c->q_from_buf || !fold_ok(c)))
+        return fail(HAKAI_ERR_STATE, "step: a folded nodal update is pending but cannot be completed");
+    double* const u_new = folded ? hkc::disp_free(c) : hkc::disp_pre(c);
+    na.u_out = folded ? u_new : nullptr;
+    na.list = folded ? c->d_own_rem : nullptr;
+    na.n_list = folded ? c->own_rem_n : 0;
     na.qbuf = c->q_from_buf ? c->d_qbuf : nullptr;
     na.fext = nullptr;
     na.nN = c->nN;
@@ -894,13 +923,13 @@
     ba.amp_off = c->d_amp_off;
     ba.amp_t = c->d_amp_t;
     ba.amp_v = c->d_amp_v;
-    ba.out = c->d_u[1 - c->cur];
+    ba.out = u_new;
     ba.ct = t * d_time;
     ba.t_rd = c->g_trd;
     ba.dt = d_time;
     ba.poison = c->d_poison;
     na.poison = c->d_poison;
-    const bool fuse_bc = c->nbc > 0 && c->d_bc_of_node && c->fuse_bc && !c->comm &&
+    const bool fuse_bc = c->nbc > 0 && c->d_bc_of_node && c->fuse_bc && !c->comm && !folded &&
                          (c->nN <= kFuseBcMaxNodes || c->fuse_bc == 2);
     if (fuse_bc) {
         na.bc_of_node = c->d_bc_of_node;
@@ -931,7 +960,8 @@
         hkc::prof_end(c, &ep);
     }
     if (c->hist && (rc = hkc::history_step(c, na, fix, t, c->g_trd, s))) return rc;
-    c->cur = 1 - c->cur;
+    advance_bufs(c, folded, 1);
+    c->fold_valid = false;
     c->q_from_buf = false;
     hk::ElemArgs ea = elem_args(c);
     ea.step_i = (int)t;
@@ -948,6 +978,11 @@
         ea.own_rows = c->d_own_rows;
         ea.own_dump = c->d_own_dump;
     }
+    const bool fold = own && !last && fold_ok(c) && c->d_fold_coef && c->fold_coef_dt == d_time;
+    if (fold) {
+        ea.fold_out = hkc::disp_free(c);
+        ea.fold_coef = c->d_fold_coef;
+    }
     if (c->g_trd) {
         ea.t_rd = c->g_trd;
         ea.t_wr = c->d_tstep + par;
@@ -956,7 +991,9 @@
     HIPCHK(hk::launch_element(ea, c->has_ductile, last, s));
     hkc::prof_end(c, &ep);
     c->own_valid = own;
+    c->fold_valid = fold;
     c->own_steps += own ? 1 : 0;
+    c->fold_steps += fold ? 1 : 0;
     c->fe_ok = !own || last;
     c->triax_ok = last;
     rc = hkc::comm_post_element(c, (long long)t);
@@ -971,17 +1008,19 @@
 static bool graph_eligible(const hakai_ctx* c, double t) {
     return c->graph && !c->comm && !c->prof && !c->q_from_buf && c->nE > 0 && hkc::contact_graph_ok(c, t) &&
            !hkc::history_needs_seed(c) &&
-           c->own_valid == own_use(const_cast<hakai_ctx*>(c));
+           c->own_valid == own_use(const_cast<hakai_ctx*>(c)) &&
+           c->fold_valid == (c->own_valid && fold_ok(c) && c->d_fold_coef);
 }
 
 static int step_graph(hakai_ctx* c, double t, double d_time, int len) {
     hipStream_t s = c->stream;
-    const int p0 = c->cur;
+    const int p0 = hkc::buf_key(c);
     const int gi = len == 2 ? 1 : 0;
     hipGraphExec_t& ge = c->g_exec[gi][p0];
-    if (!c->d_tstep) HIPCHK(dalloc(&c->d_tstep, 2));
-    if (c->tdev_next != (long long)t) HIPCHK(hk::launch_set_step(c->d_tstep + (1 - p0), t - 1.0, s));
-    if (ge && (c->g_epoch[gi][p0] != c->epoch || c->g_dt[gi][p0] != d_time || c->g_len[gi][p0] != len)) {
+    if (!c->d_tstep) HIPCHK(dalloc(&c->d_tstep, 3));
+    if (c->tdev_next != (long long)t) HIPCHK(hk::launch_set_step(c->d_tstep + c->pre, t - 1.0, s));
+    if (ge && (c->g_epoch[gi][p0] != c->epoch || c->g_dt[gi][p0] != d_time || c->g_len[gi][p0] != len ||
+               c->g_fold[gi][p0] != c->fold_valid)) {
         HIPCHK(hipStreamSynchronize(s));
         (void)hipGraphExecDestroy(ge);
         ge = nullptr;
@@ -991,7 +1030,7 @@
         HIPCHK(hipStreamBeginCapture(s, hipStreamCaptureModeThreadLocal));
         int rc = 0;
         for (int k = 0; k < len && !rc; ++k) {
-            c->g_trd = c->d_tstep + (1 - c->cur);
+            c->g_trd = c->d_tstep + c->pre;
             rc = step_once(c, t + k, d_time, false);
         }
         c->g_trd = nullptr;
@@ -1010,10 +1049,13 @@
         c->g_epoch[gi][p0] = c->epoch;
         c->g_dt[gi][p0] = d_time;
         c->g_len[gi][p0] = len;
+        c->g_fold[gi][p0] = c->fold_valid;
     } else {
         hkc::contact_graph_advance(c, t + len - 1);
         c->q_from_buf = false;
+        advance_bufs(c, c->fold_valid, len);
         c->own_steps += c->own_valid ? len : 0;
+        c->fold_steps += c->fold_valid ? len : 0;
         c->fe_ok = !c->own_valid;
         c->triax_ok = false;
         c->steps_done += len;
@@ -1026,7 +1068,7 @@
 }
 
 struct CallSnap {
-    int cur = 0;
+    int cur = 0, pre = 1;
     long long done = 0;
     bool fe_ok = true, triax_ok = true, own_valid = false, q_from_buf = false;
     bool comm_pending = false;
@@ -1036,6 +1078,7 @@
     CallSnap s;
     hkc::comm_pending_get(c, &s.comm_pending, &s.comm_par);
     s.cur = c->cur;
+    s.pre = c->pre;
     s.done = c->steps_done;
     s.fe_ok = c->fe_ok;
     s.triax_ok = c->triax_ok;
@@ -1054,7 +1097,8 @@
             const long long good = (long long)pz[1] - (long long)t_first;
             const bool rolled = good >= 0 && good <= n_steps;
             if (rolled) {
-                c->cur = (good & 1) ? 1 - s0.cur : s0.cur;
+                c->cur = (good & 1) ? s0.pre : s0.cur;
+                c->pre = (good & 1) ? s0.cur : s0.pre;
                 c->steps_done = s0.done + good;
                 if (good == 0) {
                     c->fe_ok = s0.fe_ok;
@@ -1102,7 +1146,12 @@
 }
 
 static int step_call(hakai_ctx* c, double t_first, int64_t n_steps, double d_time) {
-    (void)own_use(c);
+    if (own_use(c) && fold_ok(c) && n_steps > 1 && c->fold_coef_dt != d_time) {
+        if (!c->d_fold_coef) HIPCHK(dalloc(&c->d_fold_coef, 3 * (size_t)c->nN));
+        HIPCHK(hk::launch_nodal_coef(c->d_mass, d_time, c->d_fold_coef, c->nN, c->stream));
+        c->fold_coef_dt = d_time;
+        hkc::graph_invalidate(c);
+    }
     const CallSnap s0 = call_snap(c);
     int64_t it = 0;
     while (it < n_steps) {
@@ -1189,6 +1238,7 @@
     if (!c || !key || !value) return fail(HAKAI_ERR_ARG, "null");
     if (!std::strcmp(key, "graph_steps")) *value = c->graph_steps;
     else if (!std::strcmp(key, "own_steps")) *value = c->own_steps;
+    else if (!std::strcmp(key, "fold_steps")) *value = c->fold_steps;
     else if (!std::strcmp(key, "exchange_retries")) *value = c->exchange_retries;
     else if (!std::strcmp(key, "own_rows")) *value = c->own_built_g > 0 ? c->own_rows : -1;
     else if (!std::strcmp(key, "own_entries")) *value = c->own_built_g > 0 ? c->own_entries : -1;
@@ -1280,6 +1330,11 @@
     if (!std::strcmp(key, "own_assembly")) {
         if (value < 0 || value > 2) return fail(HAKAI_ERR_ARG, "own_assembly must be 0, 1 or 2");
         c->own_assembly = (int)value;
+        return 0;
+    }
+    if (!std::strcmp(key, "own_fold")) {
+        if (value != 0 && value != 1) return fail(HAKAI_ERR_ARG, "own_fold must be 0 or 1");
+        c->own_fold = (int)value;
         return 0;
     }
     if (!std::strcmp(key, "own_pass_batches")) {
diff --git a/hakai-fem_amd/csrc/hakai_comm.cpp b/hakai-fem_amd/csrc/hakai_comm.cpp
--- a/hakai-fem_amd/csrc/hakai_comm.cpp
+++ b/hakai-fem_amd/csrc/hakai_comm.cpp
@@ -400,7 +400,7 @@
     if (!m || m->n_up + m->n_dn == 0 || !m->pending) return 0;
     const int n = m->n_up + m->n_dn;
     hipLaunchKernelGGL(k_save_upre, dim3((n + 255) / 256), dim3(256), 0, c->stream, m->d_up, m->n_up, m->d_dn, m->n_dn,
-                       c->d_u[1 - c->cur], m->d_saved);
+                       hkc::disp_pre(c), m->d_saved);
     HIPCHK(hipGetLastError());
     return 0;
 }
@@ -441,14 +441,14 @@
         const int n = m->n_up + m->n_dn;
         hipLaunchKernelGGL(k_fix_own, dim3((n + 255) / 256), dim3(256), 0, c->stream, m->d_up, m->n_up, m->d_dn,
                            m->n_dn, c->d_own_rp, c->d_own_ridx, c->d_own_rows, m->nslot, m->d_up_sendP[par],
-                           m->d_up_recvC, m->d_dn_recvP, m->d_saved, c->d_u[c->cur], c->d_u[1 - c->cur], c->d_mass,
+                           m->d_up_recvC, m->d_dn_recvP, m->d_saved, hkc::disp(c), hkc::disp_pre(c), c->d_mass,
                            c->contact ? c->d_fext : nullptr, d_time, c->d_poison);
         HIPCHK(hipGetLastError());
     } else if (!c->q_from_buf) {
         const int n = m->n_up + m->n_dn;
         hipLaunchKernelGGL(k_fix, dim3((n + 255) / 256), dim3(256), 0, c->stream, m->d_up, m->n_up, m->d_dn, m->n_dn,
                            c->d_inc_ptr, c->d_inc, c->d_fe, m->nslot, m->d_up_sendP[par], m->d_up_recvC, m->d_dn_recvP,
-                           m->d_saved, c->d_u[c->cur], c->d_u[1 - c->cur], c->d_mass, c->contact ? c->d_fext : nullptr,
+                           m->d_saved, hkc::disp(c), hkc::disp_pre(c), c->d_mass, c->contact ? c->d_fext : nullptr,
                            d_time, c->d_poison);
         HIPCHK(hipGetLastError());
     }
diff --git a/hakai-fem_amd/csrc/hakai_contact.hip b/hakai-fem_amd/csrc/hakai_contact.hip
--- a/hakai-fem_amd/csrc/hakai_contact.hip
+++ b/hakai-fem_amd/csrc/hakai_contact.hip
@@ -804,8 +804,8 @@
     Contact* C = c->contact;
     StepIn in;
     in.coord = c->d_coord;
-    in.u = c->d_u[c->cur];
-    in.u_pre = c->d_u[1 - c->cur];
+    in.u = hkc::disp(c);
+    in.u_pre = hkc::disp_pre(c);
     in.flag = c->d_flag;
     in.conn = c->d_conn;
     in.mass = c->d_mass;
diff --git a/hakai-fem_amd/csrc/hakai_internal.hpp b/hakai-fem_amd/csrc/hakai_internal.hpp
--- a/hakai-fem_amd/csrc/hakai_internal.hpp
+++ b/hakai-fem_amd/csrc/hakai_internal.hpp
@@ -28,8 +28,8 @@
     hipStream_t stream = nullptr;
     long long nN = 0, nE = 0, nEp = 0, ld = 0;
     double* d_coord = nullptr;
-    double* d_u[2] = {nullptr, nullptr};
-    int cur = 0;
+    double* d_u[3] = {nullptr, nullptr, nullptr};
+    int cur = 0, pre = 1;
     double* d_mass = nullptr;
     int* d_conn = nullptr;
     int* d_flag = nullptr;
@@ -96,10 +96,11 @@
     long long k_n[HAKAI_K_COUNT] = {0, 0, 0, 0};
     double* d_tstep = nullptr;
     const double* g_trd = nullptr;
-    hipGraphExec_t g_exec[2][2] = {{nullptr, nullptr}, {nullptr, nullptr}};
-    double g_dt[2][2] = {{0.0, 0.0}, {0.0, 0.0}};
-    long long g_epoch[2][2] = {{-1, -1}, {-1, -1}};
-    int g_len[2][2] = {{0, 0}, {0, 0}};
+    hipGraphExec_t g_exec[2][6] = {};
+    double g_dt[2][6] = {};
+    long long g_epoch[2][6] = {{-1, -1, -1, -1, -1, -1}, {-1, -1, -1, -1, -1, -1}};
+    int g_len[2][6] = {};
+    bool g_fold[2][6] = {};
     long long epoch = 0;
     long long tdev_next = -1;
     int graph = 16;
@@ -110,6 +111,13 @@
     int own_band_rows = 0;
     int own_pass_batches = 0;
     bool own_valid = false;
+    int own_fold = 0;
+    bool fold_valid = false;
+    long long fold_steps = 0;
+    int* d_own_rem = nullptr;
+    double* d_fold_coef = nullptr;
+    double fold_coef_dt = 0.0;
+    long long own_rem_n = 0;
     int* d_own_off = nullptr;
     int* d_own_seq = nullptr;
     int* d_own_bstart = nullptr;
@@ -133,6 +141,10 @@
 
 
 namespace hkc {
+inline double* disp(const hakai_ctx* c) { return c->d_u[c->cur]; }
+inline double* disp_pre(const hakai_ctx* c) { return c->d_u[c->pre]; }
+inline double* disp_free(const hakai_ctx* c) { return c->d_u[3 - c->cur - c->pre]; }
+inline int buf_key(const hakai_ctx* c) { return 2 * c->cur + (c->pre == (c->cur + 1) % 3 ? 1 : 0); }
 void prof_begin(hakai_ctx* c, int kernel, EventPair* p);
 void prof_end(hakai_ctx* c, EventPair* p);
 void comm_destroy(hakai_ctx* c);
diff --git a/hakai-fem_amd/csrc/hakai_kernels.hip b/hakai-fem_amd/csrc/hakai_kernels.hip
--- a/hakai-fem_amd/csrc/hakai_kernels.hip
+++ b/hakai-fem_amd/csrc/hakai_kernels.hip
@@ -713,7 +713,36 @@
 
 __device__ __forceinline__ int own_lane(int4 en, int j) { return own_lane(en.y, en.z, en.w, j); }
 
-__device__ __forceinline__ void own_entry(const ElemArgs& a, int4 en, const double* s_fe, double* s_part) {
+struct NodalCoef {
+    double mdt2, inv, hc;
+};
+__device__ __forceinline__ NodalCoef nodal_coef(double m, double dt) {
+#pragma clang fp contract(off)
+    const double dC = 0.0 * m;
+    const double mdt2 = m / (dt * dt);
+    return {mdt2, 1.0 / (mdt2 + dC / 2.0 / dt), dC / 2.0 / dt};
+}
+__device__ __forceinline__ double nodal_dof(const NodalCoef& k, double f, double Q, double uc, double up) {
+#pragma clang fp contract(off)
+    return k.inv * (f - Q + k.mdt2 * (2.0 * uc - up) + k.hc * up);
+}
+
+struct FoldIn {
+    double k[3], uc[3], up[3];
+};
+__device__ __forceinline__ void fold_load(const ElemArgs& a, int4 en, FoldIn& f) {
+    const unsigned n = (en.y & kOwnUpd) ? (unsigned)en.x : 0u;
+#pragma unroll
+    for (int c = 0; c < 3; ++c) {
+        f.k[c] = at32(a.fold_coef, 24u * n)[c];
+        f.uc[c] = at32(a.u, 24u * n)[c];
+        f.up[c] = at32(a.u_pre, 24u * n)[c];
+    }
+}
+
+template <bool FOLD>
+__device__ __forceinline__ void own_entry(const ElemArgs& a, int4 en, const double* s_fe, double* s_part,
+                                          const FoldIn& fi) {
 #pragma clang fp contract(off)
     const int slot = own_slot(en.y), flags = own_flags(en.y), n = own_n(en.y);
     double* dump = a.own_dump + 8 * (long long)blockIdx.x;
@@ -739,7 +768,13 @@
 #pragma unroll
         for (int c = 0; c < 3; ++c) s_part[3 * slot + c] = v[c];
     }
-    double* dst = (flags & kOwnFin) ? a.own_q + 3 * (long long)en.x : dump;
+    const bool upd = FOLD && (en.y & kOwnUpd);
+    if (upd) {
+        const NodalCoef k = {fi.k[0], fi.k[1], fi.k[2]};
+#pragma unroll
+        for (int c = 0; c < 3; ++c) v[c] = nodal_dof(k, 0.0, v[c], fi.uc[c], fi.up[c]);
+    }
+    double* dst = (flags & kOwnFin) ? (upd ? a.fold_out : a.own_q) + 3 * (long long)en.x : dump;
 #pragma unroll
     for (int c = 0; c < 3; ++c) dst[c] = v[c];
 }
@@ -757,8 +792,11 @@
 #define HK_DIAG_PASS
 #endif
 
+template <bool FOLD>
 __device__ __forceinline__ void own_pass(const ElemArgs& a, int4 en, long long sb, const double* s_fe,
                                          double* s_part HK_DIAG_ARG) {
+    FoldIn fi = {};
+    if (FOLD) fold_load(a, en, fi);
 #ifdef HK_DIAG_WAVE
     const long long t0 = clock64();
 #endif
@@ -767,11 +805,15 @@
     const long long t1 = clock64();
 #endif
     const int o0 = a.own_off[sb], o1 = a.own_off[sb + 1];
-    if (o0 + (int)(threadIdx.x & ~63u) < o1) own_entry(a, en, s_fe, s_part);
+    if (o0 + (int)(threadIdx.x & ~63u) < o1) own_entry<FOLD>(a, en, s_fe, s_part, fi);
     if (en.y & kOwnRound2) {
         const int idx = o0 + kBlock + (int)threadIdx.x;
-        if (o0 + kBlock + (int)(threadIdx.x & ~63u) < o1)
-            own_entry(a, a.own_list[idx < o1 ? idx : a.own_nop], s_fe, s_part);
+        if (o0 + kBlock + (int)(threadIdx.x & ~63u) < o1) {
+            const int4 e2 = a.own_list[idx < o1 ? idx : a.own_nop];
+            FoldIn f2 = fi;
+            if (FOLD) fold_load(a, e2, f2);
+            own_entry<FOLD>(a, e2, s_fe, s_part, f2);
+        }
     }
 #ifdef HK_DIAG_WAVE
     const long long t2 = clock64();
@@ -781,8 +823,10 @@
 #endif
 }
 
-template <bool DO_DELETE, bool STORE_TRIAX, bool ANY_PLASTIC, bool LDS_MATS, int NT, bool EXACT, int OS = 0>
+template <bool DO_DELETE, bool STORE_TRIAX, bool ANY_PLASTIC, bool LDS_MATS, int NT, bool EXACT, int OS = 0,
+          bool FOLD = false>
 __global__ __launch_bounds__(kBlock, 2) void k_element_pipe(ElemArgs a) {
+    static_assert(!FOLD || (OS > 0 && !EXACT && !STORE_TRIAX), "FOLD: owner assembly, fused kernel, not a call's last step");
     constexpr bool OWN = OS > 0;
     constexpr int kOwnFe = OS * kEPB * kFeStride;
     __shared__ __attribute__((aligned(16))) double s_nd[kEPB * kLdsStride];
@@ -864,7 +908,7 @@
             elem_step<DO_DELETE, STORE_TRIAX, ANY_PLASTIC, false, NT, OWN>(a, mats, elem_of(i), k, nd8, cur, sfe);
         if (OWN) {
             if ((i + 1) % S == 0 || i + 1 == count)
-                own_pass(a, ent_cur, sb_of(i), s_fe + ((i / S) & 1) * kOwnFe, s_part HK_DIAG_PASS);
+                own_pass<FOLD>(a, ent_cur, sb_of(i), s_fe + ((i / S) & 1) * kOwnFe, s_part HK_DIAG_PASS);
             ent_cur = ent_nxt;
         }
         cur = nxt;
@@ -923,6 +967,17 @@
 template <bool ANY_PLASTIC, bool LDS_MATS, int NT, bool EXACT, int OS>
 static void launch_pipe(const ElemArgs& a, bool do_delete, bool store_triax, unsigned grid, hipStream_t s) {
     const size_t dyn = (OS > 0 ? 24 * (size_t)a.own_slots : 0) + (LDS_MATS ? sizeof(DevMat) * (size_t)a.nmat : 0);
+    if constexpr (OS > 0 && !EXACT) {
+        if (a.fold_out) {
+            if (do_delete)
+                hipLaunchKernelGGL((k_element_pipe<true, false, ANY_PLASTIC, LDS_MATS, NT, EXACT, OS, true>),
+                                   dim3(grid), dim3(kBlock), dyn, s, a);
+            else
+                hipLaunchKernelGGL((k_element_pipe<false, false, ANY_PLASTIC, LDS_MATS, NT, EXACT, OS, true>),
+                                   dim3(grid), dim3(kBlock), dyn, s, a);
+            return;
+        }
+    }
     if (do_delete) {
         if (store_triax)
             hipLaunchKernelGGL((k_element_pipe<true, true, ANY_PLASTIC, LDS_MATS, NT, EXACT, OS>), dim3(grid),
@@ -981,12 +1036,14 @@
             a.own_slots > own_slot_cap(a.exact != 0, a.own, a.nmat))
             return hipErrorInvalidValue;
         if (a.own_grid <= 0 || a.own_grid > nb) return hipErrorInvalidValue;
+        if (a.fold_out && (a.exact || store_triax || !a.fold_coef)) return hipErrorInvalidValue;
         if (a.exact)
             launch_pipe_p<true>(a, do_delete, store_triax, (unsigned)a.own_grid, s);
         else
             launch_pipe_p<false>(a, do_delete, store_triax, (unsigned)a.own_grid, s);
         return hipGetLastError();
     }
+    if (a.fold_out) return hipErrorInvalidValue;
     if (a.pipe_blocks > 0 && !a.vol) {
         const unsigned grid = (unsigned)std::min<long long>(nb, a.pipe_blocks);
         if (a.exact)
@@ -1070,27 +1127,39 @@
     }
 }
 
+__global__ __launch_bounds__(kBlock) void k_nodal_coef(const double* __restrict__ mass, double dt,
+                                                       double* __restrict__ coef, long long nN) {
+    const long long n = (long long)blockIdx.x * kBlock + threadIdx.x;
+    if (n >= nN) return;
+    const NodalCoef k = nodal_coef(mass[n], dt);
+    coef[3 * n + 0] = k.mdt2;
+    coef[3 * n + 1] = k.inv;
+    coef[3 * n + 2] = k.hc;
+}
+
+hipError_t launch_nodal_coef(const double* mass, double dt, double* coef, long long nN, hipStream_t s) {
+    if (nN <= 0) return hipSuccess;
+    hipLaunchKernelGGL(k_nodal_coef, dim3((unsigned)((nN + kBlock - 1) / kBlock)), dim3(kBlock), 0, s, mass, dt, coef,
+                       nN);
+    return hipGetLastError();
+}
+
 template <bool BCF>
 __device__ __forceinline__ void nodal_update(const NodalArgs& a, long long n, const NodeIn& in, double Q0, double Q1,
-                                             double Q2) {
+                                             double Q2, double* out) {
 #pragma clang fp contract(off)
-    const double m = in.m;
-    const double dt = a.dt;
-    const double dC = 0.0 * m;
-    const double mdt2 = m / (dt * dt);
-    const double inv = 1.0 / (mdt2 + dC / 2.0 / dt);
+    const NodalCoef k = nodal_coef(in.m, a.dt);
     const double Q[3] = {Q0, Q1, Q2};
     const int b0 = BCF ? a.bc_of_node[n] : -1;
 #pragma unroll
     for (int c = 0; c < 3; ++c) {
-        const double up = in.up[c];
-        double v = inv * (in.f[c] - Q[c] + mdt2 * (2.0 * in.uc[c] - up) + dC / 2.0 / dt * up);
+        double v = nodal_dof(k, in.f[c], Q[c], in.uc[c], in.up[c]);
         if (BCF) {
             const long long dc = 3 * n + c;
             for (int j = b0; j >= 0 && j < a.bc.n && a.bc.dof[j] <= dc; ++j)
                 if (a.bc.dof[j] == dc) v = bc_value(a.bc, j);
         }
-        a.u_pre_out[3 * n + c] = v;
+        out[3 * n + c] = v;
     }
 }
 
@@ -1099,8 +1168,13 @@
 #pragma clang fp contract(off)
     if (poisoned(a.poison)) return;
     const unsigned lb = xcd_remap_rev(blockIdx.x, gridDim.x);
-    const long long n = (long long)lb * kBlock + threadIdx.x;
-    if (n >= a.nN) return;
+    long long n = (long long)lb * kBlock + threadIdx.x;
+    if (MODE == 4) {
+        if (n >= a.n_list) return;
+        n = a.list[n];
+    } else if (n >= a.nN) {
+        return;
+    }
     NodeIn in;
     nodal_load<FEXT>(a, n, in);
     double Q0 = 0.0, Q1 = 0.0, Q2 = 0.0;
@@ -1108,7 +1182,7 @@
         Q0 = a.qbuf[3 * n + 0];
         Q1 = a.qbuf[3 * n + 1];
         Q2 = a.qbuf[3 * n + 2];
-    } else if (MODE == 3) {
+    } else if (MODE == 3 || MODE == 4) {
         Q0 = a.own_q[3 * n + 0];
         Q1 = a.own_q[3 * n + 1];
         Q2 = a.own_q[3 * n + 2];
@@ -1146,7 +1220,7 @@
             Q2 += f[2];
         }
     }
-    nodal_update<BCF>(a, n, in, Q0, Q1, Q2);
+    nodal_update<BCF>(a, n, in, Q0, Q1, Q2, MODE == 4 ? a.u_out : a.u_pre_out);
 }
 
 template <bool FEXT, bool BCF>
@@ -1163,6 +1237,13 @@
 
 hipError_t launch_nodal(const NodalArgs& a, hipStream_t s) {
     if (a.nN <= 0) return hipSuccess;
+    if (a.list) {
+        if (!a.own_q || !a.u_out || a.qbuf || a.fext || a.bc_of_node || a.n_list > a.nN) return hipErrorInvalidValue;
+        if (a.n_list <= 0) return hipSuccess;
+        hipLaunchKernelGGL((k_nodal<4, false, false>), dim3((unsigned)((a.n_list + kBlock - 1) / kBlock)), dim3(kBlock),
+                           0, s, a);
+        return hipGetLastError();
+    }
     const unsigned grid = (unsigned)((a.nN + kBlock - 1) / kBlock);
     if (a.bc_of_node) {
         if (a.fext)
diff --git a/hakai-fem_amd/csrc/hakai_kernels.hpp b/hakai-fem_amd/csrc/hakai_kernels.hpp
--- a/hakai-fem_amd/csrc/hakai_kernels.hpp
+++ b/hakai-fem_amd/csrc/hakai_kernels.hpp
@@ -49,6 +49,8 @@
     double* own_q;
     double* own_rows;
     double* own_dump;
+    double* fold_out;
+    const double* fold_coef;
 };
 
 struct BCArgs {
@@ -86,6 +88,9 @@
     const int* own_rp;
     const int* own_ridx;
     const double* own_rows;
+    double* u_out;
+    const int* list;
+    long long n_list;
 };
 
 
@@ -99,6 +104,7 @@
 hipError_t launch_negjac(const ElemArgs& a, unsigned long long* count, hipStream_t s);
 hipError_t launch_nodal(const NodalArgs& a, hipStream_t s);
 hipError_t launch_bc(const BCArgs& a, hipStream_t s);
+hipError_t launch_nodal_coef(const double* mass, double dt, double* coef, long long nN, hipStream_t s);
 hipError_t launch_set_step(double* slot, double t_prev, hipStream_t s);
 hipError_t launch_hold(int rounds, hipStream_t s);
 
diff --git a/hakai-fem_amd/csrc/hakai_own_entry.hpp b/hakai-fem_amd/csrc/hakai_own_entry.hpp
--- a/hakai-fem_amd/csrc/hakai_own_entry.hpp
+++ b/hakai-fem_amd/csrc/hakai_own_entry.hpp
@@ -17,7 +17,9 @@
     return (int)(((unsigned)slot & 1023u) | (unsigned)flags << 10 | (unsigned)n << 14 | (unsigned)lane7 << 18 |
                  ((unsigned)slot & 1024u) << 18);
 }
-static_assert((own_pack_y(kOwnSlotsMax - 1, 15, 15, 511) & kOwnRound2) == 0, "kOwnRound2 overlaps a packed field");
+constexpr int kOwnUpd = 1 << 29;
+static_assert((own_pack_y(kOwnSlotsMax - 1, 15, 15, 511) & (kOwnRound2 | kOwnUpd)) == 0 && (kOwnRound2 & kOwnUpd) == 0,
+              "kOwnRound2 / kOwnUpd overlap a packed field");
 
 HK_HD void own_pack(int target, int slot, int flags, int n, const int lanes[8], int w[4]) {
     unsigned long long lo = 0;
diff --git a/hakai-fem_amd/csrc/hakai_own_plan.cpp b/hakai-fem_amd/csrc/hakai_own_plan.cpp
--- a/hakai-fem_amd/csrc/hakai_own_plan.cpp
+++ b/hakai-fem_amd/csrc/hakai_own_plan.cpp
@@ -142,6 +142,7 @@
     if (G <= 0 || in.max_inc > 8 || in.ptr.size() != (size_t)nN + 1) return false;
     pl.S = S;
     struct Ent { int target, slot, flags, n; int lanes[8]; int inc[4]; };
+    std::vector<std::pair<long long, int>> fin_of(nN, {-1, 0});
     std::vector<int> pos_of(nb), block_of(nb);
     std::vector<long long> sb_pos(nb);
     for (long long lb = 0; lb < G; ++lb)
@@ -195,6 +196,7 @@
             sg.refs.emplace_back(sb, (int)per[sb].size() - 1);
         }
         per[sg.s1][sg.refs.back().second].flags |= kOwnFin;
+        fin_of[n] = sg.refs.back();
         if (sg.s1 > sg.s0) segs[hb].push_back(std::move(sg));
         for (; j < j1; ++j) exports.emplace_back(sb_pos[batch_of(j)], j);
     }
@@ -294,6 +296,13 @@
             const Ent& en = per[b][i];
             own_pack(en.target, en.slot, en.flags, en.n, en.lanes, &list[4 * ((size_t)off[b] + i)]);
         }
+    pl.remnant.clear();
+    for (long long n = 0; n < nN; ++n) {
+        if (fin_of[n].first >= 0 && rp[n + 1] == rp[n])
+            list[4 * ((size_t)off[fin_of[n].first] + (size_t)fin_of[n].second) + 1] |= kOwnUpd;
+        else
+            pl.remnant.push_back((int)n);
+    }
     const int no_lanes[8] = {0, 0, 0, 0, 0, 0, 0, 0};
     own_pack(0, 0, kOwnNop, 0, no_lanes, &list[4 * (size_t)ne]);
     pl.rp = std::move(rp);
diff --git a/hakai-fem_amd/csrc/hakai_own_plan.hpp b/hakai-fem_amd/csrc/hakai_own_plan.hpp
--- a/hakai-fem_amd/csrc/hakai_own_plan.hpp
+++ b/hakai-fem_amd/csrc/hakai_own_plan.hpp
@@ -13,6 +13,7 @@
 struct OwnPlan {
     int S = 2;
     std::vector<int> off, list, rp, ridx;
+    std::vector<int> remnant;
     long long rows = 0, ne = 0;
     int max_slots = 1;
     long long round2 = 0;
```

Result: slower. 2542 (-1.7%).
